# Meowuu7/equi-articulated-pose

Measured on AMD Instinct MI355X. Metric: point-clouds/sec (4096 pts, 60 anchors) fwd+bwd, higher is better.
Workload: dtype f32; 1 GPU; 8 x 4096-pt synthetic laptop clouds per GPU, 3-block inter backbone 1->64->128->512 (NN=64,K=24,A=60), forward+backward+Adam; clouds_per_gpu=8, points=4096, anchors=60

## Files before the change

equi-articulated-pose_amd/csrc/bn_act.hip:

```cpp
#include "common.h"

namespace {

constexpr int TB = 256;
constexpr int VPT = 8;
constexpr int SEG = TB * VPT * 4;

__device__ __forceinline__ float wave_sum(float v) {
#pragma unroll
    for (int o = 32; o > 0; o >>= 1) v += __shfl_xor(v, o);
    return v;
}

__device__ __forceinline__ void block_reduce2(float a, float b, float *pa, float *pb) {
    __shared__ float sa[TB / 64], sb[TB / 64];
    a = wave_sum(a); b = wave_sum(b);
    if ((threadIdx.x & 63) == 0) { sa[threadIdx.x >> 6] = a; sb[threadIdx.x >> 6] = b; }
    __syncthreads();
    if (threadIdx.x == 0) {
        float ta = 0.f, tb = 0.f;
#pragma unroll
        for (int i = 0; i < TB / 64; ++i) { ta += sa[i]; tb += sb[i]; }
        *pa = ta; *pb = tb;
    }
// ... 96 lines not shown
    const size_t o = ((size_t)ci * gridDim.z + bi) * nseg + seg;
    block_reduce2(s, q, pg + o, pgx + o);
}

template <bool CLOUD>
__global__ __launch_bounds__(TB) void bn_act_bwd_apply_kernel(int c, long n, float slope, const float *__restrict__ gy,
                                                             const float *__restrict__ x, const float *__restrict__ scale,
                                                             const float *__restrict__ shift, const float *__restrict__ mean,
                                                             const float *__restrict__ invstd, const float *__restrict__ k2,
                                                             const float *__restrict__ k3, float *__restrict__ gx,
                                                             const float *__restrict__ mask, int na) {
    const int seg = blockIdx.x, ci = blockIdx.y, bi = blockIdx.z;
    const int si = CLOUD ? bi * c + ci : ci;
    const float sc = scale[si], sh = shift[si], mu = mean[si], is = invstd[si], c2 = k2[si], c3 = k3[si];
    const size_t r0 = ((size_t)bi * c + ci) * n;
    const float *mrow = (CLOUD && mask) ? mask + (size_t)bi * (unsigned)(n / na) : nullptr;
    const long base = (long)seg * SEG;
    auto one = [&](float g, float xv, float m) {
        const float pre = fmaf(xv, sc, sh);
        const float gg = pre > 0.f ? g : g * slope;
        if (CLOUD) return fmaf(-m, fmaf((xv - mu) * is, c3, c2), gg * sc);
        return fmaf(gg, sc, -c2) - ((xv - mu) * is) * c3;
    };
#pragma unroll
    for (int v = 0; v < VPT; ++v) {
        const long i = base + ((long)v * TB + threadIdx.x) * 4;
        if (i + 3 < n) {
            const float4 g = *reinterpret_cast<const float4 *>(gy + r0 + i);
            const float4 a = *reinterpret_cast<const float4 *>(x + r0 + i);
            const float m = mrow ? mrow[(unsigned)i / (unsigned)na] : 1.f;
            *reinterpret_cast<float4 *>(gx + r0 + i) = make_float4(one(g.x, a.x, m), one(g.y, a.y, m), one(g.z, a.z, m), one(g.w, a.w, m));
        } else {
            for (long j = i; j < n; ++j) gx[r0 + j] = one(gy[r0 + j], x[r0 + j], mrow ? mrow[(unsigned)j / (unsigned)na] : 1.f);
        }
    }
}

constexpr int RM_PIECES = 16;
__global__ __launch_bounds__(256) void bn_act_bwd_apply_rowmax_kernel(int c, long n4, int nq, float slope, const float4 *__restrict__ gy,
                                                                      const float4 *__restrict__ x, const float *__restrict__ scale,
                                                                      const float *__restrict__ shift, const float *__restrict__ mean,
                                                                      const float *__restrict__ invstd, const float *__restrict__ k2,
                                                                      const float *__restrict__ k3, float4 *__restrict__ gx,
                                                                      unsigned *__restrict__ rowmax) {
    __shared__ unsigned s_max[256][4];
    const int ci = blockIdx.y, bi = blockIdx.z, t = threadIdx.x;
    const int T = nq * (256 / nq);
    const float sc = scale[ci], sh = shift[ci], mu = mean[ci], is = invstd[ci], c2 = k2[ci], c3 = k3[ci];
    const size_t r0 = ((size_t)bi * c + ci) * (size_t)n4;
    const long base = (long)blockIdx.x * RM_PIECES * T;
    auto one = [&](float g, float xv) {
        const float pre = fmaf(xv, sc, sh);
        const float gg = pre > 0.f ? g : g * slope;
        return fmaf(gg, sc, -c2) - ((xv - mu) * is) * c3;
    };
    unsigned m0 = 0, m1 = 0, m2 = 0, m3 = 0;
    if (t < T) {
        float4 g[RM_PIECES], a[RM_PIECES];
#pragma unroll
        for (int v = 0; v < RM_PIECES; ++v) {
            const long i = base + (long)v * T + t;
            if (i < n4) { g[v] = gy[r0 + i]; a[v] = x[r0 + i]; }
        }
#pragma unroll
        for (int v = 0; v < RM_PIECES; ++v) {
            const long i = base + (long)v * T + t;
            if (i < n4) {
                const float4 o = make_float4(one(g[v].x, a[v].x), one(g[v].y, a[v].y), one(g[v].z, a[v].z), one(g[v].w, a[v].w));
                gx[r0 + i] = o;
                m0 = max(m0, __float_as_uint(o.x) & 0x7fffffffu); m1 = max(m1, __float_as_uint(o.y) & 0x7fffffffu);
                m2 = max(m2, __float_as_uint(o.z) & 0x7fffffffu); m3 = max(m3, __float_as_uint(o.w) & 0x7fffffffu);
            }
        }
    }
    s_max[t][0] = m0; s_max[t][1] = m1; s_max[t][2] = m2; s_max[t][3] = m3;
    __syncthreads();
    if (t < 4 * nq) {
        unsigned v = 0;
        for (int u = t >> 2; u < T; u += nq) v = max(v, s_max[u][t & 3]);
        if (v) atomicMax(rowmax + ((size_t)bi * c + ci) * (4 * nq) + t, v);
    }
}

__global__ __launch_bounds__(256) void bn_act_bwd_reduce_fromy_kernel(int c, long n4, int nq, int nblk, float slope, float inv_slope, const float4 *__restrict__ gy,
                                                                      const float4 *__restrict__ y, const float *__restrict__ beta,
                                                                      const float *__restrict__ inv_gamma, float *__restrict__ pg, float *__restrict__ pgx,
                                                                      unsigned *__restrict__ gmax, unsigned *__restrict__ xmax) {
    __shared__ unsigned s_max[256][8];
    const int ci = blockIdx.y, bi = blockIdx.z, t = threadIdx.x;
    const int T = nq * (256 / nq);
    const float be = beta[ci], ig = inv_gamma[ci];
    const size_t r0 = ((size_t)bi * c + ci) * (size_t)n4;
    const long base = (long)blockIdx.x * RM_PIECES * T;
    float s = 0.f, q = 0.f;
    unsigned mg[4] = {0, 0, 0, 0}, mx[4] = {0, 0, 0, 0};
    if (t < T) {
        float4 g[RM_PIECES], a[RM_PIECES];
#pragma unroll
        for (int v = 0; v < RM_PIECES; ++v) {
            const long i = base + (long)v * T + t;
            if (i < n4) { g[v] = gy[r0 + i]; a[v] = y[r0 + i]; }
        }
#pragma unroll
        for (int v = 0; v < RM_PIECES; ++v) {
            const long i = base + (long)v * T + t;
            if (i < n4) {
                const float gv[4] = {g[v].x, g[v].y, g[v].z, g[v].w}, yv[4] = {a[v].x, a[v].y, a[v].z, a[v].w};
#pragma unroll
                for (int e = 0; e < 4; ++e) {
                    const bool pos = yv[e] > 0.f;
                    const float gg = pos ? gv[e] : gv[e] * slope, xh = ((pos ? yv[e] : yv[e] * inv_slope) - be) * ig;
                    s += gg;
                    q = fmaf(gg, xh, q);
                    mg[e] = max(mg[e], __float_as_uint(gg) & 0x7fffffffu);
                    mx[e] = max(mx[e], __float_as_uint(xh) & 0x7fffffffu);
                }
            }
        }
    }
#pragma unroll
    for (int e = 0; e < 4; ++e) { s_max[t][e] = mg[e]; s_max[t][4 + e] = mx[e]; }
    const size_t o = ((size_t)ci * gridDim.z + bi) * nblk + blockIdx.x;
    block_reduce2(s, q, pg + o, pgx + o);
    if (t < 4 * nq) {
        unsigned vg = 0, vx = 0;
        for (int u = t >> 2; u < T; u += nq) { vg = max(vg, s_max[u][t & 3]); vx = max(vx, s_max[u][4 + (t & 3)]); }
        const size_t at = ((size_t)bi * c + ci) * (4 * nq) + t;
        if (vg) atomicMax(gmax + at, vg);
        if (vx) atomicMax(xmax + at, vx);
    }
}

inline int nseg_of(long n) { return (int)((n + SEG - 1) / SEG); }

}

extern "C" int eap_bn_act_segments(int64_t n) { return nseg_of((long)n); }

extern "C" int eap_bn_stats_f32(int b, int c, int64_t n, const float *x, float *psum, float *psq, eap_stream_t stream) {
    if (b <= 0 || c <= 0 || n <= 0) return 0;
    if ((n & 3) != 0) return eap::bad_arg("bn_stats: row length must be a multiple of 4");
    const int nseg = nseg_of(n);
    return eap::run_kernel("bn_stats", bn_stats_kernel<false>, nseg, c, b, dim3(TB), 0, eap::S(stream), c, (long)n, nseg, x, psum, psq, (const float *)nullptr, 1);
}

extern "C" int eap_bn_act_fwd_f32(int b, int c, int64_t n, float slope, const float *x, const float *scale,
                                  const float *shift, float *y, eap_stream_t stream) {
    if (b <= 0 || c <= 0 || n <= 0) return 0;
    if ((n & 3) != 0) return eap::bad_arg("bn_act_fwd: row length must be a multiple of 4");
    return eap::run_kernel("bn_act_fwd", bn_act_fwd_kernel<false, false>, nseg_of(n), c, b, dim3(TB), 0, eap::S(stream), c, (long)n, slope, x, scale, shift,
                           (const float *)nullptr, y);
}

extern "C" int eap_bn_act_add_fwd_f32(int b, int c, int64_t n, float slope, const float *x, const float *scale,
                                      const float *shift, const float *res, float *y, eap_stream_t stream) {
    if (b <= 0 || c <= 0 || n <= 0) return 0;
    if ((n & 3) != 0) return eap::bad_arg("bn_act_add_fwd: row length must be a multiple of 4");
    return eap::run_kernel("bn_act_add_fwd", bn_act_fwd_kernel<true, false>, nseg_of(n), c, b, dim3(TB), 0, eap::S(stream), c, (long)n, slope, x, scale, shift,
                           res, y);
}

extern "C" int eap_bn_act_bwd_reduce_f32(int b, int c, int64_t n, float slope, const float *gy, const float *x,
                                         const float *scale, const float *shift, const float *mean,
                                         const float *invstd, float *pg, float *pgx, eap_stream_t stream) {
    if (b <= 0 || c <= 0 || n <= 0) return 0;
    if ((n & 3) != 0) return eap::bad_arg("bn_act_bwd_reduce: row length must be a multiple of 4");
    const int nseg = nseg_of(n);
    return eap::run_kernel("bn_act_bwd_reduce", bn_act_bwd_reduce_kernel<false>, nseg, c, b, dim3(TB), 0, eap::S(stream), c, (long)n, nseg, slope, gy, x,
                           scale, shift, mean, invstd, pg, pgx);
}

extern "C" int eap_bn_act_bwd_apply_f32(int b, int c, int64_t n, float slope, const float *gy, const float *x,
                                        const float *scale, const float *shift, const float *mean,
                                        const float *invstd, const float *k2, const float *k3, float *gx,
                                        eap_stream_t stream) {
    if (b <= 0 || c <= 0 || n <= 0) return 0;
    if ((n & 3) != 0) return eap::bad_arg("bn_act_bwd_apply: row length must be a multiple of 4");
    return eap::run_kernel("bn_act_bwd_apply", bn_act_bwd_apply_kernel<false>, nseg_of(n), c, b, dim3(TB), 0, eap::S(stream), c, (long)n, slope, gy, x,
                           scale, shift, mean, invstd, k2, k3, gx, (const float *)nullptr, 1);
}

extern "C" int eap_bn_act_bwd_apply_rowmax_f32(int b, int c, int64_t n, int na, float slope, const float *gy, const float *x,
                                               const float *scale, const float *shift, const float *mean,
                                               const float *invstd, const float *k2, const float *k3, float *gx, uint32_t *rowmax,
                                               eap_stream_t stream) {
    if (b <= 0 || c <= 0 || n <= 0) return 0;
    if (na <= 0 || (na & 3) != 0 || na > 256 || n % na != 0 ||
        ((reinterpret_cast<uintptr_t>(gy) | reinterpret_cast<uintptr_t>(x) | reinterpret_cast<uintptr_t>(gx)) & 15) != 0)
        return eap::bad_arg("bn_act_bwd_apply_rowmax: rows of [points][na], na a multiple of 4 up to 256, 16-byte aligned tensors");
    hipStream_t s = eap::S(stream);
    if (int e = eap::hip_fail(hipMemsetAsync(rowmax, 0, sizeof(uint32_t) * (size_t)b * c * na, s), "bn_act_bwd_apply_rowmax memset")) return e;
    const int nq = na / 4, T = nq * (256 / nq);
    const long n4 = (long)(n / 4);
    return eap::run_kernel("bn_act_bwd_apply_rowmax", bn_act_bwd_apply_rowmax_kernel, eap::cdiv(n4, (long)RM_PIECES * T), c, b, dim3(256), 0, s, c, n4, nq,
                           slope, reinterpret_cast<const float4 *>(gy), reinterpret_cast<const float4 *>(x), scale, shift, mean, invstd, k2, k3,
                           reinterpret_cast<float4 *>(gx), rowmax);
}

extern "C" int eap_bn_act_fromy_blocks(int64_t n, int na) {
    if (na <= 0 || (na & 3) != 0 || na > 256) return 0;
    const int nq = na / 4, T = nq * (256 / nq);
    const long n4 = (long)(n / 4);
    return (int)((n4 + (long)RM_PIECES * T - 1) / ((long)RM_PIECES * T));
}

extern "C" int eap_bn_act_bwd_reduce_fromy_f32(int b, int c, int64_t n, int na, float slope, const float *gy, const float *y, const float *beta,
                                               const float *inv_gamma, float *pg, float *pgx, uint32_t *gmax, uint32_t *xmax, eap_stream_t stream) {
    if (b <= 0 || c <= 0 || n <= 0) return 0;
    if (na <= 0 || (na & 3) != 0 || na > 256 || n % na != 0 || !(slope > 0.f) ||
        ((reinterpret_cast<uintptr_t>(gy) | reinterpret_cast<uintptr_t>(y)) & 15) != 0)
        return eap::bad_arg("bn_act_bwd_reduce_fromy: rows of [points][na], na a multiple of 4 up to 256, 16-byte aligned tensors, a positive slope");
    hipStream_t s = eap::S(stream);
    if (int e = eap::hip_fail(hipMemsetAsync(gmax, 0, sizeof(uint32_t) * (size_t)b * c * na, s), "bn_act_bwd_reduce_fromy memset")) return e;
    if (int e = eap::hip_fail(hipMemsetAsync(xmax, 0, sizeof(uint32_t) * (size_t)b * c * na, s), "bn_act_bwd_reduce_fromy memset")) return e;
    const int nq = na / 4, nblk = eap_bn_act_fromy_blocks(n, na);
    return eap::run_kernel("bn_act_bwd_reduce_fromy", bn_act_bwd_reduce_fromy_kernel, nblk, c, b, dim3(256), 0, s, c, (long)(n / 4), nq, nblk, slope,
                           1.0f / slope, reinterpret_cast<const float4 *>(gy), reinterpret_cast<const float4 *>(y), beta, inv_gamma, pg, pgx, gmax, xmax);
}

namespace {
inline int cloud_dims(const char *who, int b, int c, long n, int na, bool masked) {
    char buf[200];
    if ((n & 3) != 0 || n >= (1l << 31)) {
        snprintf(buf, sizeof(buf), "%s: row length must be a multiple of 4 below 2^31", who);
        return eap::bad_arg(buf);
    }
    if (masked && (na <= 0 || (na & 3) != 0 || n % na != 0)) {
        snprintf(buf, sizeof(buf), "%s: with a mask a row is [points][na], na a multiple of 4", who);
        return eap::bad_arg(buf);
    }
    return 0;
}
}

extern "C" int eap_bn_stats_masked_f32(int b, int c, int64_t n, int na, const float *x, const float *mask, float *psum, float *psq,
                                       eap_stream_t stream) {
    if (b <= 0 || c <= 0 || n <= 0) return 0;
    if (!mask) return eap::bad_arg("bn_stats_masked: mask is null");
    if (int e = cloud_dims("bn_stats_masked", b, c, (long)n, na, true)) return e;
    const int nseg = nseg_of(n);
    return eap::run_kernel("bn_stats_masked", bn_stats_kernel<true>, nseg, c, b, dim3(TB), 0, eap::S(stream), c, (long)n, nseg, x, psum, psq, mask, na);
}

extern "C" int eap_bn_act_cloud_fwd_f32(int b, int c, int64_t n, float slope, const float *x, const float *scale, const float *shift,
                                        float *y, eap_stream_t stream) {
    if (b <= 0 || c <= 0 || n <= 0) return 0;
    if (int e = cloud_dims("bn_act_cloud_fwd", b, c, (long)n, 0, false)) return e;
    return eap::run_kernel("bn_act_cloud_fwd", bn_act_fwd_kernel<false, true>, nseg_of(n), c, b, dim3(TB), 0, eap::S(stream), c, (long)n, slope, x, scale,
                           shift, (const float *)nullptr, y);
}

extern "C" int eap_bn_act_cloud_bwd_reduce_f32(int b, int c, int64_t n, float slope, const float *gy, const float *x, const float *scale,
                                               const float *shift, const float *mean, const float *invstd, float *pg, float *pgx,
                                               eap_stream_t stream) {
    if (b <= 0 || c <= 0 || n <= 0) return 0;
    if (int e = cloud_dims("bn_act_cloud_bwd_reduce", b, c, (long)n, 0, false)) return e;
    const int nseg = nseg_of(n);
    return eap::run_kernel("bn_act_cloud_bwd_reduce", bn_act_bwd_reduce_kernel<true>, nseg, c, b, dim3(TB), 0, eap::S(stream), c, (long)n, nseg, slope, gy, x,
                           scale, shift, mean, invstd, pg, pgx);
}

extern "C" int eap_bn_act_cloud_bwd_apply_f32(int b, int c, int64_t n, int na, float slope, const float *gy, const float *x,
                                              const float *scale, const float *shift, const float *mean, const float *invstd,
                                              const float *k2, const float *k3, const float *mask, float *gx, eap_stream_t stream) {
    if (b <= 0 || c <= 0 || n <= 0) return 0;
    if (int e = cloud_dims("bn_act_cloud_bwd_apply", b, c, (long)n, na, mask != nullptr)) return e;
    return eap::run_kernel("bn_act_cloud_bwd_apply", bn_act_bwd_apply_kernel<true>, nseg_of(n), c, b, dim3(TB), 0, eap::S(stream), c, (long)n, slope, gy, x,
                           scale, shift, mean, invstd, k2, k3, gx, mask, mask ? na : 1);
}
```

equi-articulated-pose_amd/csrc/inv_lists.hip:

```cpp
#include "common.h"

namespace {

constexpr int RT = 1024;
constexpr int MAXN = 16384;
constexpr int SORT_COMPACT = 2048;

__global__ __launch_bounds__(256) void inv_count_kernel(int per_cloud, int n, const int32_t *__restrict__ idx,
                                                        int32_t *__restrict__ counts) {
    extern __shared__ int s_hist[];
    const int bi = blockIdx.y, t = threadIdx.x;
    for (int i = t; i < n; i += 256) s_hist[i] = 0;
    __syncthreads();
    const int chunk = (per_cloud + gridDim.x - 1) / gridDim.x;
    const int beg = blockIdx.x * chunk, end = min(per_cloud, beg + chunk);
    const int32_t *src = idx + (size_t)bi * per_cloud;
    for (int e = beg + t; e < end; e += 256) {
        const int q = src[e];
        if ((unsigned)q < (unsigned)n) atomicAdd(&s_hist[q], 1);
    }
    __syncthreads();
    for (int i = t; i < n; i += 256) {
        const int v = s_hist[i];
        if (v) atomicAdd(&counts[(size_t)bi * n + i], v);
// ... 99 lines not shown
        if (i < qend) v = src[i];
        const bool m0 = v.x == q, m1 = v.y == q, m2 = v.z == q, m3 = v.w == q;
        const unsigned long long b0 = __ballot(m0), b1 = __ballot(m1), b2 = __ballot(m2), b3 = __ballot(m3);
        if ((b0 | b1 | b2 | b3) == 0ull) continue;
        int pos = base;
        pos += __builtin_amdgcn_mbcnt_hi((unsigned)(b0 >> 32), __builtin_amdgcn_mbcnt_lo((unsigned)b0, 0));
        pos += __builtin_amdgcn_mbcnt_hi((unsigned)(b1 >> 32), __builtin_amdgcn_mbcnt_lo((unsigned)b1, 0));
        pos += __builtin_amdgcn_mbcnt_hi((unsigned)(b2 >> 32), __builtin_amdgcn_mbcnt_lo((unsigned)b2, 0));
        pos += __builtin_amdgcn_mbcnt_hi((unsigned)(b3 >> 32), __builtin_amdgcn_mbcnt_lo((unsigned)b3, 0));
        const int e = 4 * i;
        if (m0) { dp[pos] = e / nn; dg[pos] = sg[e]; ++pos; }
        if (m1) { dp[pos] = (e + 1) / nn; dg[pos] = sg[e + 1]; ++pos; }
        if (m2) { dp[pos] = (e + 2) / nn; dg[pos] = sg[e + 2]; ++pos; }
        if (m3) { dp[pos] = (e + 3) / nn; dg[pos] = sg[e + 3]; ++pos; }
        base += __popcll(b0) + __popcll(b1) + __popcll(b2) + __popcll(b3);
    }
}

__global__ __launch_bounds__(256) void rows_gather_kernel(int c, int n, int na4, int rcap, int rld,
                                                          const int32_t *__restrict__ rows, const float4 *__restrict__ src,
                                                          float4 *__restrict__ dst) {
    const int bi = blockIdx.z, ci = blockIdx.y;
    const int e = blockIdx.x * 256 + threadIdx.x;
    if (e >= rcap * na4) return;
    const int r = e / na4, a = e - r * na4;
    const int q = rows[(size_t)bi * rld + r];
    float4 v = make_float4(0.f, 0.f, 0.f, 0.f);
    if (q >= 0) v = src[(((size_t)bi * c + ci) * n + q) * na4 + a];
    dst[(((size_t)bi * c + ci) * rcap + r) * na4 + a] = v;
}

__global__ __launch_bounds__(256) void rows_scatter_kernel(int c, int n, int na4, int rcap, int rld,
                                                           const int32_t *__restrict__ rows, const float4 *__restrict__ src,
                                                           float4 *__restrict__ dst) {
    const int bi = blockIdx.z, ci = blockIdx.y;
    const int e = blockIdx.x * 256 + threadIdx.x;
    if (e >= rcap * na4) return;
    const int r = e / na4, a = e - r * na4;
    const int q = rows[(size_t)bi * rld + r];
    if (q >= 0) dst[(((size_t)bi * c + ci) * n + q) * na4 + a] = src[(((size_t)bi * c + ci) * rcap + r) * na4 + a];
}

constexpr int PACKED_SLOTS = 64, PACKED_MAX_NA = 64;
__global__ __launch_bounds__(256) void rows_gather_packed_kernel(int c, int n, int na, int rp, int rld, long long ld, const int32_t *__restrict__ rows,
                                                                 const int32_t *__restrict__ n_rows, const float *__restrict__ src, float *__restrict__ dst) {
    __shared__ float tile[PACKED_SLOTS][PACKED_MAX_NA + 1];
    const int bi = blockIdx.z, ci = blockIdx.y, r0 = blockIdx.x * PACKED_SLOTS, t = threadIdx.x;
    const int live = eap::live16(n_rows[bi], rp), nr = min(n_rows[bi], live);
    if (r0 >= live) return;
    const float *s = src + ((size_t)bi * c + ci) * n * na;
    for (int i = t; i < PACKED_SLOTS * na; i += 256) {
        const int rr = i / na, a = i - rr * na, r = r0 + rr;
        const int q = r < nr ? rows[(size_t)bi * rld + r] : -1;
        tile[rr][a] = (q >= 0 && q < n) ? s[(size_t)q * na + a] : 0.f;
    }
    __syncthreads();
    float *d = dst + ((size_t)bi * c + ci) * ld;
    for (int i = t; i < PACKED_SLOTS * na; i += 256) {
        const int a = i / PACKED_SLOTS, rr = i - a * PACKED_SLOTS, r = r0 + rr;
        if (r < live) d[(size_t)a * live + r] = tile[rr][a];
    }
}

__global__ __launch_bounds__(256) void rows_scatter_packed_kernel(int c, int c_ld, int n, int na, int rp, int rld, long long ld, const int32_t *__restrict__ rows,
                                                                  const int32_t *__restrict__ n_rows, const float *__restrict__ src, float *__restrict__ dst) {
    __shared__ float tile[PACKED_SLOTS][PACKED_MAX_NA + 1];
    const int bi = blockIdx.z, ci = blockIdx.y, r0 = blockIdx.x * PACKED_SLOTS, t = threadIdx.x;
    const int live = eap::live16(n_rows[bi], rp), nr = min(n_rows[bi], live);
    if (r0 >= live) return;
    const float *s = src + ((size_t)bi * c_ld + ci) * ld;
    for (int i = t; i < PACKED_SLOTS * na; i += 256) {
        const int a = i / PACKED_SLOTS, rr = i - a * PACKED_SLOTS, r = r0 + rr;
        if (r < live) tile[rr][a] = s[(size_t)a * live + r];
    }
    __syncthreads();
    float *d = dst + ((size_t)bi * c + ci) * n * na;
    for (int i = t; i < PACKED_SLOTS * na; i += 256) {
        const int rr = i / na, a = i - rr * na, r = r0 + rr;
        const int q = r < nr ? rows[(size_t)bi * rld + r] : -1;
        if (q >= 0 && q < n) d[(size_t)q * na + a] = tile[rr][a];
    }
}

}

extern "C" int eap_inv_lists_rows(int b, int p, int n, int nn, const int32_t *idx, int32_t *counts, int32_t *rows,
                                  int32_t *off, int32_t *cnt, int32_t *n_rows, eap_stream_t stream) {
    if (b <= 0 || p <= 0 || nn <= 0 || n <= 0) return 0;
    if (n > MAXN) return eap::bad_arg("inv_lists_rows: more than 16384 support points per cloud");
    if ((long long)p * nn >= (1ll << 31)) return eap::bad_arg("inv_lists_rows: more than 2^31 entries per cloud");
    hipStream_t s = eap::S(stream);
    int e = eap::hip_fail(hipMemsetAsync(counts, 0, sizeof(int32_t) * (size_t)b * n, s), "inv_lists_rows memset");
    if (e) return e;
    const int per_cloud = p * nn;
    e = eap::run_kernel("inv_lists_rows (count)", inv_count_kernel, eap::cdiv(per_cloud, 8192), b, 1, dim3(256), sizeof(int) * n, s, per_cloud, n, idx, counts);
    if (e) return e;
    int n2 = RT;
    while (n2 < n) n2 <<= 1;
    const size_t shmem = sizeof(unsigned long long) * n2;
    return eap::run_kernel("inv_lists_rows (sort)", inv_rows_kernel, b, 1, 1, dim3(RT), shmem, s, n, n2, counts, rows, off, cnt, n_rows);
}

extern "C" int eap_inv_lists_fill(int b, int p, int n, int nn, int rcap, const int32_t *idx, const float *gx,
                                  const int32_t *rows, const int32_t *off, int32_t *ent_p, float *ent_gx,
                                  eap_stream_t stream) {
    if (b <= 0 || p <= 0 || nn <= 0 || rcap <= 0) return 0;
    if (((long long)p * nn & 3) != 0) return eap::bad_arg("inv_lists_fill: p * nn must be a multiple of 4");
    if (rcap > n) return eap::bad_arg("inv_lists_fill: rcap exceeds the number of support points");
    return eap::run_kernel("inv_lists_fill", inv_fill_kernel, rcap, b, 1, dim3(256), 0, eap::S(stream), p * nn, nn, n, n, idx, reinterpret_cast<const float4 *>(gx),
                           rows, off, ent_p, reinterpret_cast<float4 *>(ent_gx));
}

extern "C" int eap_rows_gather_f32(int b, int c, int n, int na, int rcap, int rows_ld, const int32_t *rows,
                                   const float *src, float *dst, eap_stream_t stream) {
    if (b <= 0 || c <= 0 || rcap <= 0) return 0;
    if ((na & 3) != 0) return eap::bad_arg("rows_gather: na must be a multiple of 4");
    return eap::run_kernel("rows_gather", rows_gather_kernel, eap::cdiv((long long)rcap * (na / 4), 256), c, b, dim3(256), 0, eap::S(stream), c, n, na / 4, rcap, rows_ld,
                           rows, reinterpret_cast<const float4 *>(src), reinterpret_cast<float4 *>(dst));
}

extern "C" int eap_rows_scatter_f32(int b, int c, int n, int na, int rcap, int rows_ld, const int32_t *rows,
                                    const float *src, float *dst, eap_stream_t stream) {
    if (b <= 0 || c <= 0) return 0;
    if ((na & 3) != 0) return eap::bad_arg("rows_scatter: na must be a multiple of 4");
    hipStream_t s = eap::S(stream);
    int e = eap::hip_fail(hipMemsetAsync(dst, 0, sizeof(float) * (size_t)b * c * n * na, s), "rows_scatter memset");
    if (e || rcap <= 0) return e;
    return eap::run_kernel("rows_scatter", rows_scatter_kernel, eap::cdiv((long long)rcap * (na / 4), 256), c, b, dim3(256), 0, s, c, n, na / 4, rcap, rows_ld, rows,
                           reinterpret_cast<const float4 *>(src), reinterpret_cast<float4 *>(dst));
}

extern "C" int eap_rows_gather_packed_f32(int b, int c, int n, int na, int rp, int rows_ld, int64_t ld, const int32_t *rows, const int32_t *n_rows,
                                          const float *src, float *dst, eap_stream_t stream) {
    if (!rows || !n_rows || !src || !dst) return eap::bad_arg("rows_gather_packed: null pointer");
    if (b <= 0 || c <= 0 || n <= 0 || na <= 0 || rp <= 0) return eap::bad_arg("rows_gather_packed: every size must be positive");
    if (na > PACKED_MAX_NA || rp % 16 != 0 || rows_ld < rp || ld < (int64_t)na * rp)
        return eap::bad_arg("rows_gather_packed: na <= 64, rp a multiple of 16, the row stride of rows >= rp, ld >= na * rp");
    return eap::run_kernel("rows_gather_packed", rows_gather_packed_kernel, eap::cdiv(rp, PACKED_SLOTS), c, b, dim3(256), 0, eap::S(stream), c, n, na, rp,
                           rows_ld, (long long)ld, rows, n_rows, src, dst);
}

extern "C" int eap_rows_scatter_packed_f32(int b, int c, int c_ld, int n, int na, int rp, int rows_ld, int64_t ld, const int32_t *rows,
                                           const int32_t *n_rows, const float *src, float *dst, eap_stream_t stream) {
    if (!rows || !n_rows || !src || !dst) return eap::bad_arg("rows_scatter_packed: null pointer");
    if (b <= 0 || c <= 0 || n <= 0 || na <= 0 || rp <= 0) return eap::bad_arg("rows_scatter_packed: every size must be positive");
    if (na > PACKED_MAX_NA || rp % 16 != 0 || rows_ld < rp || ld < (int64_t)na * rp || c_ld < c)
        return eap::bad_arg("rows_scatter_packed: na <= 64, rp a multiple of 16, the row stride of rows >= rp, ld >= na * rp, c_ld >= c");
    hipStream_t s = eap::S(stream);
    if (int e = eap::hip_fail(hipMemsetAsync(dst, 0, sizeof(float) * (size_t)b * c * n * na, s), "rows_scatter_packed memset")) return e;
    return eap::run_kernel("rows_scatter_packed", rows_scatter_packed_kernel, eap::cdiv(rp, PACKED_SLOTS), c, b, dim3(256), 0, s, c, c_ld, n, na, rp, rows_ld,
                           (long long)ld, rows, n_rows, src, dst);
}
```

equi-articulated-pose_amd/csrc/narrow_conv.hip:

```cpp
#include "common.h"
#include "device_prims.h"
#include <type_traits>

namespace {

constexpr int NT = 256, WAVES = 4;
constexpr int TILE = 128;
constexpr int SEGC = 2048;

__device__ __forceinline__ int drow(int r, int h) { return (r & 3) + 8 * (r >> 2) + 4 * h; }

template <int KS2>
__device__ __forceinline__ void load_x(f32x4 (&xa)[KS2], const float *__restrict__ xb, long n, long col0, unsigned voff, bool ok, int ck, int h) {
#pragma unroll
    for (int s = 0; s < KS2; ++s)
        xa[s] = (ok && 2 * s + h < ck) ? ld_off<f32x4>(xb + (size_t)(2 * s) * n + col0, voff) : (f32x4){0.f, 0.f, 0.f, 0.f};
}

template <int KS2>
__device__ __forceinline__ void load_w(float (&wf)[KS2], const float *__restrict__ W, int orow, int ck, int h) {
#pragma unroll
    for (int s = 0; s < KS2; ++s) wf[s] = (2 * s + h < ck) ? W[(size_t)orow * ck + 2 * s + h] : 0.f;
}

template <int KS2, bool T>
__device__ __forceinline__ void conv_tile(f32x16 (&d)[4], const f32x4 (&xa)[KS2], const float (&wf)[KS2]) {
#pragma unroll
    for (int c = 0; c < 4; ++c)
#pragma unroll
        for (int r = 0; r < 16; ++r) d[c][r] = 0.f;
#pragma unroll
    for (int s = 0; s < KS2; ++s) {
        if (T) {
            d[0] = __builtin_amdgcn_mfma_f32_32x32x2f32(xa[s].x, wf[s], d[0], 0, 0, 0);
            d[1] = __builtin_amdgcn_mfma_f32_32x32x2f32(xa[s].y, wf[s], d[1], 0, 0, 0);
            d[2] = __builtin_amdgcn_mfma_f32_32x32x2f32(xa[s].z, wf[s], d[2], 0, 0, 0);
            d[3] = __builtin_amdgcn_mfma_f32_32x32x2f32(xa[s].w, wf[s], d[3], 0, 0, 0);
        } else {
            d[0] = __builtin_amdgcn_mfma_f32_32x32x2f32(wf[s], xa[s].x, d[0], 0, 0, 0);
            d[1] = __builtin_amdgcn_mfma_f32_32x32x2f32(wf[s], xa[s].y, d[1], 0, 0, 0);
            d[2] = __builtin_amdgcn_mfma_f32_32x32x2f32(wf[s], xa[s].z, d[2], 0, 0, 0);
            d[3] = __builtin_amdgcn_mfma_f32_32x32x2f32(wf[s], xa[s].w, d[3], 0, 0, 0);
        }
    }
}

__device__ __forceinline__ void block_sums(float (&sa)[16], float (&qa)[16], float (*s_red)[2][32], int ct, int o0, int bi, int nb,
                                           int nseg, int seg, float *__restrict__ pa, float *__restrict__ pq) {
    const int t = threadIdx.x, lane = t & 63, wave = t >> 6, li = lane & 31, h = lane >> 5;
#pragma unroll
    for (int r = 0; r < 16; ++r) {
        float a = sa[r], q = qa[r];
#pragma unroll
        for (int d = 16; d > 0; d >>= 1) { a += __shfl_xor(a, d); q += __shfl_xor(q, d); }
        if (li == 0) { s_red[wave][0][drow(r, h)] = a; s_red[wave][1][drow(r, h)] = q; }
    }
    __syncthreads();
    if (t < 32 * ct) {
        float a = 0.f, q = 0.f;
        for (int w = t >> 5; w < WAVES; w += ct) { a += s_red[w][0][t & 31]; q += s_red[w][1][t & 31]; }
        const size_t at = ((size_t)(o0 + t) * nb + bi) * nseg + seg;
        pa[at] = a; pq[at] = q;
    }
}

struct Pos {
    int seg, bi, lane, li, h, ch0, cw, ncw;
    long beg, end;
    unsigned xoff;
    __device__ Pos(int ct, long n) {
        seg = blockIdx.x; bi = blockIdx.z;
        const int wave = threadIdx.x >> 6;
        lane = threadIdx.x & 63; li = lane & 31; h = lane >> 5;
        ch0 = (blockIdx.y * ct + wave % ct) * 32; cw = wave / ct; ncw = WAVES / ct;
        beg = (long)seg * SEGC; end = min(n, beg + SEGC);
        xoff = 4u * ((unsigned)h * (unsigned)n + 4u * li);
    }
};

template <int KS2>
__global__ __launch_bounds__(NT) void narrow_conv_stats_kernel(int ct, int ck, long n, int nseg, const float *__restrict__ W,
                                                                 const float *__restrict__ x, float *__restrict__ pivot,
                                                                 float *__restrict__ psum, float *__restrict__ psq) {
    __shared__ __attribute__((aligned(16))) float s_piv[64];
    __shared__ float s_red[WAVES][2][32];
    const Pos w(ct, n);
    const int t = threadIdx.x, o0 = blockIdx.y * ct * 32, h = w.h;
    if (t < 32 * ct) {
        float p = 0.f;
        for (int k = 0; k < ck; ++k) p = fmaf(W[(size_t)(o0 + t) * ck + k], x[(size_t)k * n], p);
        s_piv[t] = p;
        if (w.seg == 0 && w.bi == 0) pivot[o0 + t] = p;
    }
    __syncthreads();
    float wf[KS2];
    load_w<KS2>(wf, W, w.ch0 + w.li, ck, h);
    f32x4 pv[4];
#pragma unroll
    for (int g = 0; g < 4; ++g) pv[g] = *reinterpret_cast<const f32x4 *>(&s_piv[w.ch0 - o0 + 8 * g + 4 * h]);
    float sa[16], qa[16];
#pragma unroll
    for (int r = 0; r < 16; ++r) sa[r] = qa[r] = 0.f;
    const float *xb = x + (size_t)w.bi * ck * n;
#pragma unroll 1
    for (long col0 = w.beg + (long)w.cw * TILE; col0 < w.end; col0 += (long)w.ncw * TILE) {
        const long col = col0 + 4 * w.li;
        const bool ok = col < n;
        f32x4 xa[KS2];
        load_x<KS2>(xa, xb, n, col0, w.xoff, ok, ck, h);
        f32x16 d[4];
        conv_tile<KS2, false>(d, xa, wf);
        if (ok) {
#pragma unroll
            for (int r = 0; r < 16; ++r)
#pragma unroll
                for (int c = 0; c < 4; ++c) {
                    const float dd = d[c][r] - pv[r >> 2][r & 3];
                    sa[r] += dd;
                    qa[r] = fmaf(dd, dd, qa[r]);
                }
        }
    }
    block_sums(sa, qa, s_red, ct, o0, w.bi, gridDim.z, nseg, w.seg, psum, psq);
}

template <int KS2>
__global__ __launch_bounds__(NT) void narrow_conv_bnact_fwd_kernel(int ct, int o, int ck, long n, float slope, const float *__restrict__ W,
                                                                     const float *__restrict__ x, const float *__restrict__ scale,
                                                                     const float *__restrict__ shift, float *__restrict__ y) {
    const Pos w(ct, n);
    const int h = w.h;
    float wf[KS2];
    load_w<KS2>(wf, W, w.ch0 + w.li, ck, h);
    f32x4 sc[4], sh[4];
#pragma unroll
    for (int g = 0; g < 4; ++g) {
        sc[g] = *reinterpret_cast<const f32x4 *>(scale + w.ch0 + 8 * g + 4 * h);
        sh[g] = *reinterpret_cast<const f32x4 *>(shift + w.ch0 + 8 * g + 4 * h);
    }
    const float *xb = x + (size_t)w.bi * ck * n;
    float *yb = y + ((size_t)w.bi * o + w.ch0) * n;
    const unsigned roff = 4u * (4u * h * (unsigned)n + 4u * w.li);
#pragma unroll 1
    for (long col0 = w.beg + (long)w.cw * TILE; col0 < w.end; col0 += (long)w.ncw * TILE) {
        const long col = col0 + 4 * w.li;
        const bool ok = col < n;
        f32x4 xa[KS2];
        load_x<KS2>(xa, xb, n, col0, w.xoff, ok, ck, h);
        f32x16 d[4];
        conv_tile<KS2, false>(d, xa, wf);
        if (ok) {
#pragma unroll
            for (int r = 0; r < 16; ++r) {
                const float a = sc[r >> 2][r & 3], b = sh[r >> 2][r & 3];
                f32x4 v;
                v.x = fmaf(d[0][r], a, b); v.y = fmaf(d[1][r], a, b); v.z = fmaf(d[2][r], a, b); v.w = fmaf(d[3][r], a, b);
                v.x = v.x > 0.f ? v.x : v.x * slope; v.y = v.y > 0.f ? v.y : v.y * slope;
                v.z = v.z > 0.f ? v.z : v.z * slope; v.w = v.w > 0.f ? v.w : v.w * slope;
                st_off<f32x4>(yb + (size_t)(8 * (r >> 2)) * n + col0, roff + 4u * (unsigned)(r & 3) * (unsigned)n, v);
            }
        }
    }
}

template <int KS2>
__global__ __launch_bounds__(NT) void narrow_conv_bwd_reduce_kernel(int ct, int o, int ck, long n, int nseg, float slope,
                                                                      const float *__restrict__ gy, const float *__restrict__ x,
                                                                      const float *__restrict__ W, const float *__restrict__ scale,
                                                                      const float *__restrict__ shift, const float *__restrict__ mean,
                                                                      const float *__restrict__ invstd, float *__restrict__ pg,
                                                                      float *__restrict__ pgx) {
    __shared__ __attribute__((aligned(16))) float s_sc[64], s_sh[64], s_mu[64], s_is[64];
    __shared__ float s_red[WAVES][2][32];
    const Pos w(ct, n);
    const int t = threadIdx.x, o0 = blockIdx.y * ct * 32, h = w.h;
    if (t < 32 * ct) { s_sc[t] = scale[o0 + t]; s_sh[t] = shift[o0 + t]; s_mu[t] = mean[o0 + t]; s_is[t] = invstd[o0 + t]; }
    __syncthreads();
    float wf[KS2];
    load_w<KS2>(wf, W, w.ch0 + w.li, ck, h);
    float sa[16], qa[16];
#pragma unroll
    for (int r = 0; r < 16; ++r) sa[r] = qa[r] = 0.f;
    const float *xb = x + (size_t)w.bi * ck * n;
    const float *gb = gy + ((size_t)w.bi * o + w.ch0) * n;
    const unsigned roff = 4u * (4u * h * (unsigned)n + 4u * w.li);
    const int lc = w.ch0 - o0;
#pragma unroll 1
    for (long col0 = w.beg + (long)w.cw * TILE; col0 < w.end; col0 += (long)w.ncw * TILE) {
        const long col = col0 + 4 * w.li;
        const bool ok = col < n;
        f32x4 xa[KS2];
        load_x<KS2>(xa, xb, n, col0, w.xoff, ok, ck, h);
        f32x16 d[4];
        conv_tile<KS2, false>(d, xa, wf);
        if (ok) {
#pragma unroll
            for (int g = 0; g < 4; ++g) {
                f32x4 gv[4];
#pragma unroll
                for (int q = 0; q < 4; ++q) gv[q] = ld_off<f32x4>(gb + (size_t)(8 * g) * n + col0, roff + 4u * q * (unsigned)n);
                const f32x4 sc = *reinterpret_cast<const f32x4 *>(&s_sc[lc + 8 * g + 4 * h]), sh = *reinterpret_cast<const f32x4 *>(&s_sh[lc + 8 * g + 4 * h]);
                const f32x4 mu = *reinterpret_cast<const f32x4 *>(&s_mu[lc + 8 * g + 4 * h]), is = *reinterpret_cast<const f32x4 *>(&s_is[lc + 8 * g + 4 * h]);
#pragma unroll
                for (int q = 0; q < 4; ++q)
#pragma unroll
                    for (int c = 0; c < 4; ++c) {
                        const float yv = d[c][4 * g + q];
                        const float pre = fmaf(yv, sc[q], sh[q]);
                        const float gg = pre > 0.f ? gv[q][c] : gv[q][c] * slope;
                        sa[4 * g + q] += gg;
                        qa[4 * g + q] = fmaf(gg, (yv - mu[q]) * is[q], qa[4 * g + q]);
                    }
            }
        }
    }
    block_sums(sa, qa, s_red, ct, o0, w.bi, gridDim.z, nseg, w.seg, pg, pgx);
}

template <int KS2>
__global__ __launch_bounds__(NT) void narrow_conv_bwd_dw_kernel(int ct, int o, int ck, long n, int nseg, float slope,
                                                                  const float *__restrict__ gy, const float *__restrict__ x,
                                                                  const float *__restrict__ W, const float *__restrict__ scale,
                                                                  const float *__restrict__ shift, const float *__restrict__ mean,
                                                                  const float *__restrict__ invstd, const float *__restrict__ k2,
                                                                  const float *__restrict__ k3, float *__restrict__ partial) {
    __shared__ float s_part[WAVES][16][64];
    const Pos w(ct, n);
    const int h = w.h, li = w.li, wave = threadIdx.x >> 6;
    const int ch = w.ch0 + li;
    float wf[KS2];
    load_w<KS2>(wf, W, ch, ck, h);
    const float sc = scale[ch], sh = shift[ch], mu = mean[ch], is = invstd[ch], c2 = k2[ch], c3 = k3[ch];
    const float *gb = gy + ((size_t)w.bi * o + w.ch0) * n;
    const unsigned goff = 4u * ((unsigned)li * (unsigned)n + 16u * h), koff = 4u * ((unsigned)min(li, ck - 1) * (unsigned)n + 16u * h);
    f32x16 dw;
#pragma unroll
    for (int r = 0; r < 16; ++r) dw[r] = 0.f;
    const float *xb = x + (size_t)w.bi * ck * n;
    const f32x4 zero4 = {0.f, 0.f, 0.f, 0.f};
#pragma unroll 1
    for (long col0 = w.beg + (long)w.cw * TILE; col0 < w.end; col0 += (long)w.ncw * TILE) {
        const long col = col0 + 4 * li;
        f32x4 xa[KS2];
        load_x<KS2>(xa, xb, n, col0, w.xoff, col < n, ck, h);
        f32x16 d[4];
        conv_tile<KS2, true>(d, xa, wf);
#pragma unroll
        for (int g = 0; g < 4; ++g) {
            f32x4 gv[4], xv[4];
#pragma unroll
            for (int q = 0; q < 4; ++q) {
                const long cq = col0 + 4 * (8 * g + 4 * h + q);
                const bool in = cq < n;
                gv[q] = in ? ld_off<f32x4>(gb + col0 + 4 * (8 * g + q), goff) : zero4;
                xv[q] = (in && li < ck) ? ld_off<f32x4>(xb + col0 + 4 * (8 * g + q), koff) : zero4;
            }
#pragma unroll
            for (int q = 0; q < 4; ++q)
#pragma unroll
                for (int c = 0; c < 4; ++c) {
                    const float yv = d[c][4 * g + q];
                    const float pre = fmaf(yv, sc, sh);
                    const float gg = pre > 0.f ? gv[q][c] : gv[q][c] * slope;
                    const float gx = fmaf(gg, sc, -c2) - ((yv - mu) * is) * c3;
                    dw = __builtin_amdgcn_mfma_f32_32x32x2f32(gx, xv[q][c], dw, 0, 0, 0);
                }
        }
    }
#pragma unroll
    for (int r = 0; r < 16; ++r) s_part[wave][r][w.lane] = dw[r];
    __syncthreads();
    if (wave < ct) {
        float *slab = partial + ((size_t)w.bi * nseg + w.seg) * o * ck;
#pragma unroll
        for (int r = 0; r < 16; ++r) {
            float v = 0.f;
            for (int u = wave; u < WAVES; u += ct) v += s_part[u][r][w.lane];
            if (li < ck) slab[(size_t)(w.ch0 + drow(r, h)) * ck + li] = v;
        }
    }
}

__global__ __launch_bounds__(256) void narrow_conv_dw_sum_kernel(int mn, int slabs, const float *__restrict__ partial, float *__restrict__ dW) {
    const int e = blockIdx.x * 4 + (threadIdx.x >> 6), lane = threadIdx.x & 63;
    if (e >= mn) return;
    float s = 0.f;
    for (int z = lane; z < slabs; z += 64) s += partial[(size_t)z * mn + e];
#pragma unroll
    for (int d = 32; d > 0; d >>= 1) s += __shfl_xor(s, d);
    if (lane == 0) dW[e] = s;
}

inline int nseg_of(long n) { return (int)((n + SEGC - 1) / SEGC); }

inline bool misaligned(const void *p) { return (reinterpret_cast<uintptr_t>(p) & 15) != 0; }

inline int refuse(const char *who, int o, int ck, long n, const void *p0, const void *p1, const void *p2 = nullptr) {
    char buf[200];
    const char *why = nullptr;
    if (ck < 1 || ck > 32) why = "1 to 32 contraction indices (C*K)";
    else if (o < 32 || o % 32 != 0) why = "a multiple of 32 output channels";
    else if (n < 0 || (n & 3) != 0 || n >= (1l << 25)) why = "a row length (P*A) that is a multiple of 4 below 2^25";
    else if (misaligned(p0) || misaligned(p1) || misaligned(p2)) why = "16-byte aligned tensors";
    if (!why) return 0;
    snprintf(buf, sizeof(buf), "%s: takes %s", who, why);
    return eap::bad_arg(buf);
}

inline int tiles_per_block(int o) { return o % 64 == 0 ? 2 : 1; }

template <typename F>
int by_depth(int ck, F &&f) {
    return ck <= 24 ? f(std::integral_constant<int, 12>{}) : f(std::integral_constant<int, 16>{});
}

}

extern "C" int eap_narrow_conv_segments(int64_t n) { return n > 0 ? nseg_of((long)n) : 0; }

extern "C" int eap_narrow_conv_stats_f32(int b, int o, int ck, int64_t n, const float *W, const float *x, float *pivot, float *psum,
                                         float *psq, eap_stream_t stream) {
    if (int e = refuse("narrow_conv_stats", o, ck, (long)n, x, nullptr)) return e;
    if (b <= 0 || n <= 0) return 0;
    const int nseg = nseg_of((long)n), ct = tiles_per_block(o);
    return by_depth(ck, [&](auto ks2) {
        return eap::run_kernel("narrow_conv_stats", narrow_conv_stats_kernel<decltype(ks2)::value>, nseg, o / (32 * ct), b, dim3(NT), 0, eap::S(stream), ct,
                               ck, (long)n, nseg, W, x, pivot, psum, psq);
    });
}

extern "C" int eap_narrow_conv_bnact_fwd_f32(int b, int o, int ck, int64_t n, float slope, const float *W, const float *x, const float *scale,
                                             const float *shift, float *y, eap_stream_t stream) {
    if (int e = refuse("narrow_conv_bnact_fwd", o, ck, (long)n, x, y, scale)) return e;
    if (misaligned(shift)) return eap::bad_arg("narrow_conv_bnact_fwd: takes 16-byte aligned tensors");
    if (b <= 0 || n <= 0) return 0;
    const int ct = tiles_per_block(o);
    return by_depth(ck, [&](auto ks2) {
        return eap::run_kernel("narrow_conv_bnact_fwd", narrow_conv_bnact_fwd_kernel<decltype(ks2)::value>, nseg_of((long)n), o / (32 * ct), b, dim3(NT), 0,
                               eap::S(stream), ct, o, ck, (long)n, slope, W, x, scale, shift, y);
    });
}

extern "C" int eap_narrow_conv_bwd_reduce_f32(int b, int o, int ck, int64_t n, float slope, const float *gy, const float *x, const float *W,
                                              const float *scale, const float *shift, const float *mean, const float *invstd, float *pg,
                                              float *pgx, eap_stream_t stream) {
    if (int e = refuse("narrow_conv_bwd_reduce", o, ck, (long)n, x, gy)) return e;
    if (b <= 0 || n <= 0) return 0;
    const int nseg = nseg_of((long)n), ct = tiles_per_block(o);
    return by_depth(ck, [&](auto ks2) {
        return eap::run_kernel("narrow_conv_bwd_reduce", narrow_conv_bwd_reduce_kernel<decltype(ks2)::value>, nseg, o / (32 * ct), b, dim3(NT), 0, eap::S(stream),
                               ct, o, ck, (long)n, nseg, slope, gy, x, W, scale, shift, mean, invstd, pg, pgx);
    });
}

extern "C" int eap_narrow_conv_bwd_dw_f32(int b, int o, int ck, int64_t n, float slope, const float *gy, const float *x, const float *W,
                                          const float *scale, const float *shift, const float *mean, const float *invstd, const float *k2,
                                          const float *k3, float *partial, float *dW, eap_stream_t stream) {
    if (int e = refuse("narrow_conv_bwd_dw", o, ck, (long)n, x, gy)) return e;
    if (b <= 0 || n <= 0) return 0;
    const int nseg = nseg_of((long)n), ct = tiles_per_block(o);
    hipStream_t s = eap::S(stream);
    int e = by_depth(ck, [&](auto ks2) {
        return eap::run_kernel("narrow_conv_bwd_dw", narrow_conv_bwd_dw_kernel<decltype(ks2)::value>, nseg, o / (32 * ct), b, dim3(NT), 0, s, ct, o, ck, (long)n,
                               nseg, slope, gy, x, W, scale, shift, mean, invstd, k2, k3, partial);
    });
    if (e) return e;
    const int mn = o * ck;
    return eap::run_kernel("narrow_conv_bwd_dw (sum)", narrow_conv_dw_sum_kernel, eap::cdiv(mn, 4), 1, 1, dim3(256), 0, s, mn, b * nseg, partial, dW);
}
```

equi-articulated-pose_amd/csrc/so3_dense.hip:

```cpp
#include <atomic>
#include "common.h"
#include "device_prims.h"
#include <type_traits>

namespace {

typedef unsigned long long u64;
typedef const __attribute__((address_space(4))) unsigned long long *cu64p;

constexpr int KC_BK = 32;
constexpr int KC_LIST_BYTES = 4096;

__host__ __device__ __forceinline__ void dense_kr(int d, int ks, int &k, int &r) {
    const int g = d / (16 * ks), rem = d - g * 16 * ks;
    k = rem >> 4;
    r = 16 * g + (rem & 15);
}


__device__ __forceinline__ void split2(float x0, float x1, unsigned &h, unsigned &l) {
    asm("v_cvt_pk_f16_f32 %0, %2, %3\n\t"
        "v_fma_mixlo_f16 %1, %0, -1.0, %2 op_sel:[0,0,0] op_sel_hi:[1,0,0]\n\t"
        "v_fma_mixhi_f16 %1, %0, -1.0, %3 op_sel:[1,0,0] op_sel_hi:[1,0,0]"
        : "=&v"(h), "=&v"(l) : "v"(x0), "v"(x1));
// ... 173 lines not shown
}

__global__ __launch_bounds__(256) void dense_rows_kernel(int n_sup, int na, int ks, int rp, int kd_pad, int rows_ld,
                                                         const float *__restrict__ s_xyz, const float *__restrict__ centre,
                                                         const int32_t *__restrict__ rows, const float *__restrict__ rk,
                                                         const float *__restrict__ row_rot, f32x4 *__restrict__ kr) {
    const int b = blockIdx.z, a = blockIdx.y, i = blockIdx.x * 256 + threadIdx.x;
    if (i >= kd_pad) return;
    f32x4 v = {1e4f, 1e4f, 1e4f, 0.f};
    if (i < ks * rp) {
        int k, r;
        dense_kr(i, ks, k, r);
        const int row = rows[(size_t)b * rows_ld + r];
        if ((unsigned)row < (unsigned)n_sup) {
            const float *kp = rk + ((size_t)a * ks + k) * 3;
            double k0 = (double)kp[0], k1 = (double)kp[1], k2 = (double)kp[2];
            if (row_rot != nullptr) {
                const float *M = row_rot + ((size_t)b * rows_ld + r) * 9;
                const double t0 = M[0] * k0 + M[1] * k1 + M[2] * k2, t1 = M[3] * k0 + M[4] * k1 + M[5] * k2, t2 = M[6] * k0 + M[7] * k1 + M[8] * k2;
                k0 = t0; k1 = t1; k2 = t2;
            }
            const double x = (double)s_xyz[((size_t)b * 3 + 0) * n_sup + row] - (double)centre[b * 4 + 0] - k0;
            const double y = (double)s_xyz[((size_t)b * 3 + 1) * n_sup + row] - (double)centre[b * 4 + 1] - k1;
            const double z = (double)s_xyz[((size_t)b * 3 + 2) * n_sup + row] - (double)centre[b * 4 + 2] - k2;
            v = (f32x4){(float)x, (float)y, (float)z, 0.f};
        }
    }
    kr[((size_t)b * na + a) * kd_pad + i] = v;
}

__global__ __launch_bounds__(256) void dense_rowmax_kernel(int m, int l, int na, int seg, long long seg_pitch4, const int32_t *__restrict__ colmap,
                                                           const f32x4 *__restrict__ T, float *__restrict__ scale, float *__restrict__ scale2) {
    __shared__ unsigned s[256][4];
    const int nq = na >> 2, G = 256 / nq, b = blockIdx.y, row = blockIdx.x, t = threadIdx.x;
    const int aq = t % nq, pg = t / nq;
    unsigned v0 = 0, v1 = 0, v2 = 0, v3 = 0;
    if (pg < G) {
        const f32x4 *src = T + ((size_t)b * m + row) * (colmap ? (size_t)1 : (size_t)(l / seg)) * seg_pitch4;
        for (int i0 = pg; i0 < l; i0 += 8 * G) {
            f32x4 q[8];
#pragma unroll
            for (int u = 0; u < 8; ++u) {
                const int i = min(i0 + u * G, l - 1), sg = i / seg;
                if (colmap != nullptr) {
                    const int ci = colmap[(size_t)b * l + i];
                    q[u] = ci >= 0 ? src[(size_t)ci * nq + aq] : (f32x4){0.f, 0.f, 0.f, 0.f};
                } else {
                    q[u] = src[(size_t)sg * seg_pitch4 + (size_t)(i - sg * seg) * nq + aq];
                }
            }
#pragma unroll
            for (int u = 0; u < 8; ++u) {
                v0 = max(v0, __float_as_uint(q[u].x) & 0x7fffffffu);
                v1 = max(v1, __float_as_uint(q[u].y) & 0x7fffffffu);
                v2 = max(v2, __float_as_uint(q[u].z) & 0x7fffffffu);
                v3 = max(v3, __float_as_uint(q[u].w) & 0x7fffffffu);
            }
        }
    }
    s[t][0] = v0; s[t][1] = v1; s[t][2] = v2; s[t][3] = v3;
    __syncthreads();
    if (t < na) {
        unsigned v = 0;
        for (int g = 0; g < G; ++g) v = max(v, s[g * nq + (t >> 2)][t & 3]);
        const float sc = pow2_scale(__uint_as_float(v));
        scale[((size_t)b * na + t) * m + row] = sc;
        scale2[((size_t)b * m + row) * na + t] = sc;
    }
}

__global__ __launch_bounds__(256) void dense_scale_kernel(long long total, int m, int na, const unsigned *__restrict__ rowmax,
                                                          float *__restrict__ scale, float *__restrict__ scale2) {
    const long long i = (long long)blockIdx.x * 256 + threadIdx.x;
    if (i >= total) return;
    const int a = (int)(i % na);
    const long long br = i / na;
    const int row = (int)(br % m);
    const long long b = br / m;
    const float sc = pow2_scale(__uint_as_float(rowmax[i]));
    scale[(b * na + a) * m + row] = sc;
    scale2[i] = sc;
}

struct SplitBn { const f32x4 *Y2; const float *coef; float slope, inv_slope; };
template <bool BN>
__global__ __launch_bounds__(256) __attribute__((amdgpu_waves_per_eu(2, 2))) void dense_split_kernel(int m, int l, int na, int kb_total, int seg, long long seg_pitch4, int mapped,
                                                          const int32_t *__restrict__ n_rows, const int32_t *__restrict__ colmap,
                                                          const f32x4 *__restrict__ T, const float *__restrict__ scale2,
                                                          u32x4 *__restrict__ planes, SplitBn bn) {
    extern __shared__ u32x4 image[];
    const int t = threadIdx.x;
    const int MT = m >> 5;
    const unsigned blk = blockIdx.x >> 1;
    const int kg = (int)(blockIdx.x & 1u), kb = (int)(blk % (unsigned)kb_total), grp_ = (int)(blk / (unsigned)kb_total), mt = grp_ % MT, b = grp_ / MT;
    const int nq = na >> 2, RG = 256 / nq;
    const int aq = t % nq, rr = t / nq;
    const int nseg = l / seg;
    if (mapped && n_rows != nullptr && 16 * kb >= ((min(n_rows[b], seg) + 15) & ~15) * nseg) return;
    const int l0 = 16 * kb + 8 * kg;
    unsigned at[8], keep[8];
    int live = 0;
    if (colmap != nullptr) {
        int ci[8] = {-1, -1, -1, -1, -1, -1, -1, -1};
        if (l0 < l) {
            const int4 c0 = *reinterpret_cast<const int4 *>(colmap + (size_t)b * l + l0), c1 = *reinterpret_cast<const int4 *>(colmap + (size_t)b * l + l0 + 4);
            ci[0] = c0.x; ci[1] = c0.y; ci[2] = c0.z; ci[3] = c0.w; ci[4] = c1.x; ci[5] = c1.y; ci[6] = c1.z; ci[7] = c1.w;
        }
#pragma unroll
        for (int e = 0; e < 8; ++e) { keep[e] = ci[e] >= 0 ? ~0u : 0u; at[e] = (unsigned)max(ci[e], 0) * (unsigned)nq; live |= (int)(keep[e] & 1u) << e; }
    } else {
        int sg = l0 / seg, sr = l0 - sg * seg;
        if (mapped) dense_kr(l0, nseg, sg, sr);
#pragma unroll
        for (int e = 0; e < 8; ++e) {
            keep[e] = l0 + e < l ? ~0u : 0u;
            at[e] = keep[e] ? (unsigned)sg * (unsigned)seg_pitch4 + (unsigned)sr * (unsigned)nq : 0u;
            live |= (int)(keep[e] & 1u) << e;
            if (++sr == seg) { sr = 0; ++sg; }
        }
#pragma unroll
        for (int e = 1; e < 8; ++e) at[e] = keep[e] ? at[e] : at[0];
    }
    if (live == 0)
        for (int i = t; i < 64 * na; i += 256) image[i] = (u32x4){0u, 0u, 0u, 0u};
    for (int it0 = rr; it0 < 32 && rr < RG && live != 0; it0 += 2 * RG) {
        f32x4 q[2][8];
        f32x4 q2[BN ? 2 : 1][BN ? 8 : 1];
        int rowv[2];
#pragma unroll
        for (int u = 0; u < 2; ++u) {
            const int row = 32 * mt + min(it0 + u * RG, 31);
            rowv[u] = row;
            const size_t row_off = ((size_t)b * m + row) * (colmap ? (size_t)1 : (size_t)nseg) * seg_pitch4 + aq;
#pragma unroll
            for (int e = 0; e < 8; ++e) q[u][e] = T[row_off + at[e]];
            if constexpr (BN) {
#pragma unroll
                for (int e = 0; e < 8; ++e) q2[u][e] = bn.Y2[row_off + at[e]];
            }
        }
        __builtin_amdgcn_sched_barrier(0);
        if constexpr (BN) {
#pragma unroll
            for (int u = 0; u < 2; ++u) {
                const float k1 = bn.coef[rowv[u]], k2 = bn.coef[m + rowv[u]], k3 = bn.coef[2 * m + rowv[u]], be = bn.coef[3 * m + rowv[u]], ig = bn.coef[4 * m + rowv[u]];
#pragma unroll
                for (int e = 0; e < 8; ++e)
#pragma unroll
                    for (int j = 0; j < 4; ++j) {
                        const float yv = q2[u][e][j], gv = q[u][e][j];
                        const bool pos = yv > 0.f;
                        const float gg = pos ? gv : gv * bn.slope, pre = pos ? yv : yv * bn.inv_slope;
                        const float gx = fmaf(gg, k1, -k2) - ((pre - be) * ig) * k3;
                        q[u][e][j] = __uint_as_float(__float_as_uint(gx) & keep[e]);
                    }
            }
        } else if (live != 255) {
#pragma unroll
            for (int u = 0; u < 2; ++u)
#pragma unroll
                for (int e = 0; e < 8; ++e)
#pragma unroll
                    for (int j = 0; j < 4; ++j) q[u][e][j] = __uint_as_float(__float_as_uint(q[u][e][j]) & keep[e]);
        }
#pragma unroll
        for (int u = 0; u < 2; ++u) {
            const int i = it0 + u * RG;
            if (i >= 32) break;
            const f32x4 sc = *reinterpret_cast<const f32x4 *>(scale2 + ((size_t)b * m + rowv[u]) * na + 4 * aq);
            u32x4 *dst = image + 256 * aq + ((i + aq) & 31);
#pragma unroll
            for (int j = 0; j < 4; ++j) {
                unsigned h[4], lo[4];
#pragma unroll
                for (int e = 0; e < 4; ++e) split2(q[u][2 * e][j] * sc[j], q[u][2 * e + 1][j] * sc[j], h[e], lo[e]);
                dst[64 * j] = (u32x4){h[0], h[1], h[2], h[3]};
                dst[64 * j + 32] = (u32x4){lo[0], lo[1], lo[2], lo[3]};
            }
        }
    }
    __syncthreads();
    const int w = t >> 6, pl = (t >> 5) & 1, i = t & 31;
    for (int k = 0; k < nq; ++k) {
        const int a = 4 * k + w;
        planes[((((size_t)b * na + a) * kb_total + kb) * MT + mt) * 128 + 64 * pl + 32 * kg + i] = image[64 * a + 32 * pl + ((i + k) & 31)];
    }
}

template <int CSTEPS>
__global__ __launch_bounds__(256) void dense_gplanes_kernel(int m, int na, int ks, int rp, int rch, int kb_total, const float *__restrict__ W3,
                                                            const float *__restrict__ Ft, const int32_t *__restrict__ n_rows,
                                                            const float *__restrict__ bound, float *__restrict__ scale, u32x4 *__restrict__ planes) {
    constexpr int C = 16 * CSTEPS, PITCH = 2 * C + 16;
    extern __shared__ __attribute__((aligned(16))) unsigned char smem[];
    __shared__ unsigned s_red[4];
    const int z = blockIdx.y, b = z / na;
    const int t = threadIdx.x, lane = t & 63, li = lane & 31, kg = lane >> 5, wave = t >> 6;
    const int rows_b = n_rows ? min((min(n_rows[b], rp) + 15) & ~15, rp) : rp;
    unsigned char *Fh = smem, *Fl = smem + (size_t)rch * PITCH;
    const int MT = m >> 5, mt = blockIdx.x * 4 + wave;
    const bool active = mt < MT;
    const int o = 32 * min(mt, MT - 1) + li;
    const float s_out = pow2_scale(bound[(size_t)z * m + o]);
    if (active && kg == 0) scale[(size_t)z * m + o] = s_out;
    for (int rc0 = 0; rc0 < rows_b; rc0 += rch) {
        const int nrows = min(rch, rows_b - rc0);
        if (rc0 > 0) __syncthreads();
        const f32x4 *src = reinterpret_cast<const f32x4 *>(Ft + ((size_t)z * rp + rc0) * C);
        const int n4 = nrows * (C / 4);
        unsigned mx = 0;
        for (int i = t; i < n4; i += 256) {
            const f32x4 v = src[i];
            mx = max(mx, max(max(__float_as_uint(v.x) & 0x7fffffffu, __float_as_uint(v.y) & 0x7fffffffu),
                             max(__float_as_uint(v.z) & 0x7fffffffu, __float_as_uint(v.w) & 0x7fffffffu)));
        }
#pragma unroll
        for (int o_ = 32; o_ > 0; o_ >>= 1) mx = max(mx, (unsigned)__shfl_xor((int)mx, o_));
        if (lane == 0) s_red[wave] = mx;
// ... 490 lines not shown
    const int wtiles = 4 * ((n + 255) / 256), steps = kd / KC_BK;
    return ((int64_t)b * wtiles * steps * 64 + 1) / 2;
}

namespace {
template <int W>
int dense_member(int b, int p, int n_sup, int nn, int rp, int rows_ld, const int32_t *idx, const int32_t *rows, const int32_t *n_rows, int32_t *slot_of,
                 uint32_t *memb, int32_t *flags, eap_stream_t stream) {
    if (b <= 0 || p <= 0) return 0;
    if (rp <= 0 || rp > 32 * W) return eap::bad_arg(W == MEMB_WORDS ? "so3_dense_member: 0 < rp <= 512" : "so3_dense_member_wide: 0 < rp <= 1024");
    hipStream_t s = eap::S(stream);
    if (int e = eap::hip_fail(hipMemsetAsync(slot_of, 0xff, sizeof(int32_t) * (size_t)b * n_sup, s), "so3_dense_member memset")) return e;
    if (int e = eap::hip_fail(hipMemsetAsync(flags, 0, sizeof(int32_t) * (size_t)b, s), "so3_dense_member memset")) return e;
    if (int e = eap::run_kernel("so3_dense_member", dense_slots_kernel, eap::cdiv(rp, 256), b, 1, dim3(256), 0, s, n_sup, rp, rows_ld, rows, n_rows, slot_of)) return e;
    return eap::run_kernel("so3_dense_member", dense_member_kernel<W>, eap::cdiv(p, 256), b, 1, dim3(256), 0, s, p, n_sup, nn, rp, idx, slot_of, memb, flags);
}

template <int W>
int dense_masks(int b, int p, int ks, int rp, int dir, const uint32_t *memb, uint64_t *mask, eap_stream_t stream) {
    if (b <= 0) return 0;
    if (!dense_shape_ok(p, 4, ks, rp, 256, W)) return eap::bad_arg("so3_dense_masks: shape not taken");
    const int n = dir ? p : ks * rp, kd = dir ? ceil_to(ks * rp, KC_BK) : p;
    const int wtiles = 4 * ((n + 255) / 256), steps = kd / KC_BK;
    return eap::run_kernel("so3_dense_masks", dense_mask_kernel<W>, eap::cdiv((long long)wtiles * steps, 4), b, 1, dim3(256), 0, eap::S(stream), p, ks, rp, dir, wtiles, steps,
                           memb, reinterpret_cast<unsigned *>(mask));
}
}

extern "C" int eap_so3_dense_member(int b, int p, int n_sup, int nn, int rp, int rows_ld, const int32_t *idx, const int32_t *rows,
                                    const int32_t *n_rows, int32_t *slot_of, uint32_t *memb, int32_t *flags, eap_stream_t stream) {
    return dense_member<MEMB_WORDS>(b, p, n_sup, nn, rp, rows_ld, idx, rows, n_rows, slot_of, memb, flags, stream);
}

extern "C" int eap_so3_dense_member_wide(int b, int p, int n_sup, int nn, int rp, int rows_ld, const int32_t *idx, const int32_t *rows,
                                         const int32_t *n_rows, int32_t *slot_of, uint32_t *memb, int32_t *flags, eap_stream_t stream) {
    return dense_member<MEMB_WORDS_WIDE>(b, p, n_sup, nn, rp, rows_ld, idx, rows, n_rows, slot_of, memb, flags, stream);
}

extern "C" int eap_so3_dense_masks(int b, int p, int ks, int rp, int dir, const uint32_t *memb, uint64_t *mask, eap_stream_t stream) {
    return dense_masks<MEMB_WORDS>(b, p, ks, rp, dir, memb, mask, stream);
}

extern "C" int eap_so3_dense_masks_wide(int b, int p, int ks, int rp, int dir, const uint32_t *memb, uint64_t *mask, eap_stream_t stream) {
    return dense_masks<MEMB_WORDS_WIDE>(b, p, ks, rp, dir, memb, mask, stream);
}

extern "C" int eap_so3_dense_tables_f32(int b, int p, int n_sup, int na, int ks, int rp, int rows_ld, float sigma, const float *q_xyz,
                                        const float *s_xyz, const int32_t *rows, const float *rk, const float *row_rot, float *centre, float *pt,
                                        float *kr, eap_stream_t stream) {
    if (b <= 0) return 0;
    if (!(sigma > 0.f)) return eap::bad_arg("so3_dense_tables: sigma > 0");
    hipStream_t s = eap::S(stream);
    const int p_pad = ceil_to(p, KC_BK), kd_pad = ceil_to(ks * rp, KC_BK);
    if (int e = eap::run_kernel("so3_dense_tables", dense_centre_kernel, b, 1, 1, dim3(256), 0, s, n_sup, s_xyz, centre)) return e;
    if (int e = eap::run_kernel("so3_dense_tables", dense_points_kernel, eap::cdiv(p_pad, 256), b, 1, dim3(256), 0, s, p, p_pad, q_xyz, centre,
                                reinterpret_cast<f32x4 *>(pt)))
        return e;
    return eap::run_kernel("so3_dense_tables", dense_rows_kernel, eap::cdiv(kd_pad, 256), na, b, dim3(256), 0, s, n_sup, na, ks, rp, kd_pad, rows_ld,
                           s_xyz, centre, rows, rk, row_rot, reinterpret_cast<f32x4 *>(kr));
}

extern "C" int eap_so3_dense_split_f32(int b, int m, int l, int na, int seg, int64_t seg_pitch, int mapped, const int32_t *n_rows, const uint32_t *rowmax,
                                       const int32_t *colmap, const float *src, float *scale, void *planes, eap_stream_t stream) {
    if (b <= 0) return 0;
    if (colmap != nullptr) {
        if (mapped || seg_pitch <= 0 || (l & 7) != 0 || (reinterpret_cast<uintptr_t>(colmap) & 15) != 0)
            return eap::bad_arg("so3_dense_split: a column map (16-byte aligned, a multiple of 8 columns) comes with the source row pitch and without the dense-index mapping");
        seg = l;
    }
    if (seg <= 0) { seg = l; seg_pitch = (int64_t)l * na; }
    if ((m % 32) != 0 || (na % 4) != 0 || na > 64 || (reinterpret_cast<uintptr_t>(src) & 15) || l % seg != 0 ||
        (seg_pitch & 3) != 0 || (colmap == nullptr && seg_pitch < (int64_t)seg * na) || (mapped && ((seg % 16) != 0 || ((l / seg) % 2) != 0)))
        return eap::bad_arg("so3_dense_split: m % 32, na % 4, na <= 64, 16-byte aligned source, whole segments of a 16-byte aligned pitch (mapped: seg % 16, an even number of segments)");
    if ((colmap ? (int64_t)1 : (int64_t)(l / seg)) * (seg_pitch / 4) > 0x7fffffffLL) return eap::bad_arg("so3_dense_split: a source row of at most 2^31 16-byte pieces");
    hipStream_t s = eap::S(stream);
    const int kb_total = ceil_to(l, KC_BK) / 16;
    float *scale2 = scale + (size_t)b * na * m;
    const int e = rowmax != nullptr
                      ? eap::run_kernel("so3_dense_split", dense_scale_kernel, eap::cdiv((long long)b * m * na, 256), 1, 1, dim3(256), 0, s, (long long)b * m * na, m, na, rowmax, scale, scale2)
                      : eap::run_kernel("so3_dense_split", dense_rowmax_kernel, m, b, 1, dim3(256), 0, s, m, l, na, seg, (long long)(seg_pitch / 4), colmap,
                                        reinterpret_cast<const f32x4 *>(src), scale, scale2);
    if (e) return e;
    return eap::run_kernel("so3_dense_split", dense_split_kernel<false>, (long long)kb_total * (m / 32) * b * 2, 1, 1, dim3(256), (size_t)na * 1024, s, m, l, na, kb_total, seg, (long long)(seg_pitch / 4),
                           mapped ? 1 : 0, n_rows, colmap, reinterpret_cast<const f32x4 *>(src), scale2, reinterpret_cast<u32x4 *>(planes), SplitBn{nullptr, nullptr, 1.f, 1.f});
}

extern "C" int eap_so3_dense_split_bn_f32(int b, int m, int l, int l_src, int na, const uint32_t *rowbound, const int32_t *colmap, const float *grad,
                                          const float *act, const float *coef, float slope, float *scale, void *planes, eap_stream_t stream) {
    if (b <= 0) return 0;
    if (colmap == nullptr && l != l_src) return eap::bad_arg("so3_dense_split_bn: without a column map l = l_src");
    if ((m % 32) != 0 || (na % 4) != 0 || na > 64 || ((reinterpret_cast<uintptr_t>(grad) | reinterpret_cast<uintptr_t>(act)) & 15) ||
        (colmap != nullptr && ((l & 7) != 0 || (reinterpret_cast<uintptr_t>(colmap) & 15) != 0)) || rowbound == nullptr || coef == nullptr || !(slope > 0.f))
        return eap::bad_arg("so3_dense_split_bn: m % 32, na % 4, na <= 64, 16-byte aligned sources, a bound per row, a positive slope (column map: 16-byte aligned, l % 8)");
    if ((int64_t)l_src * na / 4 > 0x7fffffffLL) return eap::bad_arg("so3_dense_split_bn: a source row of at most 2^31 16-byte pieces");
    hipStream_t s = eap::S(stream);
    const int kb_total = ceil_to(l, KC_BK) / 16;
    float *scale2 = scale + (size_t)b * na * m;
    if (int e = eap::run_kernel("so3_dense_split_bn", dense_scale_kernel, eap::cdiv((long long)b * m * na, 256), 1, 1, dim3(256), 0, s, (long long)b * m * na, m, na, rowbound, scale,
                                scale2))
        return e;
    const int seg = colmap ? l : l_src;
    return eap::run_kernel("so3_dense_split_bn", dense_split_kernel<true>, (long long)kb_total * (m / 32) * b * 2, 1, 1, dim3(256), (size_t)na * 1024, s, m, l, na, kb_total, seg,
                           (long long)l_src * na / 4, 0, nullptr, colmap, reinterpret_cast<const f32x4 *>(grad), scale2, reinterpret_cast<u32x4 *>(planes),
                           SplitBn{reinterpret_cast<const f32x4 *>(act), coef, slope, 1.0f / slope});
}

namespace {
int untranspose_args(const char *what, int o, int p, int na, const float *yt, const float *y) {
    char buf[256];
    const char *why = nullptr;
    if (o <= 0 || p <= 0) why = "o > 0 and p > 0";
    else if (na <= 0 || (na % 4) != 0) why = "na % 4 == 0 (rows of Y are stored as 16-byte pieces)";
    else if (na > 64) why = "na <= 64 (the tile of a block)";
    else if (yt == nullptr || (reinterpret_cast<uintptr_t>(yt) & 15) != 0) why = "yt 16-byte aligned";
    else if (y == nullptr || (reinterpret_cast<uintptr_t>(y) & 15) != 0) why = "y 16-byte aligned";
    if (why == nullptr) return 0;
    snprintf(buf, sizeof(buf), "%s: %s", what, why);
    return eap::bad_arg(buf);
}

int untranspose_tile(const char *what, int b, int o, int p, int na, int p_dst, const int32_t *map, const float *yt, float *y, const float *bn_scale,
                     const float *bn_shift, float slope, eap_stream_t stream) {
    return eap::run_kernel(what, dense_untranspose_tile_kernel, (long long)eap::cdiv(p, UT_PTS) * o * b, 1, 1, dim3(256), sizeof(float) * (size_t)na * UT_PTS,
                           eap::S(stream), o, p, na, p_dst, map, yt, y, bn_scale, bn_shift, slope);
}
}

extern "C" int eap_so3_dense_untranspose_bnact_f32(int b, int o, int p, int na, int p_dst, const int32_t *map, const float *yt, const float *bn_scale,
                                                   const float *bn_shift, float slope, float *y, eap_stream_t stream) {
    if (b <= 0) return 0;
    if (bn_scale == nullptr || bn_shift == nullptr || (map != nullptr && p_dst <= 0) || (map == nullptr && p_dst != p))
        return eap::bad_arg("so3_dense_untranspose_bnact: scale and shift per channel; p_dst = p without a map");
    if (int e = untranspose_args("so3_dense_untranspose_bnact", o, p, na, yt, y)) return e;
    return untranspose_tile("so3_dense_untranspose_bnact", b, o, p, na, p_dst, map, yt, y, bn_scale, bn_shift, slope, stream);
}

extern "C" int eap_so3_dense_gplanes_supported(int o, int c, int na, int ks, int rp) {
    return (o % 32) == 0 && (c == 64 || c == 128) && na > 0 && ks > 0 && (ks % 2) == 0 && rp > 0 && (rp % 16) == 0;
}

extern "C" int eap_so3_dense_gplanes_f32(int b, int o, int c, int na, int ks, int rp, const float *W3, const float *Ft, const int32_t *n_rows,
                                         const float *bound, float *scale, void *planes, eap_stream_t stream) {
    if (b <= 0) return 0;
    if (!eap_so3_dense_gplanes_supported(o, c, na, ks, rp) ||
        ((reinterpret_cast<uintptr_t>(W3) | reinterpret_cast<uintptr_t>(Ft) | reinterpret_cast<uintptr_t>(planes)) & 15) != 0)
        return eap::bad_arg("so3_dense_gplanes: shape not taken (eap_so3_dense_gplanes_supported), 16-byte aligned operands");
    const int kb_total = ceil_to(ks * rp, KC_BK) / 16;
    const int fit = (int)((84u * 1024u) / ((size_t)(2 * c + 16) * 2)) / 16 * 16;
    const int rch = min(rp, max(fit, 32));
    const size_t shmem = (size_t)rch * (2 * c + 16) * 2;
    return eap::run_kernel("so3_dense_gplanes", c == 128 ? dense_gplanes_kernel<8> : dense_gplanes_kernel<4>, eap::cdiv(o / 32, 4), (long long)b * na, 1, dim3(256), shmem,
                           eap::S(stream), o, na, ks, rp, rch, kb_total, W3, Ft, n_rows, bound, scale, reinterpret_cast<u32x4 *>(planes));
}

namespace {

int dense_product(int dir, int packed, int b, int o, int p, int na, int ks, int rp, int64_t ldz, float sigma, const int32_t *n_rows, const void *planes,
                  const float *scale, const float *pt, const float *kr, const uint64_t *mask, const int32_t *steps, float *out, eap_stream_t stream) {
    if (b <= 0) return 0;
    if (!eap_so3_dense_supported(p, na, ks, rp, o)) return eap::bad_arg("so3_dense_product: shape not taken (eap_so3_dense_supported)");
    const int p_pad = ceil_to(p, KC_BK), kd_pad = ceil_to(ks * rp, KC_BK);
    KcArgs g;
    g.MT = o / 32; g.na = na; g.zcount = b * na; g.row_slots = rp; g.packed = packed;
    g.N = dir ? p : ks * rp;
    g.KS = (dir ? kd_pad : p) / KC_BK;
    const bool wide = (o % 256) == 0;
    g.tiles_m = wide ? o / 256 : o / 128;
    g.blocks_n = (g.N + 255) / 256;
    g.mask_tiles = 4 * g.blocks_n;
    g.A = reinterpret_cast<const u32x4 *>(planes);
    g.scale = scale;
    const f32x4 *ptT = reinterpret_cast<const f32x4 *>(pt), *krT = reinterpret_cast<const f32x4 *>(kr);
    if (dir == 0) {
        g.strT = ptT; g.strB = p_pad; g.strA = 0;
        g.colT = krT; g.colB = (long long)na * kd_pad; g.colA = kd_pad;
        if (ldz < (int64_t)na * rp) return eap::bad_arg("so3_dense_product: ldz < na rp");
        g.cB = (long long)o * ks * ldz; g.cA = rp; g.ldm = (long long)ks * ldz; g.rp = rp; g.kstride = ldz;
    } else {
        g.strT = krT; g.strB = (long long)na * kd_pad; g.strA = kd_pad;
        g.colT = ptT; g.colB = p_pad; g.colA = 0;
        g.cB = (long long)na * o * p; g.cA = (long long)o * p; g.ldm = p; g.rp = p; g.kstride = 0;
    }
    g.mask = reinterpret_cast<const unsigned *>(mask);
    g.steps = (steps != nullptr && g.KS <= KC_LIST_BYTES / 4) ? steps : nullptr;
    g.C = out;
    g.neg_inv_sigma = -1.0f / sigma;
    g.n_rows = n_rows; g.ks = ks; g.trim = dir ? 2 : 1;
// ... 96 lines not shown
```

equi-articulated-pose_amd/vgtk/_hip.py:

```python
import ctypes
import os
import re
import struct
import types
import warnings
import weakref

import torch

_PKG_ROOT = os.path.abspath(os.path.join(os.path.dirname(__file__), '..'))
LIB_PATH = os.path.join(_PKG_ROOT, 'libeap_hip.so')

if not os.path.exists(LIB_PATH):
    raise ImportError(
        f'{LIB_PATH} not found: build the HIP extension first '
        '(python -c "import __graft_entry__ as g; g.build()" or make -C equi-articulated-pose_amd/csrc). '
        'This package has no CPU fallback.')

lib = ctypes.CDLL(LIB_PATH)


_HEADERS = (os.path.join(_PKG_ROOT, 'include', 'eap_hip.h'), os.path.join(os.path.dirname(_PKG_ROOT), 'include', 'eap_hip.h'))
HEADER_PATH = next((p for p in _HEADERS if os.path.exists(p)), _HEADERS[-1])

# ... 1099 lines not shown


def matmul_reduce_tail(A, B, out, ncols):
    if not matmul_reduce_tail_takes(A, B, out):
        raise RuntimeError('matmul_reduce_tail: the operands do not qualify for the split kernel (matmul_reduce_tail_takes)')
    ta, tb, M, N, K, lda, sa, ldb, sb, ldc, _, batch = _product(A, B, out, reduce=True)
    ws = torch.empty(max(int(abi.eap_gemm_bf16x3_reduce_workspace(M, N, K, batch)), 4), dtype=torch.float32, device=out.device)
    tag = {'flops': 2.0 * M * N * K * batch, 'shape': ('gemm_reduce_tail', 0, 1, M, N, K, batch)}
    call('eap_gemm_bf16x3_reduce_tail_f32', out, M, N, K, A, lda, sa, B, ldb, sb, out, ldc, batch, ncols, ws, tag=tag)


def so3_dense_gplanes_bound(W3, fc4, ks):
    check_input(W3, fc4)
    b, c, rp, na = fc4.shape
    o = W3.shape[0] // ks
    dev = fc4.device
    fpart = torch.empty(b, c, na, dtype=torch.float32, device=dev)
    wsum = torch.empty(o, dtype=torch.float32, device=dev)
    bound = torch.empty(b, na, o, dtype=torch.float32, device=dev)
    call('eap_so3_dense_gplanes_bound_f32', fc4, b, o, c, na, int(ks), rp, W3, fc4, fpart, wsum, bound)
    return bound


def so3_dense_point_order(order, memb, q_xyz):
    check_input(order, memb, q_xyz)
    b, p = order.shape
    order32 = torch.empty(b, p, dtype=torch.int32, device=order.device)
    memb_out, xyz_out = torch.empty_like(memb), torch.empty_like(q_xyz)
    pivot_pos = torch.empty(1, dtype=torch.int32, device=order.device)
    call('eap_so3_dense_point_order', order, b, p, memb.shape[2], order, memb, q_xyz, order32, memb_out, xyz_out, pivot_pos)
    return order32, memb_out, xyz_out, pivot_pos


def so3_dense_fwd(g, geo, p, c=0, ldg=None, out=None, col_map=None, operand=None, o=None):
    yt = _dense_fwd_yt(g, geo, p, c, ldg, operand, o)
    b, na, o = yt.shape[0], geo.na, yt.shape[2]
    if col_map is not None:
        if out is None or col_map.dtype != torch.int32 or tuple(col_map.shape) != (b, p) or not col_map.is_contiguous() or not out.is_contiguous():
            raise RuntimeError('so3_dense_fwd: col_map must be a contiguous int32 [b,p] and come with a contiguous out')
        call('eap_so3_dense_untranspose_map_f32', yt, b, o, p, na, out.shape[2], geo.columns(col_map), yt, out)
        return out
    y = torch.empty(b, o, p, na, dtype=torch.float32, device=yt.device)
    chunks = (p + 63) // 64
    ps = torch.empty(o, b * chunks, dtype=torch.float32, device=yt.device)
    pq = torch.empty_like(ps)
    if geo.order is not None:
        call('eap_so3_dense_untranspose_map_stats_f32', yt, b, o, p, na, p, geo.order, geo.pivot_pos, yt, y, ps, pq)
    else:
        call('eap_so3_dense_untranspose_f32', yt, b, o, p, na, yt, y, ps, pq)
    leave_stats_hint(y, (ps, pq))
    return y


def _dense_fwd_yt(g, geo, p, c, ldg, operand, o):
    na = geo.na
    if operand is None:
        b, o = g.shape[:2]
        ldg = geo.rp * na if ldg is None else int(ldg)
        scale, planes = so3_dense_split(g, seg=geo.rp, seg_pitch=ldg, shape=(b, o, geo.ks * geo.rp, na), mapped=True, n_rows=geo.n_rows)
    else:
        scale, planes = operand
        b = geo.b
    yt = torch.empty(b, na, o, p, dtype=torch.float32, device=planes.device)
    return _dense_product(1, geo, b, o, p, 0, scale, planes, yt, 2.0 * b * c * geo.ks * na * (p * geo.nn + o * p - o * geo.rp))


def so3_dense_fwd_bnact(g, geo, p, c, ldg, norm_moments, operand=None, o=None, affine=None, partials=False):
    yt = _dense_fwd_yt(g, geo, p, c, ldg, operand, o)
    b, na, o = yt.shape[0], geo.na, yt.shape[2]
    if affine is not None:
        bn_scale, bn_shift, slope = affine[0].contiguous(), affine[1].contiguous(), float(affine[2])
    else:
        ps, pq = _partials(yt, b * na, o, p)
        call('eap_bn_stats_f32', yt, b * na, o, p, yt, ps, pq)
        if partials:
            bn_scale, bn_shift, slope = norm_moments(ps, pq, yt[0, 0, :, 0], b * na * p)
        else:
            bn_scale, bn_shift, slope = norm_moments(ps.sum(1, dtype=torch.float64), pq.sum(1, dtype=torch.float64), yt[0, 0, :, 0].double(), b * na * p)
    y = torch.empty(b, o, p, na, dtype=torch.float32, device=yt.device)
    call('eap_so3_dense_untranspose_bnact_f32', yt, b, o, p, na, p, geo.order, yt, bn_scale, bn_shift, slope, y)
    return y


def bn_act_bwd_reduce_fromy(gy, y, beta, inv_gamma, slope, partials=False):
    b, c, p, na = y.shape
    n = p * na
    nblk = int(abi.eap_bn_act_fromy_blocks(n, na))
    pg = torch.empty(c, b * nblk, dtype=torch.float32, device=y.device)
    pgx = torch.empty_like(pg)
    gmax = torch.empty(b, c, na, dtype=torch.int32, device=y.device)
    xmax = torch.empty_like(gmax)
    call('eap_bn_act_bwd_reduce_fromy_f32', y, b, c, n, na, slope, gy, y, beta, inv_gamma, pg, pgx, gmax, xmax)
    if partials:
        return pg, pgx, gmax.view(torch.float32), xmax.view(torch.float32)
    return pg.sum(1, dtype=torch.float64), pgx.sum(1, dtype=torch.float64), gmax.view(torch.float32), xmax.view(torch.float32)


def so3_dense_bwd_bn(gy, yact, geo, ldz, coef, rowbound, slope, packed=False):
    b, o, p, na = gy.shape
    ldz = na * geo.rp if ldz is None else int(ldz)
    colmap = geo.columns(None)
    l = p if colmap is None else colmap.shape[1]
    scale = torch.empty(2, b, na, o, dtype=torch.float32, device=gy.device)
    planes = torch.empty(b * na * o * ((l + 31) // 32 * 32), dtype=torch.int32, device=gy.device)
    call('eap_so3_dense_split_bn_f32', gy, b, o, l, p, na, rowbound.view(torch.int32), colmap, gy, yact, coef, slope, scale, planes)
    z = torch.empty(b, o, geo.ks, ldz, dtype=torch.float32, device=gy.device)
    return _dense_product(0, geo, b, o, l, ldz, scale, planes, z, 2.0 * b * o * l * na * geo.ks * geo.nn, packed=packed)


def _partials(x, b, c, n):
    nseg = int(abi.eap_bn_act_segments(n))
    return (torch.empty(c, b * nseg, dtype=torch.float32, device=x.device),
            torch.empty(c, b * nseg, dtype=torch.float32, device=x.device))


_STATS_HINT = [None]
STATS_HINTS_TAKEN = 0


def _leave_hint(slot, t, payload):
    slot[0] = (weakref.ref(t), t._version, tuple(t.shape), payload)


def _take_hint(slot, t):
    h, slot[0] = slot[0], None
    if not USE_ROWMAX_HINT or h is None or h[0]() is not t or h[1] != t._version or h[2] != tuple(t.shape):
        return None
    return h[3]


def leave_stats_hint(t, partials):
    _leave_hint(_STATS_HINT, t, partials)


def take_stats_hint(t):
    global STATS_HINTS_TAKEN
    partials = _take_hint(_STATS_HINT, t)
    STATS_HINTS_TAKEN += partials is not None
    return partials


def bn_stats(x, b, c, n):
    hint = take_stats_hint(x)
    if hint is not None and hint[0].shape[0] == c:
        return hint[0].sum(1, dtype=torch.float64), hint[1].sum(1, dtype=torch.float64)
    ps, pq = _partials(x, b, c, n)
    call('eap_bn_stats_f32', x, b, c, n, x, ps, pq)
    return ps.sum(1, dtype=torch.float64), pq.sum(1, dtype=torch.float64)


def bn_act_fwd(x, b, c, n, scale, shift, slope, residual=None):
    y = torch.empty_like(x)
    if residual is None:
        call('eap_bn_act_fwd_f32', x, b, c, n, slope, x, scale, shift, y)
    else:
        call('eap_bn_act_add_fwd_f32', x, b, c, n, slope, x, scale, shift, residual, y)
    return y


def bn_act_bwd_reduce(gy, x, b, c, n, scale, shift, mean, invstd, slope):
    pg, pgx = _partials(x, b, c, n)
    call('eap_bn_act_bwd_reduce_f32', x, b, c, n, slope, gy, x, scale, shift, mean, invstd, pg, pgx)
    return pg.sum(1, dtype=torch.float64), pgx.sum(1, dtype=torch.float64)


_ROWMAX_HINT = [None]
USE_ROWMAX_HINT = True
ROWMAX_HINTS_TAKEN = 0


def leave_rowmax_hint(t, rowmax):
    _leave_hint(_ROWMAX_HINT, t, rowmax)


def take_rowmax_hint(t):
    global ROWMAX_HINTS_TAKEN
    rowmax = _take_hint(_ROWMAX_HINT, t)
    ROWMAX_HINTS_TAKEN += rowmax is not None
    return rowmax


def bn_act_bwd_apply(gy, x, b, c, n, scale, shift, mean, invstd, k2, k3, slope):
    gx = torch.empty_like(x)
    if x.dim() == 4 and x.shape[3] % 4 == 0 and x.shape[3] <= 64 and n == x.shape[2] * x.shape[3] and c % 128 == 0 and gx.data_ptr() % 16 == 0 \
            and gy.data_ptr() % 16 == 0 and x.data_ptr() % 16 == 0:
        rowmax = torch.empty(b, c, x.shape[3], dtype=torch.int32, device=x.device)
        call('eap_bn_act_bwd_apply_rowmax_f32', x, b, c, n, int(x.shape[3]), slope, gy, x, scale, shift, mean, invstd, k2, k3, gx, rowmax)
        leave_rowmax_hint(gx, rowmax)
        return gx
    call('eap_bn_act_bwd_apply_f32', x, b, c, n, slope, gy, x, scale, shift, mean, invstd, k2, k3, gx)
    return gx



NARROW_CONV_MAX_CK = 32


def narrow_conv_takes(o, ck, n):
    return 1 <= ck <= NARROW_CONV_MAX_CK and o >= 32 and o % 32 == 0 and n % 4 == 0 and n < (1 << 25)


def _narrow_partials(x, b, o, n):
    nseg = int(abi.eap_narrow_conv_segments(n))
    return (torch.empty(o, b * nseg, dtype=torch.float32, device=x.device),
            torch.empty(o, b * nseg, dtype=torch.float32, device=x.device))


def narrow_conv_stats(W, x, partials=False):
    check_input(W, x)
    b, ck, n = x.shape
    o = W.shape[0]
    ps, pq = _narrow_partials(x, b, o, n)
    pivot = torch.empty(o, dtype=torch.float32, device=x.device)
    call('eap_narrow_conv_stats_f32', x, b, o, ck, n, W, x, pivot, ps, pq)
    if partials:
        return ps, pq, pivot
    return ps.sum(1, dtype=torch.float64), pq.sum(1, dtype=torch.float64), pivot.double()


def narrow_conv_bnact_fwd(W, x, scale, shift, slope):
    check_input(W, x, scale, shift)
    b, ck, n = x.shape
    o = W.shape[0]
    y = torch.empty(b, o, n, dtype=torch.float32, device=x.device)
    call('eap_narrow_conv_bnact_fwd_f32', x, b, o, ck, n, slope, W, x, scale, shift, y)
    return y


def narrow_conv_bwd_reduce(gy, x, W, scale, shift, mean, invstd, slope, partials=False):
    check_input(gy, x, W, scale, shift, mean, invstd)
    b, ck, n = x.shape
    o = W.shape[0]
    pg, pgx = _narrow_partials(x, b, o, n)
    call('eap_narrow_conv_bwd_reduce_f32', x, b, o, ck, n, slope, gy, x, W, scale, shift, mean, invstd, pg, pgx)
    if partials:
        return pg, pgx
    return pg.sum(1, dtype=torch.float64), pgx.sum(1, dtype=torch.float64)


def narrow_conv_bwd_dw(gy, x, W, scale, shift, mean, invstd, k2, k3, slope):
    check_input(gy, x, W, scale, shift, mean, invstd, k2, k3)
    b, ck, n = x.shape
    o = W.shape[0]
    nseg = int(abi.eap_narrow_conv_segments(n))
    partial = torch.empty(b * nseg, o, ck, dtype=torch.float32, device=x.device)
    dW = torch.empty(o, ck, dtype=torch.float32, device=x.device)
    call('eap_narrow_conv_bwd_dw_f32', x, b, o, ck, n, slope, gy, x, W, scale, shift, mean, invstd, k2, k3, partial, dW)
    return dW



def bn_stats_masked(x, b, c, n, na, mask):
    ps, pq = _partials(x, b, c, n)
    call('eap_bn_stats_masked_f32', x, b, c, n, na, x, mask, ps, pq)
    return ps.view(c, b, -1).sum(2, dtype=torch.float64).t(), pq.view(c, b, -1).sum(2, dtype=torch.float64).t()


def bn_act_cloud_fwd(x, b, c, n, scale, shift, slope):
    y = torch.empty_like(x)
    call('eap_bn_act_cloud_fwd_f32', x, b, c, n, slope, x, scale, shift, y)
    return y


def bn_act_cloud_bwd_reduce(gy, x, b, c, n, scale, shift, mean, invstd, slope):
    pg, pgx = _partials(x, b, c, n)
    call('eap_bn_act_cloud_bwd_reduce_f32', x, b, c, n, slope, gy, x, scale, shift, mean, invstd, pg, pgx)
    return pg.view(c, b, -1).sum(2, dtype=torch.float64).t(), pgx.view(c, b, -1).sum(2, dtype=torch.float64).t()


def bn_act_cloud_bwd_apply(gy, x, b, c, n, na, scale, shift, mean, invstd, k2, k3, mask, slope):
    gx = torch.empty_like(x)
    call('eap_bn_act_cloud_bwd_apply_f32', x, b, c, n, na, slope, gy, x, scale, shift, mean, invstd, k2, k3, mask, gx)
    return gx



def _cloud_mean_entries(na):
    return 'eap_bn_act_cloud_mean_wide' if na > 64 else 'eap_bn_act_cloud_mean'


def bn_act_cloud_mean_fwd(x, scale, shift, w, inv_den, slope):
    b, c, p, na = x.shape
    out = torch.empty(b, c, na, dtype=torch.float32, device=x.device)
    call(_cloud_mean_entries(na) + '_fwd_f32', x, b, c, p, na, slope, x, scale, shift, w, inv_den, out)
    return out


def bn_act_cloud_mean_bwd_reduce(g, x, scale, shift, mean, invstd, w, inv_den, slope):
    b, c, p, na = x.shape
    parts = int(getattr(abi, _cloud_mean_entries(na) + '_parts')(p))
    pg = torch.empty(b, c, parts, dtype=torch.float32, device=x.device)
    pgx = torch.empty_like(pg)
    call(_cloud_mean_entries(na) + '_bwd_reduce_f32', x, b, c, p, na, slope, g, x, scale, shift, mean, invstd, w, inv_den, pg, pgx)
    return pg.sum(2, dtype=torch.float64), pgx.sum(2, dtype=torch.float64)


def bn_act_cloud_mean_bwd_apply(g, x, scale, shift, mean, invstd, k2, k3, w, inv_den, stat_mask, slope):
    b, c, p, na = x.shape
    gx = torch.empty_like(x)
    call(_cloud_mean_entries(na) + '_bwd_apply_f32', x, b, c, p, na, slope, g, x, scale, shift, mean, invstd, k2, k3, w, inv_den, stat_mask, gx)
    return gx



def _slot_f32(*tensors):
    check_input(*tensors)
    for t in tensors:
        if t is not None and t.dtype != torch.float32:
            raise RuntimeError(f'slot attention kernels take float32 tensors, not {t.dtype}')


def slot_attn_stats(x, ln_eps):
    _slot_f32(x)
    b, d, n = x.shape
    mean = torch.empty(b, n, dtype=torch.float32, device=x.device)
    rstd = torch.empty_like(mean)
    call('eap_slot_attn_stats_f32', x, b, d, n, ln_eps, x, mean, rstd)
    return mean, rstd


def slot_attn_scores_fwd(x, mean, rstd, u, c0, eps):
    _slot_f32(x, mean, rstd, u, c0)
    (b, d, n), s = x.shape, u.shape[1]
    attn = torch.empty(b, s, n, dtype=torch.float32, device=x.device)
    call('eap_slot_attn_scores_fwd_f32', x, b, s, d, n, eps, x, mean, rstd, u, c0, attn)
    return attn


def slot_attn_pool(x, mean, rstd, w):
    _slot_f32(x, mean, rstd, w)
# ... 56 lines not shown
```

equi-articulated-pose_amd/vgtk/so3conv/functional.py:

```python
import math
import os
import weakref

import numpy as np
import torch

import vgtk
import vgtk.functional as fr
import vgtk.pc as pctk
import vgtk.spconv as zpconv
import vgtk.cuda.grouping as cuda_nn

from .. import _hip
from . import norm_fold

inter_so3conv_feat_grouping = zpconv.inter_zpconv_grouping_naive
batched_index_select = zpconv.batched_index_select
batched_index_select_other = zpconv.batched_index_select_other

MATERIALIZE_INTER_W = False

GAMMA_SIZE = 3
ROOT = vgtk.__path__[0]
Rs, R_idx, canonical_relative = fr.icosahedron_so3(GAMMA_SIZE)
# ... 870 lines not shown
    return torch.empty(feats.shape[0], W.shape[0], grouping.points(feats), feats.shape[3], dtype=feats.dtype, device=feats.device)


def _group_contract(grouping, feats, W, y, slabs, keep, contract):
    x = None
    for b0, b1 in slabs:
        x = grouping.group(feats, b0, b1)
        contract(W, x, y[b0:b1].view(b1 - b0, y.shape[1], -1), b0)
        x = x if keep else None
    return x


def _backward_textbook(grouping, gy, W, feats, x, need_f, need_w, slabs):
    b, c, n, _ = feats.shape
    (o, ck), p, a = W.shape, gy.shape[2], gy.shape[3]
    pa, layout = p * a, grouping.layout
    gF = gW = None
    for b0, b1 in slabs:
        nb = b1 - b0
        gys = gy[b0:b1].view(nb, o, pa)
        if need_w:
            xs = x if x is not None else grouping.group(feats, b0, b1)
            gW = torch.empty_like(W) if gW is None else gW
            if layout == 2:
                _hip.matmul_reduce(gys, xs.view(nb, pa, ck), gW, accumulate=b0 > 0)
            elif layout == 1:
                _hip.gemm_reduce(0, 1, o, ck, pa, gys, pa, o * pa, xs, pa, ck * pa, gW, ck, nb, b_blocked=True)
            else:
                _hip.matmul_reduce(gys, xs.view(nb, ck, pa).transpose(1, 2), gW, accumulate=b0 > 0)
            xs = None
        if need_f:
            gx = torch.empty(nb, ck, pa, dtype=gy.dtype, device=gy.device)
            _hip.matmul(W.t() if gy.dtype == torch.float64 else W.t().contiguous(), gys, gx)
            g = grouping.group_transposed(gx.view(nb, c, grouping.mid, p, a), n, b0, b1)
            del gx
            if nb == b:
                gF = g
            else:
                gF = torch.empty_like(feats) if gF is None else gF
                gF[b0:b1] = g
            del g
    return gF, gW


def _forward_lists(feats, W, args, layout, keep, folded, head, fill):
    b, c, n, na = feats.shape
    ks, mult = args.rk.shape[1], args.mult
    if fill:
        head.fill(args.idx, args.gx, n)
    grouping = _ListGrouping(args, layout)
    y = _empty_output(grouping, feats, W)
    x_bound = _grouped_bound(feats, args.idx) if layout == 2 else None
    tp = (not keep and STORE_ORDER_COLUMNS and layout == 2 and _hip.so3_group_fwd_tp_takes(c, na, ks)
          and (mult is None or (grouping.coset is not None and _hip.so3_group_perm_lists2_takes(c, na, ks, n))))
    grouping.store_order = tp
    Wc = W.index_select(1, _hip.so3_group_fwd_tp_columns(c, ks, W.device)) if tp else W

    def contract(Wc, x, ys, b0):
        _contract_into(Wc, x, ys, layout, folded, b0, x_bound=None if x_bound is None else (x_bound[b0:b0 + x.shape[0]], na, 1.0))
    return y, _group_contract(grouping, feats, Wc, y, _f32_slabs(b, keep), keep, contract)



def _forward_narrow(feats, W, args, train_ep):
    idx, rk = args.idx, args.rk
    b, c, _, na = feats.shape
    p, ks, o = idx.shape[1], rk.shape[1], W.shape[0]
    x = _hip.so3_inter_group_fwd(feats, idx, args.gx, rk, args.mult, args.sigma, args.nonident).view(b, c * ks, p * na)
    if train_ep.takes_partials(x):
        scale, shift, slope = train_ep.moments_from_partials(*_hip.narrow_conv_stats(W, x, partials=True), b * p * na)
    else:
        s1, s2, pivot = _hip.narrow_conv_stats(W, x)
        scale, shift, slope = train_ep.moments(s1, s2, pivot, b * p * na)
    y = _hip.narrow_conv_bnact_fwd(W, x, scale, shift, slope).view(b, o, p, na)
    train_ep.applied = True
    mean, invstd = train_ep.stats
    return y, x, (scale, shift, mean.float(), invstd.float(), train_ep.saved[3], slope, bool(train_ep.norm.sync))


def _native_norm_bwd(gy, count, sync):
    return bool(_hip.NATIVE_NORM_GLUE and gy.is_cuda and isinstance(count, int) and not norm_fold._syncing(sync))


def _backward_narrow(gy, W, x, bn, need_w):
    scale, shift, mean, invstd, count, slope, sync = bn
    b, o = gy.shape[0], gy.shape[1]
    gy = gy.view(b, o, -1)
    if _native_norm_bwd(gy, count, sync):
        g_bn_w, g_bn_b, k2, k3 = _hip.norm_fold_bwd(*_hip.narrow_conv_bwd_reduce(gy, x, W, scale, shift, mean, invstd, slope, partials=True), scale, count)
        return (_hip.narrow_conv_bwd_dw(gy, x, W, scale, shift, mean, invstd, k2, k3, slope) if need_w else None), g_bn_w, g_bn_b
    sg, sgx = _hip.narrow_conv_bwd_reduce(gy, x, W, scale, shift, mean, invstd, slope)
    gW = None
    if need_w:
        k2, k3 = norm_fold.backward_coefficients(scale, sg, sgx, count, True, sync)
        gW = _hip.narrow_conv_bwd_dw(gy, x, W, scale, shift, mean, invstd, k2, k3, slope)
    return gW, sgx.float(), sg.float()



def _weight_operand(W, c, ks, pad_c=None):
    o = W.shape[0]
    W2 = W.view(o, c, ks).permute(1, 0, 2).reshape(c, o * ks).contiguous()
    if pad_c is not None and pad_c != c:
        W2 = torch.cat([W2, torch.zeros(pad_c - c, o * ks, dtype=torch.float32, device=W.device)])
    return W2


def _rows_grad_from_z(z, W2, c, rp, na, ldz, anchor_major, z_bound=None, reorder=None):
    b, (pad_c, oks) = z.shape[0], W2.shape
    gFc = torch.empty(b, pad_c, ldz, dtype=torch.float32, device=z.device)
    _hip.matmul(W2, z.view(b, oks, ldz), gFc, b_bound=z_bound)
    if anchor_major:
        return gFc[:, :c, :rp * na].reshape(b, c, na, rp).transpose(2, 3)
    gFc = gFc.view(b, c, rp, na)
    return gFc if reorder is None else _hip.anchor_reorder(gFc, reorder)


def _weight_grad_rows(z, fc4, o, ks, ldz, anchor_major, reorder=None):
    b, c, rp, na = fc4.shape
    if reorder is not None:
        fc4 = _hip.anchor_reorder(fc4, reorder)
    fc = fc4.transpose(2, 3).contiguous() if anchor_major else fc4
    return _weight_grad_from_z(z, fc.view(b, c, rp * na), b, c, o, ks, rp * na, ldz)



DENSE_TAIL_PACKED = True


def _dense_tail_packed_takes(W, feats, head, geo, c, pad_c, ldz, need_f, need_w):
    na, o, ks, rp = feats.shape[3], W.shape[0], geo.ks, geo.rp
    if not (need_f and need_w and pad_c == c and c % 128 == 0 and rp % 16 == 0 and ldz == _hip.dense_pitch(na * rp) and geo.n_rows is not None
            and head.n_rows is geo.n_rows and feats.is_cuda):
        return False
    return _hip.dense_tail_packed_takes(c, o * ks, na * rp, ldz)


def _dense_tail_packed(z, W, feats, head, geo, colmax, p, ldz, need_f, need_w):
    b, c, n, na = feats.shape
    o, ks, rp = W.shape[0], geo.ks, geo.rp
    ra = na * rp
    words, ncols = _hip.so3_dense_zbound_packed(colmax, head.cnt, head.n_rows, rp, p, ldz)
    zm = z.view(b, o * ks, ldz)
    gFc = torch.empty(b, c, ldz, dtype=torch.float32, device=z.device)
    _hip.matmul_tail(_weight_operand(W, c, ks), zm, gFc, ncols, (words.view(torch.int32), 4, 1.0))
    gF = _hip.rows_scatter_packed(gFc, c, head.rows, head.n_rows, rp, n, na)
    fc = _hip.rows_gather_packed(feats, head.rows, head.n_rows, rp, ldz)
    dt = torch.empty(c, o * ks, dtype=torch.float32, device=z.device)
    _hip.matmul_reduce_tail(fc[..., :ra], zm[..., :ra].transpose(1, 2), dt, ncols)
    return gF, dt.view(c, o, ks).permute(1, 0, 2).reshape(o, c * ks).contiguous()


def _backward_dense(gy, W, feats, head, geo, bn, yact, need_f, need_w):
    b, c, n, na = feats.shape
    o, ks, p, rp = W.shape[0], geo.ks, gy.shape[2], geo.rp
    if BACKWARD_LOG is not None:
        BACKWARD_LOG.append({'channels': (c, o), 'support_rows': n, 'referenced_rows_max': int(rp), 'regime': 'dense rows',
                             **({'norm': 'in the node'} if bn is not None else {})})
    ra = na * rp
    pad_c = 128 if (c == 64 and bn is not None) else c
    ldz = _hip.dense_pitch(ra) if (pad_c % 128 == 0 and (o * ks) % 16 == 0 and need_f) else ra
    gF = gW = g_bn_w = g_bn_b = z_bound = None
    if bn is not None:
        k1, beta, inv_gamma, count, slope, sync = bn
        native = _native_norm_bwd(gy, count, sync)
        if native:
            pg, pgx, gmax, xmax = _hip.bn_act_bwd_reduce_fromy(gy, yact, beta, inv_gamma, slope, partials=True)
            g_bn_w, g_bn_b, _, _, coef, bound, colmax = _hip.norm_fold_bwd(pg, pgx, k1, count, beta, inv_gamma, gmax, xmax)
        else:
            sg, sgx, gmax, xmax = _hip.bn_act_bwd_reduce_fromy(gy, yact, beta, inv_gamma, slope)
            g_bn_w, g_bn_b = sgx.float(), sg.float()
            k2, k3 = norm_fold.backward_coefficients(k1, sg, sgx, count, True, sync)
            coef = torch.stack([k1, k2, k3, beta, inv_gamma]).contiguous()
            bound = (k1.abs()[None, :, None] * gmax + k2.abs()[None, :, None] + k3.abs()[None, :, None] * xmax).contiguous()
        if DENSE_TAIL_PACKED and native and _dense_tail_packed_takes(W, feats, head, geo, c, pad_c, ldz, need_f, need_w):
            z = _hip.so3_dense_bwd_bn(gy, yact, geo, ldz, coef, bound, slope, packed=True)
            return (*_dense_tail_packed(z, W, feats, head, geo, colmax, p, ldz, need_f, need_w), g_bn_w, g_bn_b)
        z = _hip.so3_dense_bwd_bn(gy, yact, geo, ldz, coef, bound, slope)
        if ldz % 4 == 0 and rp % 4 == 0 and native:
            z_bound = (_hip.so3_dense_zbound(colmax, head.cnt, head.n_rows, rp, p, ldz).view(torch.int32), 4, 1.0)
        elif ldz % 4 == 0 and rp % 4 == 0:
            live = torch.arange(rp, device=gy.device)[None, :] < head.n_rows[:, None]
            cntf = torch.where(live, head.cnt[:, :rp], torch.zeros_like(head.cnt[:, :rp])).clamp(min=0, max=p).to(torch.float32)
            cols = bound.amax(1)[:, :, None] * cntf[:, None, :]
            words = torch.zeros(b, ldz // 4, dtype=torch.float32, device=gy.device)
            words[:, :ra // 4] = cols.view(b, na, rp // 4, 4).amax(3).view(b, ra // 4)
            z_bound = (words.view(torch.int32), 4, 1.0)
    else:
        z = _hip.so3_dense_bwd(gy, geo, ldz)
    if need_f:
        gFr = _rows_grad_from_z(z, _weight_operand(W, c, ks, pad_c), c, rp, na, ldz, True, z_bound)
        gF = _hip.rows_scatter(gFr.contiguous(), head.rows, n)
    if need_w:
        gW = _weight_grad_rows(z, _hip.rows_gather(feats, head.rows, rp), o, ks, ldz, True)
    return gF, gW, g_bn_w, g_bn_b


def _backward_dense_parts(gy, W, feats, head, pd, need_f, need_w):
    b, c, n, na = feats.shape
    o, ks, rp = W.shape[0], pd.ks, pd.rp
    ra = na * rp
    if BACKWARD_LOG is not None:
        BACKWARD_LOG.append({'channels': (c, o), 'support_rows': n, 'referenced_rows_max': int(rp), 'regime': 'dense rows', 'parts': pd.parts.n})
    ldz = _hip.dense_pitch(ra) if (c % 128 == 0 and (o * ks) % 16 == 0 and need_f) else ra
    W2 = _weight_operand(W, c, ks) if need_f else None
    fc0 = _hip.rows_gather(feats, head.rows, rp) if need_w else None
    gFr = gW = None
    rowmax = _hip.take_rowmax_hint(gy)
    for i, geo in enumerate(pd.geo):
        perm = pd.perm[i]
        z = _hip.so3_dense_bwd(gy, geo, ldz, colmap=pd.parts.col_map[i], rowmax=rowmax)
        pe = None if perm is None else perm[:, None].expand(b, c, rp, na)
        if need_f:
            t = _rows_grad_from_z(z, W2, c, rp, na, ldz, True)
            if gFr is None:
                gFr = torch.zeros(b, c, rp, na, dtype=torch.float32, device=gy.device)
            if pe is None:
                gFr += t
            else:
                gFr.scatter_add_(3, pe, t.contiguous())
        if need_w:
            gw = _weight_grad_rows(z, fc0 if pe is None else fc0.gather(3, pe), o, ks, ldz, True)
            gW = gw if gW is None else gW + gw
        del z
    gF = _hip.rows_scatter(gFr, head.rows, n) if need_f else None
    return gF, gW


def _backward_lists(gy, W, feats, idx, gx, rk, mult, args, head, rcap, any_nonident, need_f, need_w):
    b, c, n, na = feats.shape
    p, ks, o = idx.shape[1], rk.shape[1], W.shape[0]
    gF = gW = None
    rcap = min((rcap + 3) & ~3, n)
    head.wait()
    rows = head.rows[:, :rcap].contiguous()
    off, cnt = head.off[:, :rcap].contiguous(), head.cnt[:, :rcap].contiguous()
    ent_p, ent_gx = head.entries if head.entries is not None else _hip.inv_lists_fill(idx, gx, head.rows, head.off, rcap)
    multinv = _group_tables_inverse(mult) if (mult is not None and any_nonident) else None
    coset = _coset_tables(multinv, args.ident) if multinv is not None else None
    z_order = z_pos = None
    if coset is not None and _hip.so3_group_perm_lists2_takes(o, na, ks, p):
        z_order, z_pos = coset[0], coset[2]
        ent_pc, ent_gx2 = _hip.so3_perm_entries(ent_p, ent_gx, coset[1], args.anchors, args.ident, na, p)
        z = _hip.so3_inter_group_inv_perm2(_hip.anchor_reorder(gy, z_order), rows, off, cnt, ent_pc, ent_gx2, rk, z_order,
                                           args.sigma, idx.shape[2])
    else:
        z = _hip.so3_inter_group_inv(gy, rows, off, cnt, ent_p, ent_gx, rk, multinv, args.sigma, idx.shape[2],
                                     args.ident, args.anchors, coset)
    if need_f:
        gFr = _rows_grad_from_z(z, _weight_operand(W, c, ks), c, rcap, na, rcap * na, False, reorder=z_pos)
        gF = _hip.rows_scatter(gFr, rows, n)
    if need_w:
        gW = _weight_grad_rows(z, _hip.rows_gather(feats, rows, rcap), o, ks, rcap * na, False, reorder=z_order)
    return gF, gW


class _InterConv(torch.autograd.Function):

    DIFFERENTIABLE = 4

    @staticmethod
    def forward(ctx, feats, W_param, bn_weight, bn_bias, args):
        feats = feats.contiguous()
        W = W_param.contiguous()
        idx, rk, mult, nonident = args.idx, args.rk, args.mult, args.nonident
        can = X_LAYOUT != 'reference' and _hip.so3_inter_group_fwd_can_block(
            feats.shape[1], feats.shape[2], feats.shape[3], rk.shape[1], mult is not None, nonident is not None)
        layout = 0 if not can else (2 if X_LAYOUT == 'transposed' else 1)
        _, c, n, na = feats.shape
        p, ks, o = idx.shape[1], rk.shape[1], W.shape[0]
        needs_grad = (ctx.needs_input_grad[0] or ctx.needs_input_grad[1]) and args.grad_mode
        train_ep = args.epilogue if isinstance(args.epilogue, TrainEpilogue) else None
        folded = None if train_ep is not None else args.epilogue
        if folded is not None and (needs_grad or not folded.inference):
            raise RuntimeError('a folded epilogue is an inference-time fusion: build and use it under torch.no_grad()')
        if args.amap is not None or args.shift is not None:
            grouping, keep = _MapGrouping(args), bool(needs_grad and ctx.needs_input_grad[1])
            if FORWARD_LOG is not None:
                FORWARD_LOG.append({'channels': (c, o), 'dense': False, 'parts': None, 'regime': grouping.regime})
            y = _empty_output(grouping, feats, W)
            x = _group_contract(grouping, feats, W, y, _f32_slabs(feats.shape[0], keep), keep,
                                lambda W, x, ys, b0: _contract_into(W, x, ys, 0, folded, b0))
            ctx.bn, ctx.conv_args, ctx.head, ctx.layout, ctx.plan = None, args, None, 0, None
            ctx.W_param = weakref.ref(W_param)
            ctx.save_for_backward(W, x, idx, args.gx, rk, None, nonident, feats, None)
            return y
        narrow = c * ks <= _hip.NARROW_CONV_MAX_CK and not ctx.needs_input_grad[0]
        if narrow and train_ep is not None and FUSE_CONV_NORM and _hip.narrow_conv_takes(o, c * ks, p * na):
            if FORWARD_LOG is not None:
                FORWARD_LOG.append({'channels': (c, o), 'dense': False, 'parts': None, 'regime': 'narrow input'})
            y, x, bn = _forward_narrow(feats, W, args, train_ep)
            wanted = args.grad_mode and any(ctx.needs_input_grad[1:_InterConv.DIFFERENTIABLE])
            ctx.bn, ctx.conv_args, ctx.head, ctx.layout, ctx.plan = (bn if wanted else None), args, None, 0, None
            ctx.narrow = True
            ctx.W_param = weakref.ref(W_param)
            ctx.save_for_backward(W, x if wanted else None, idx, None, rk, None, None, feats, None)
            return y
        lists_ok = BACKWARD_MODE != 'dx' and _inv_lists_supported(idx, n, na, ks) and not narrow
        keep = needs_grad and (not lists_ok or _keep_x_hint(W_param))
        plan = _DensePlan(args, n, o, lists_ok, needs_grad, keep, folded, train_ep.norm if (train_ep is not None and FUSE_CONV_NORM) else None)
        head = plan.head if needs_grad else None
        if FORWARD_LOG is not None:
            FORWARD_LOG.append({'channels': (c, o), 'dense': bool(plan.forward), 'parts': None if plan.parts is None else plan.parts.n})
        if plan.forward:
            bn_only = args.grad_mode and not needs_grad and (ctx.needs_input_grad[2] or ctx.needs_input_grad[3])
            join = FUSE_CONV_NORM and not bn_only and train_ep is not None and not plan.head.norm_ill()
            y, ctx.bn = _forward_dense(feats, W, plan, p, train_ep if join else None, folded)
            x, layout = None, 0
# ... 671 lines not shown
```

include/eap_hip.h:

```cpp
#ifndef EAP_HIP_H
#define EAP_HIP_H

#include <stdint.h>

#ifdef __cplusplus
extern "C" {
#endif

typedef void *eap_stream_t;

const char *eap_last_error(void);
int eap_launch_dims_ok(int64_t gx, int64_t gy, int64_t gz, int bx, int by, int bz);
const char *eap_last_kernel(void);
int eap_abi_version(void);


int eap_ball_query_f32(int b, int n, int m, float radius, int nsample, const float *new_xyz,
                       const float *xyz, int32_t *idx, eap_stream_t stream);
int eap_ball_query_f64(int b, int n, int m, float radius, int nsample, const double *new_xyz,
                       const double *xyz, int32_t *idx, eap_stream_t stream);

int eap_furthest_point_sampling_f32(int b, int n, int m, const float *xyz, float *temp,
                                    int32_t *idx, eap_stream_t stream);
int eap_furthest_point_sampling_f64(int b, int n, int m, const double *xyz, double *temp,
// ... 107 lines not shown
                                const float *rk, const uint8_t *mult, float *gfeats,
                                eap_stream_t stream);

int64_t eap_so3_inter_group_bwd_workspace(int b, int c, int p, int n, int na);
int eap_so3_inter_group_bwd_slab_f32(int b, int c, int p, int n, int nn, int na, int ks, float sigma,
                                     const float *gout, const int32_t *idx, const float *gx,
                                     const float *rk, const uint8_t *mult, int identity_anchor,
                                     float *gfeats, float *workspace, eap_stream_t stream);


int eap_so3_anchor_map_f32(int b, int p, int n, int nn, int na, const int32_t *idx, const float *q_pose,
                           const float *s_pose, const float *anchors, uint8_t *amap, int32_t *nontrivial,
                           eap_stream_t stream);

int eap_so3_inter_group_fwd_map_f32(int b, int c, int p, int n, int nn, int na, int ks, float sigma,
                                    const float *feats, const int32_t *idx, const float *gx, const float *rk,
                                    const uint8_t *amap, float *out, eap_stream_t stream);

int64_t eap_so3_inter_group_bwd_map_workspace(int b, int c, int p, int n, int na);
int eap_so3_inter_group_bwd_map_f32(int b, int c, int p, int n, int nn, int na, int ks, float sigma,
                                    const float *gout, const int32_t *idx, const float *gx, const float *rk,
                                    const uint8_t *amap, float *gfeats, float *workspace, eap_stream_t stream);


int eap_so3_residual_index_f32(int b, int p, int n, int nn, const int32_t *idx, const float *q_pose,
                               const float *s_pose, const float *res, uint8_t *shift, int32_t *nontrivial,
                               eap_stream_t stream);

int eap_so3_inter_group_fwd_res_f32(int b, int c, int p, int n, int nn, int na, int ks, float sigma,
                                    const float *feats, const int32_t *idx, const float *gx, const float *rk,
                                    const uint8_t *shift, float *out, eap_stream_t stream);

int64_t eap_so3_inter_group_bwd_res_workspace(int b, int c, int p, int n, int na);
int eap_so3_inter_group_bwd_res_f32(int b, int c, int p, int n, int nn, int na, int ks, float sigma,
                                    const float *gout, const int32_t *idx, const float *gx, const float *rk,
                                    const uint8_t *shift, float *gfeats, float *workspace, eap_stream_t stream);

int eap_so3_group_lists_tiles(int tiles);
int eap_so3_group_lists_store16(int on);
int eap_so3_group_perm_lists2(int on);
int eap_so3_group_perm_lists2_takes(int channels, int na, int ks, int n_support);
int eap_so3_perm_entries_f32(int b, int per_cloud, int na, int n_support, const int32_t *ent_p, const float *ent_gx, const uint8_t *code,
                             const float *anchors, int identity_anchor, const int32_t *nonident, int32_t *ent_pc, float *ent_gx2,
                             eap_stream_t stream);
int eap_so3_inter_group_fwd_perm2_t_f32(int b, int c, int p, int n, int nn, int na, int ks, float sigma, const float *feats,
                                        const float *feats_c, const int32_t *idx, const float *gx, const int32_t *ent_pc,
                                        const float *ent_gx2, const float *rk, const uint8_t *order, const int32_t *nonident,
                                        int store_order_columns, float *out, eap_stream_t stream);
int eap_so3_group_fwd_tp_takes(int c, int na, int ks);
int eap_so3_group_fwd_tp_columns(int c, int ks, int32_t *perm);
int eap_so3_inter_group_fwd_tp_f32(int b, int c, int p, int n, int nn, int na, int ks, float sigma, const float *feats,
                                   const int32_t *idx, const float *gx, const float *rk, float *out, eap_stream_t stream);
int eap_so3_inter_group_inv_perm2_f32(int b, int o, int p, int nn, int na, int ks, int rcap, float sigma, const float *gy,
                                      const int32_t *rows, const int32_t *off, const int32_t *cnt, const int32_t *ent_pc,
                                      const float *ent_gx2, const float *rk, const uint8_t *order, float *z, eap_stream_t stream);

int eap_so3_inter_group_inv_f32(int b, int o, int p, int nn, int na, int ks, int rcap, float sigma,
                                const float *gy, const int32_t *rows, const int32_t *off,
                                const int32_t *cnt, const int32_t *ent_p, const float *ent_gx,
                                const float *rk, const uint8_t *multinv, const float *anchors,
                                int identity_anchor, float *z, eap_stream_t stream);
int eap_anchor_reorder_f32(int64_t rows, int na, const float *src, const uint8_t *order, float *dst, eap_stream_t stream);
int eap_anchor_reorder_clouds_f32(int b, int64_t rows_per_cloud, int na, const float *src, const uint8_t *order,
                                  const int32_t *nonident, float *dst, eap_stream_t stream);
int eap_so3_inter_group_inv_coset_f32(int b, int o, int p, int nn, int na, int ks, int rcap, float sigma,
                                      const float *gy, const int32_t *rows, const int32_t *off, const int32_t *cnt,
                                      const int32_t *ent_p, const float *ent_gx, const float *rk, const uint8_t *multinv,
                                      const float *anchors, int identity_anchor, const uint8_t *coset_order,
                                      const uint8_t *coset_code, float *z, eap_stream_t stream);

int eap_inv_lists_rows(int b, int p, int n, int nn, const int32_t *idx, int32_t *counts, int32_t *rows,
                       int32_t *off, int32_t *cnt, int32_t *n_rows, eap_stream_t stream);
int eap_inv_lists_fill(int b, int p, int n, int nn, int rcap, const int32_t *idx, const float *gx,
                       const int32_t *rows, const int32_t *off, int32_t *ent_p, float *ent_gx,
                       eap_stream_t stream);
int eap_rows_gather_f32(int b, int c, int n, int na, int rcap, int rows_ld, const int32_t *rows,
                        const float *src, float *dst, eap_stream_t stream);
int eap_rows_scatter_f32(int b, int c, int n, int na, int rcap, int rows_ld, const int32_t *rows,
                         const float *src, float *dst, eap_stream_t stream);
int eap_rows_gather_packed_f32(int b, int c, int n, int na, int rp, int rows_ld, int64_t ld, const int32_t *rows, const int32_t *n_rows,
                               const float *src, float *dst, eap_stream_t stream);
int eap_rows_scatter_packed_f32(int b, int c, int c_ld, int n, int na, int rp, int rows_ld, int64_t ld, const int32_t *rows,
                                const int32_t *n_rows, const float *src, float *dst, eap_stream_t stream);

int eap_so3_dense_supported(int p, int na, int ks, int rp, int o);
int eap_so3_dense_member(int b, int p, int n, int nn, int rp, int rows_ld, const int32_t *idx, const int32_t *rows,
                         const int32_t *n_rows, int32_t *slot_of, uint32_t *memb, int32_t *flags, eap_stream_t stream);
int64_t eap_so3_dense_mask_words(int b, int p, int ks, int rp, int dir);
int eap_so3_dense_masks(int b, int p, int ks, int rp, int dir, const uint32_t *memb, uint64_t *mask, eap_stream_t stream);
int eap_so3_dense_tables_f32(int b, int p, int n, int na, int ks, int rp, int rows_ld, float sigma, const float *q_xyz,
                             const float *s_xyz, const int32_t *rows, const float *rk, const float *row_rot, float *centre, float *pt,
                             float *kr, eap_stream_t stream);
int eap_so3_dense_split_f32(int b, int m, int l, int na, int seg, int64_t seg_pitch, int mapped, const int32_t *n_rows, const uint32_t *rowmax,
                            const int32_t *colmap, const float *src, float *scale, void *planes, eap_stream_t stream);
int eap_so3_dense_product_f32(int dir, int b, int o, int p, int na, int ks, int rp, int64_t ldz, float sigma, const int32_t *n_rows, const void *planes,
                              const float *scale,
                              const float *pt, const float *kr, const uint64_t *mask, float *out, eap_stream_t stream);
int eap_so3_dense_untranspose_f32(int b, int o, int p, int na, const float *yt, float *y, float *psum, float *psq, eap_stream_t stream);
int eap_so3_dense_untranspose_map_f32(int b, int o, int p, int na, int p_dst, const int32_t *map, const float *yt, float *y,
                                      eap_stream_t stream);
int eap_so3_dense_untranspose_map_stats_f32(int b, int o, int p, int na, int p_dst, const int32_t *map, const int32_t *pivot_pos, const float *yt,
                                            float *y, float *psum, float *psq, eap_stream_t stream);
int eap_so3_dense_split_bn_f32(int b, int m, int l, int l_src, int na, const uint32_t *rowbound, const int32_t *colmap, const float *grad,
                               const float *act, const float *coef, float slope, float *scale, void *planes, eap_stream_t stream);
int eap_so3_dense_untranspose_bnact_f32(int b, int o, int p, int na, int p_dst, const int32_t *map, const float *yt, const float *bn_scale,
                                        const float *bn_shift, float slope, float *y, eap_stream_t stream);
int eap_so3_dense_gplanes_supported(int o, int c, int na, int ks, int rp);
int eap_so3_dense_gplanes_f32(int b, int o, int c, int na, int ks, int rp, const float *W3, const float *Ft, const int32_t *n_rows,
                              const float *bound, float *scale, void *planes, eap_stream_t stream);
int eap_so3_dense_point_keys(int b, int p, const uint32_t *memb, int32_t *keys, eap_stream_t stream);
int64_t eap_so3_dense_steps_words(int b, int p, int ks, int rp, int dir);
int eap_so3_dense_steps(int b, int p, int ks, int rp, int dir, int skip, const int32_t *n_rows, const uint64_t *mask, int32_t *steps,
                        eap_stream_t stream);
int eap_so3_dense_product_steps_f32(int dir, int b, int o, int p, int na, int ks, int rp, int64_t ldz, float sigma, const int32_t *n_rows,
                                    const void *planes, const float *scale, const float *pt, const float *kr, const uint64_t *mask,
                                    const int32_t *steps, float *out, eap_stream_t stream);
int eap_so3_dense_product_packed_f32(int b, int o, int p, int na, int ks, int rp, int64_t ldz, float sigma, const int32_t *n_rows,
                                     const void *planes, const float *scale, const float *pt, const float *kr, const uint64_t *mask,
                                     const int32_t *steps, float *out, eap_stream_t stream);
int eap_so3_dense_live16(int n_rows, int rp);
int eap_so3_dense_max_rows(void);
int eap_so3_dense_member_wide(int b, int p, int n, int nn, int rp, int rows_ld, const int32_t *idx, const int32_t *rows,
                              const int32_t *n_rows, int32_t *slot_of, uint32_t *memb, int32_t *flags, eap_stream_t stream);
int eap_so3_dense_point_keys_wide(int b, int p, const uint32_t *memb, int64_t *keys, eap_stream_t stream);
int eap_so3_dense_masks_wide(int b, int p, int ks, int rp, int dir, const uint32_t *memb, uint64_t *mask, eap_stream_t stream);
int eap_so3_dense_steps_wide(int b, int p, int ks, int rp, int dir, int skip, const int32_t *n_rows, const uint64_t *mask, int32_t *steps,
                             eap_stream_t stream);
int64_t eap_so3_dense_probe_workspace(int b);
int eap_so3_dense_probe(int b, int p, int words, const int32_t *n_rows, const int32_t *nonident, const int32_t *dflags,
                        const uint32_t *memb, const float *rot_a, int64_t blocks_a, const float *rot_b, int64_t blocks_b,
                        const float *rot_cloud, const float *norm_w, const float *norm_b, int channels, float ratio,
                        int32_t *work, int32_t *out, eap_stream_t stream);


int eap_so3_intra_group_fwd_f32(int b, int c, int p, int na, int t, const float *feats,
                                const int32_t *intra_idx, float *out, eap_stream_t stream);
int eap_so3_intra_group_bwd_f32(int b, int c, int p, int na, int t, const float *gout,
                                const int32_t *intra_idx, float *gfeats, eap_stream_t stream);



int eap_gemm_f32(int transA, int transB, int M, int N, int K, const float *A, int64_t lda,
                 int64_t strideA, const float *B, int64_t ldb, int64_t strideB, float *C,
                 int64_t ldc, int64_t strideC, int batch, eap_stream_t stream);

int64_t eap_gemm_f32_reduce_workspace(int M, int N, int K, int batch);
int eap_gemm_f32_reduce(int transA, int transB, int M, int N, int K, const float *A, int64_t lda,
                        int64_t strideA, const float *B, int64_t ldb, int64_t strideB, float *C,
                        int64_t ldc, int batch, float *workspace, eap_stream_t stream);

int eap_gemm_bf16x3_f32_supported(int M, int N, int K, const float *A, int64_t lda, const float *B, int64_t ldb,
                                  int64_t strideB);
int eap_gemm_bf16x3_f32(int M, int N, int K, const float *A, int64_t lda, const float *B, int64_t ldb, int64_t strideB,
                        float *C, int64_t ldc, int64_t strideC, int batch, eap_stream_t stream);
int eap_gemm_bf16x3_presplit(int on);
int eap_gemm_bf16x3_nn_f32_supported(int M, int N, int K, const float *A, int64_t lda, const float *B, int64_t ldb,
                                     int64_t strideB);
int eap_gemm_bf16x3_nn_f32(int M, int N, int K, const float *A, int64_t lda, const float *B, int64_t ldb, int64_t strideB,
                           float *C, int64_t ldc, int64_t strideC, int batch, eap_stream_t stream);
int eap_gemm_bf16x3_ep_f32(int transB, int M, int N, int K, const float *A, int64_t lda, const float *B, int64_t ldb, int64_t strideB,
                           float *C, int64_t ldc, int64_t strideC, int batch, const float *scale, const float *shift, float slope,
                           const float *residual, int64_t strideRes, eap_stream_t stream);
int eap_gemm_bf16x3_reduce_f32_supported(int M, int N, int K, const float *A, int64_t lda, int64_t strideA, const float *B,
                                         int64_t ldb, int64_t strideB, int64_t ldc);
int64_t eap_gemm_bf16x3_reduce_workspace(int M, int N, int K, int batch);
int eap_gemm_bf16x3_reduce_f32(int M, int N, int K, const float *A, int64_t lda, int64_t strideA, const float *B, int64_t ldb,
                               int64_t strideB, float *C, int64_t ldc, int batch, float *workspace, eap_stream_t stream);
int eap_gemm_bf16x3_reduce_tail_f32(int M, int N, int K, const float *A, int64_t lda, int64_t strideA, const float *B, int64_t ldb,
                                    int64_t strideB, float *C, int64_t ldc, int batch, const int32_t *ncols, float *workspace,
                                    eap_stream_t stream);
int eap_so3_intra_conv_bf16x3_f32_supported(int b, int o, int c, int p, int na, int nt);
int eap_so3_intra_conv_bf16x3_f32(int b, int o, int c, int p, int na, int nt, const float *W, const float *feats,
                                  const int32_t *intra_idx, float *out, eap_stream_t stream);
int eap_absmax_rows_f32(const float *x, int batch, int rows, int cols, int64_t ld, int64_t stride, int32_t *out_bits, eap_stream_t stream);
int eap_absmax_colgroups_f32(const float *x, int batch, int rows, int cols, int64_t ld, int64_t stride, int grp, int32_t *out_bits,
                             eap_stream_t stream);
int eap_so3_grouped_bound_f32(int b, int p, int nn, int n_sup, const int32_t *point_max_bits, const int32_t *idx, int32_t *out_bits,
                              eap_stream_t stream);
int eap_gemm_f16x2_f32(int trans_b, int M, int N, int K, const float *A, int64_t lda, const float *B, int64_t ldb, int64_t strideB,
                       float *C, int64_t ldc, int64_t strideC, int batch, const int32_t *abs_a, const int32_t *abs_b, int grp_b, float mult_b,
                       const float *scale, const float *shift, float slope, const float *residual, int64_t strideRes,
                       eap_stream_t stream);
int eap_gemm_f16x2_splitk_slabs(int M, int N, int K, int batch, int cus);
int64_t eap_gemm_f16x2_splitk_workspace(int M, int N, int batch, int slabs);
int eap_gemm_f16x2_splitk_f32(int M, int N, int K, const float *A, int64_t lda, const float *B, int64_t ldb, int64_t strideB,
                              float *C, int64_t ldc, int64_t strideC, int batch, const int32_t *abs_a, const int32_t *abs_b, int grp_b,
                              float mult_b, int slabs, float *workspace, int64_t workspace_floats, eap_stream_t stream);
// ... 19 lines not shown
int64_t eap_gemm_skinny_reduce_workspace(int M, int N, int K, int batch);
int eap_gemm_skinny_reduce_f32(int M, int N, int K, const float *A, int64_t lda, int64_t strideA, const float *B, int64_t ldb,
                               int64_t strideB, float *C, int64_t ldc, int batch, float *workspace, eap_stream_t stream);

int eap_so3_inter_group_fwd_can_block(int c, int n, int na, int ks, int has_mult, int has_flag);
int eap_so3_inter_group_fwd_xb_f32(int b, int c, int p, int n, int nn, int na, int ks, float sigma,
                                   const float *feats, const int32_t *idx, const float *gx,
                                   const float *rk, const uint8_t *mult, const int32_t *nonident,
                                   float *out, eap_stream_t stream);
int eap_so3_inter_group_fwd_t_f32(int b, int c, int p, int n, int nn, int na, int ks, float sigma,
                                  const float *feats, const int32_t *idx, const float *gx,
                                  const float *rk, const uint8_t *mult, const int32_t *nonident,
                                  float *out, eap_stream_t stream);
int eap_gemm_f32_xb(int transA, int transB, int M, int N, int K, const float *A, int64_t lda,
                    int64_t strideA, const float *B, int64_t b_block_rows, int64_t strideB, float *C,
                    int64_t ldc, int64_t strideC, int batch, eap_stream_t stream);
int eap_gemm_f32_reduce_xb(int transA, int transB, int M, int N, int K, const float *A, int64_t lda,
                           int64_t strideA, const float *B, int64_t b_block_rows, int64_t strideB,
                           float *C, int64_t ldc, int batch, float *workspace, eap_stream_t stream);

int eap_so3_intra_conv_f32(int b, int o, int c, int p, int na, int nt, const float *W, const float *feats,
                           const int32_t *intra_idx, float *out, eap_stream_t stream);


int eap_so3_intra_group2d_fwd_f32(int b, int c, int p, int na, int nr, int t, const float *feats, const int32_t *intra_idx, float *out,
                                  eap_stream_t stream);
int eap_so3_intra_group2d_bwd_f32(int b, int c, int p, int na, int nr, int t, const float *gout, const int32_t *intra_idx, float *gfeats,
                                  eap_stream_t stream);
int eap_so3_intra_conv2d_f32(int b, int o, int c, int p, int na, int nr, int nt, const float *W, const float *feats,
                             const int32_t *intra_idx, float *out, eap_stream_t stream);
int eap_so3_intra_conv2d_split_supported(int b, int o, int c, int p, int na, int nr, int nt);
int eap_so3_intra_conv2d_bf16x3_f32(int b, int o, int c, int p, int na, int nr, int nt, const float *W, const float *feats,
                                    const int32_t *intra_idx, float *out, eap_stream_t stream);
int eap_so3_intra_conv2d_f16x2_f32(int b, int o, int c, int p, int na, int nr, int nt, const float *W, const float *feats,
                                   const int32_t *intra_idx, float *out, const int32_t *abs_w, const int32_t *abs_f, eap_stream_t stream);


int eap_chamfer_fwd_f32(int b, int n, int m, const float *xyz1, const float *xyz2, float *dist1,
                        float *dist2, int32_t *idx1, int32_t *idx2, eap_stream_t stream);
int eap_chamfer_fwd_f64(int b, int n, int m, const double *xyz1, const double *xyz2, double *dist1,
                        double *dist2, int32_t *idx1, int32_t *idx2, eap_stream_t stream);
int eap_chamfer_bwd_f32(int b, int n, int m, const float *xyz1, const float *xyz2,
                        const int32_t *idx1, const int32_t *idx2, const float *g1, const float *g2,
                        float *gxyz1, float *gxyz2, eap_stream_t stream);
int eap_chamfer_bwd_ordered_f32(int b, int n, int m, const float *xyz1, const float *xyz2,
                                const int32_t *idx1, const int32_t *idx2, const float *g1, const float *g2,
                                float *gxyz1, float *gxyz2, eap_stream_t stream);
int eap_chamfer_bwd_ordered_f64(int b, int n, int m, const double *xyz1, const double *xyz2,
                                const int32_t *idx1, const int32_t *idx2, const double *g1, const double *g2,
                                double *gxyz1, double *gxyz2, eap_stream_t stream);

int eap_orbit_chamfer_fwd_f32(int g, int s, int a, int m, int n, const float *recon, const float *ori, const uint8_t *member,
                              float *r2o_all, int32_t *r2o_all_idx, float *r2o_in, int32_t *r2o_in_idx, float *o2r_all,
                              int32_t *o2r_idx, float *o2r_in, eap_stream_t stream);
int eap_orbit_chamfer_fwd_f64(int g, int s, int a, int m, int n, const double *recon, const double *ori, const uint8_t *member,
                              double *r2o_all, int32_t *r2o_all_idx, double *r2o_in, int32_t *r2o_in_idx, double *o2r_all,
                              int32_t *o2r_idx, double *o2r_in, eap_stream_t stream);
int eap_orbit_chamfer_bwd_f32(int g, int s, int a, int m, int n, const float *recon, const float *ori, const uint8_t *member,
                              const int32_t *r2o_all_idx, const int32_t *r2o_in_idx, const int32_t *o2r_idx, const float *g_r2o_all,
                              const float *g_r2o_in, const float *g_o2r_all, const float *g_o2r_in, float *grecon, eap_stream_t stream);
int eap_orbit_chamfer_bwd_f64(int g, int s, int a, int m, int n, const double *recon, const double *ori, const uint8_t *member,
                              const int32_t *r2o_all_idx, const int32_t *r2o_in_idx, const int32_t *o2r_idx, const double *g_r2o_all,
                              const double *g_r2o_in, const double *g_o2r_all, const double *g_o2r_in, double *grecon, eap_stream_t stream);

int eap_bn_act_segments(int64_t n);
int eap_bn_stats_f32(int b, int c, int64_t n, const float *x, float *psum, float *psq, eap_stream_t stream);
int eap_bn_act_fwd_f32(int b, int c, int64_t n, float slope, const float *x, const float *scale,
                       const float *shift, float *y, eap_stream_t stream);
int eap_bn_act_add_fwd_f32(int b, int c, int64_t n, float slope, const float *x, const float *scale,
                           const float *shift, const float *res, float *y, eap_stream_t stream);
int eap_bn_act_bwd_reduce_f32(int b, int c, int64_t n, float slope, const float *gy, const float *x,
                              const float *scale, const float *shift, const float *mean,
                              const float *invstd, float *pg, float *pgx, eap_stream_t stream);
int eap_bn_act_bwd_apply_f32(int b, int c, int64_t n, float slope, const float *gy, const float *x,
                             const float *scale, const float *shift, const float *mean,
                             const float *invstd, const float *k2, const float *k3, float *gx,
                             eap_stream_t stream);
int eap_bn_act_bwd_apply_rowmax_f32(int b, int c, int64_t n, int na, float slope, const float *gy, const float *x,
                                    const float *scale, const float *shift, const float *mean, const float *invstd,
                                    const float *k2, const float *k3, float *gx, uint32_t *rowmax, eap_stream_t stream);
int eap_bn_act_fromy_blocks(int64_t n, int na);
int eap_bn_act_bwd_reduce_fromy_f32(int b, int c, int64_t n, int na, float slope, const float *gy, const float *y, const float *beta,
                                    const float *inv_gamma, float *pg, float *pgx, uint32_t *gmax, uint32_t *xmax, eap_stream_t stream);

int eap_bn_stats_masked_f32(int b, int c, int64_t n, int na, const float *x, const float *mask, float *psum, float *psq,
                            eap_stream_t stream);
int eap_bn_act_cloud_fwd_f32(int b, int c, int64_t n, float slope, const float *x, const float *scale, const float *shift,
                             float *y, eap_stream_t stream);
int eap_bn_act_cloud_bwd_reduce_f32(int b, int c, int64_t n, float slope, const float *gy, const float *x, const float *scale,
                                    const float *shift, const float *mean, const float *invstd, float *pg, float *pgx,
                                    eap_stream_t stream);
int eap_bn_act_cloud_bwd_apply_f32(int b, int c, int64_t n, int na, float slope, const float *gy, const float *x,
                                   const float *scale, const float *shift, const float *mean, const float *invstd,
                                   const float *k2, const float *k3, const float *mask, float *gx, eap_stream_t stream);

int eap_narrow_contract_supported(int b, int o, int c, int64_t n);
int eap_narrow_contract_fwd_f32(int b, int o, int c, int64_t n, const float *W, const float *x, float *y, eap_stream_t stream);
int eap_narrow_contract_dx_f32(int b, int o, int c, int64_t n, const float *W, const float *g, float *dx, eap_stream_t stream);
int eap_narrow_contract_dw_slabs(int64_t n);
int eap_narrow_contract_dw_f32(int b, int o, int c, int64_t n, const float *g, const float *x, float *partial, eap_stream_t stream);

int eap_narrow_conv_segments(int64_t n);
int eap_narrow_conv_stats_f32(int b, int o, int ck, int64_t n, const float *W, const float *x, float *pivot, float *psum, float *psq,
                              eap_stream_t stream);
int eap_narrow_conv_bnact_fwd_f32(int b, int o, int ck, int64_t n, float slope, const float *W, const float *x, const float *scale,
                                  const float *shift, float *y, eap_stream_t stream);
int eap_narrow_conv_bwd_reduce_f32(int b, int o, int ck, int64_t n, float slope, const float *gy, const float *x, const float *W,
                                   const float *scale, const float *shift, const float *mean, const float *invstd, float *pg, float *pgx,
                                   eap_stream_t stream);
int eap_narrow_conv_bwd_dw_f32(int b, int o, int ck, int64_t n, float slope, const float *gy, const float *x, const float *W,
                               const float *scale, const float *shift, const float *mean, const float *invstd, const float *k2,
                               const float *k3, float *partial, float *dW, eap_stream_t stream);

int eap_norm_fold_train_f32(int o, int parts, int64_t pivot_stride, int64_t count, int64_t eps_bits, int64_t momentum_bits, const float *ps,
                            const float *pq, const float *pivot, const float *gamma, const float *beta, float *running_mean, float *running_var,
                            float *scale, float *shift, double *mean, double *invstd, float *beta_copy, float *inv_gamma, eap_stream_t stream);
int eap_norm_fold_bwd_f32(int o, int parts, int b, int na, int64_t count, const float *pg, const float *pgx, const float *k1, const float *beta,
                          const float *inv_gamma, const float *gmax, const float *xmax, float *dgamma, float *dbeta, float *k2, float *k3, float *coef,
                          float *bound, float *colmax, eap_stream_t stream);
int eap_so3_dense_zbound_f32(int b, int na, int rp, int p, int ldz, int64_t cnt_stride, const float *colmax, const int32_t *cnt,
                             const int32_t *n_rows, float *words, eap_stream_t stream);
int eap_so3_dense_zbound_packed_f32(int b, int na, int rp, int p, int ldz, int64_t cnt_stride, const float *colmax, const int32_t *cnt,
                                    const int32_t *n_rows, float *words, int32_t *ncols, eap_stream_t stream);
int eap_so3_dense_gplanes_bound_f32(int b, int o, int c, int na, int ks, int rp, const float *W3, const float *fc4, float *fpart, float *wsum,
                                    float *bound, eap_stream_t stream);
int eap_so3_dense_point_order(int b, int p, int words, const int64_t *order, const uint32_t *memb, const float *q_xyz, int32_t *order32,
                              uint32_t *memb_out, float *xyz_out, int32_t *pivot_pos, eap_stream_t stream);

int eap_anchor_attn_pool_fwd_f32(int b, int c, int n, int na, float temperature, const float *x, const float *logits,
                                 float *out, float *conf, eap_stream_t stream);
int eap_anchor_attn_pool_bwd_f32(int b, int c, int n, int na, float temperature, const float *x, const float *logits,
                                 const float *g, float *dx, float *dlogits, eap_stream_t stream);
int eap_slot_masked_mean_fwd_f32(int b, int ns, int c, int n, int na, const float *x, const float *mask,
                                 const float *inv_den, float *out, eap_stream_t stream);
int eap_slot_masked_mean_bwd_f32(int b, int ns, int c, int n, int na, const float *g, const float *mask,
                                 const float *inv_den, float *dx, eap_stream_t stream);
int eap_masked_max_fwd_f32(int b, int c, int n, int na, const float *x, const float *mask, float *out, int32_t *arg,
                           eap_stream_t stream);
int eap_masked_max_bwd_f32(int b, int c, int n, int na, const float *g, const int32_t *arg, const float *mask, float *dx,
                           eap_stream_t stream);
int eap_anchor_attn_pool_wide_fwd_f32(int b, int c, int n, int na, float temperature, const float *x, const float *logits,
                                      float *out, float *conf, eap_stream_t stream);
int eap_anchor_attn_pool_wide_bwd_f32(int b, int c, int n, int na, float temperature, const float *x, const float *logits,
                                      const float *g, float *dx, float *dlogits, eap_stream_t stream);
int eap_slot_masked_mean_wide_fwd_f32(int b, int ns, int c, int n, int na, const float *x, const float *mask,
                                      const float *inv_den, float *out, eap_stream_t stream);
int eap_slot_masked_mean_wide_bwd_f32(int b, int ns, int c, int n, int na, const float *g, const float *mask,
                                      const float *inv_den, float *dx, eap_stream_t stream);
int eap_masked_max_wide_fwd_f32(int b, int c, int n, int na, const float *x, const float *mask, float *out, int32_t *arg,
                                eap_stream_t stream);
int eap_masked_max_wide_bwd_f32(int b, int c, int n, int na, const float *g, const int32_t *arg, const float *mask, float *dx,
                                eap_stream_t stream);
int eap_bn_act_cloud_mean_fwd_f32(int b, int c, int n, int na, float slope, const float *x, const float *scale, const float *shift,
                                  const float *w, const float *inv_den, float *out, eap_stream_t stream);
int eap_bn_act_cloud_mean_parts(int n);
int eap_bn_act_cloud_mean_bwd_reduce_f32(int b, int c, int n, int na, float slope, const float *g, const float *x, const float *scale,
                                         const float *shift, const float *mean, const float *invstd, const float *w, const float *inv_den,
                                         float *pg, float *pgx, eap_stream_t stream);
int eap_bn_act_cloud_mean_bwd_apply_f32(int b, int c, int n, int na, float slope, const float *g, const float *x, const float *scale,
                                        const float *shift, const float *mean, const float *invstd, const float *k2, const float *k3,
                                        const float *w, const float *inv_den, const float *stat_mask, float *gx, eap_stream_t stream);
int eap_bn_act_cloud_mean_wide_fwd_f32(int b, int c, int n, int na, float slope, const float *x, const float *scale, const float *shift,
                                       const float *w, const float *inv_den, float *out, eap_stream_t stream);
int eap_bn_act_cloud_mean_wide_parts(int n);
int eap_bn_act_cloud_mean_wide_bwd_reduce_f32(int b, int c, int n, int na, float slope, const float *g, const float *x, const float *scale,
                                              const float *shift, const float *mean, const float *invstd, const float *w, const float *inv_den,
                                              float *pg, float *pgx, eap_stream_t stream);
int eap_bn_act_cloud_mean_wide_bwd_apply_f32(int b, int c, int n, int na, float slope, const float *g, const float *x, const float *scale,
                                             const float *shift, const float *mean, const float *invstd, const float *k2, const float *k3,
                                             const float *w, const float *inv_den, const float *stat_mask, float *gx, eap_stream_t stream);

int eap_slot_attn_stats_f32(int b, int d, int n, float ln_eps, const float *x, float *mean, float *rstd, eap_stream_t stream);
int eap_slot_attn_scores_fwd_f32(int b, int s, int d, int n, float eps, const float *x, const float *mean, const float *rstd, const float *u,
                                 const float *c0, float *attn, eap_stream_t stream);
int eap_slot_attn_pool_parts(int n);
int eap_slot_attn_pool_f32(int b, int s, int d, int n, const float *x, const float *mean, const float *rstd, const float *w, float *psum,
                           eap_stream_t stream);
int eap_slot_attn_scores_bwd_f32(int b, int s, int d, int n, float eps, const float *x, const float *mean, const float *rstd, const float *attn,
                                 const float *gmsum, const float *gwsum, const float *gattn, float *gdots, eap_stream_t stream);
int eap_slot_attn_input_grad_f32(int b, int j, int d, int n, const float *x, const float *mean, const float *rstd, const float *rows,
                                 const float *vecs, float *gx, eap_stream_t stream);

int eap_pointnet_max_parts(int n);
int eap_pointnet_max_fwd_f32(int b, int c, int o, int n, int na, const float *feats, const float *xyz, const float *centre, const float *member,
                             const float *wt, const float *v, const float *bias, float *pval, int32_t *parg, float *out, int32_t *arg,
                             eap_stream_t stream);
int eap_pointnet_max_bwd_data_f32(int b, int c, int o, int n, int na, const float *g, const int32_t *arg, const float *w, int ldw, float *dfeats,
                                  float *dcoords, eap_stream_t stream);
int eap_pointnet_max_bwd_weight_f32(int b, int c, int o, int n, int na, const float *g, const int32_t *arg, const float *feats, const float *xyz,
                                    const float *centre, const float *anchors, float *dwp, eap_stream_t stream);

int eap_so3_prep_f64(int b, int p, int n, int nn, int na, const double *q_xyz, const double *s_xyz, const int32_t *idx,
                     const double *q_pose, const double *s_pose, const double *anchors, int identity_anchor, double *g, int32_t *r,
                     int32_t *nonident, eap_stream_t stream);
int eap_so3_inter_weights_f64(int b, int p, int nn, int na, int ks, int64_t sigma_bits, const double *g, const double *rk, double *w,
// ... 26 lines not shown
```

Before: 173.1 point-clouds/sec.

## Skip reading zero gradient rows in BN backward via a listed-points bitmask

After a rows_scatter writes a gradient that is nonzero only at the listed (subsampled) points, the code leaves a hint, and the backward BN/conv reductions build a per-cloud bitmask of those points. The kernels then skip global loads of gy for unlisted points or whole tiles, substituting zeros. This is meant to cut memory traffic in the backward reduce, dW and dense-BN kernels. In exchange it adds a bitmask build kernel, a memset, extra bit tests per load, and relies on the scattered gradient being zero outside the listed rows.

```diff
diff --git a/equi-articulated-pose_amd/csrc/bn_act.hip b/equi-articulated-pose_amd/csrc/bn_act.hip
--- a/equi-articulated-pose_amd/csrc/bn_act.hip
+++ b/equi-articulated-pose_amd/csrc/bn_act.hip
@@ -202,13 +202,17 @@
     }
 }
 
+template <bool LISTED>
 __global__ __launch_bounds__(256) void bn_act_bwd_reduce_fromy_kernel(int c, long n4, int nq, int nblk, float slope, float inv_slope, const float4 *__restrict__ gy,
                                                                       const float4 *__restrict__ y, const float *__restrict__ beta,
                                                                       const float *__restrict__ inv_gamma, float *__restrict__ pg, float *__restrict__ pgx,
-                                                                      unsigned *__restrict__ gmax, unsigned *__restrict__ xmax) {
+                                                                      unsigned *__restrict__ gmax, unsigned *__restrict__ xmax,
+                                                                      const unsigned *__restrict__ listed, int lwords) {
     __shared__ unsigned s_max[256][8];
     const int ci = blockIdx.y, bi = blockIdx.z, t = threadIdx.x;
     const int T = nq * (256 / nq);
+    const unsigned *lrow = LISTED ? listed + (size_t)bi * lwords : nullptr;
+    const long pt0 = (long)blockIdx.x * RM_PIECES * (T / nq) + t / nq;
     const float be = beta[ci], ig = inv_gamma[ci];
     const size_t r0 = ((size_t)bi * c + ci) * (size_t)n4;
     const long base = (long)blockIdx.x * RM_PIECES * T;
@@ -219,7 +223,15 @@
 #pragma unroll
         for (int v = 0; v < RM_PIECES; ++v) {
             const long i = base + (long)v * T + t;
-            if (i < n4) { g[v] = gy[r0 + i]; a[v] = y[r0 + i]; }
+            if (i < n4) {
+                a[v] = y[r0 + i];
+                if (LISTED) {
+                    const long pt = pt0 + (long)v * (T / nq);
+                    g[v] = ((lrow[pt >> 5] >> (pt & 31)) & 1u) ? gy[r0 + i] : make_float4(0.f, 0.f, 0.f, 0.f);
+                } else {
+                    g[v] = gy[r0 + i];
+                }
+            }
         }
 #pragma unroll
         for (int v = 0; v < RM_PIECES; ++v) {
@@ -324,18 +336,41 @@
     return (int)((n4 + (long)RM_PIECES * T - 1) / ((long)RM_PIECES * T));
 }
 
-extern "C" int eap_bn_act_bwd_reduce_fromy_f32(int b, int c, int64_t n, int na, float slope, const float *gy, const float *y, const float *beta,
-                                               const float *inv_gamma, float *pg, float *pgx, uint32_t *gmax, uint32_t *xmax, eap_stream_t stream) {
-    if (b <= 0 || c <= 0 || n <= 0) return 0;
+namespace {
+int reduce_fromy(const char *who, int b, int c, int64_t n, int na, float slope, const float *gy, const float *y, const float *beta, const float *inv_gamma,
+                 const uint32_t *listed, float *pg, float *pgx, uint32_t *gmax, uint32_t *xmax, eap_stream_t stream) {
+    char buf[256];
     if (na <= 0 || (na & 3) != 0 || na > 256 || n % na != 0 || !(slope > 0.f) ||
-        ((reinterpret_cast<uintptr_t>(gy) | reinterpret_cast<uintptr_t>(y)) & 15) != 0)
-        return eap::bad_arg("bn_act_bwd_reduce_fromy: rows of [points][na], na a multiple of 4 up to 256, 16-byte aligned tensors, a positive slope");
+        ((reinterpret_cast<uintptr_t>(gy) | reinterpret_cast<uintptr_t>(y)) & 15) != 0) {
+        snprintf(buf, sizeof(buf), "%s: rows of [points][na], na a multiple of 4 up to 256, 16-byte aligned tensors, a positive slope", who);
+        return eap::bad_arg(buf);
+    }
+    if (n / na >= (1ll << 31)) {
+        snprintf(buf, sizeof(buf), "%s: fewer than 2^31 points per row", who);
+        return eap::bad_arg(buf);
+    }
     hipStream_t s = eap::S(stream);
     if (int e = eap::hip_fail(hipMemsetAsync(gmax, 0, sizeof(uint32_t) * (size_t)b * c * na, s), "bn_act_bwd_reduce_fromy memset")) return e;
     if (int e = eap::hip_fail(hipMemsetAsync(xmax, 0, sizeof(uint32_t) * (size_t)b * c * na, s), "bn_act_bwd_reduce_fromy memset")) return e;
-    const int nq = na / 4, nblk = eap_bn_act_fromy_blocks(n, na);
-    return eap::run_kernel("bn_act_bwd_reduce_fromy", bn_act_bwd_reduce_fromy_kernel, nblk, c, b, dim3(256), 0, s, c, (long)(n / 4), nq, nblk, slope,
-                           1.0f / slope, reinterpret_cast<const float4 *>(gy), reinterpret_cast<const float4 *>(y), beta, inv_gamma, pg, pgx, gmax, xmax);
+    const int nq = na / 4, nblk = eap_bn_act_fromy_blocks(n, na), lwords = (int)((n / na + 31) / 32);
+    auto kernel = listed ? bn_act_bwd_reduce_fromy_kernel<true> : bn_act_bwd_reduce_fromy_kernel<false>;
+    return eap::run_kernel(who, kernel, nblk, c, b, dim3(256), 0, s, c, (long)(n / 4), nq, nblk, slope, 1.0f / slope, reinterpret_cast<const float4 *>(gy),
+                           reinterpret_cast<const float4 *>(y), beta, inv_gamma, pg, pgx, gmax, xmax, listed, lwords);
+}
+}
+
+extern "C" int eap_bn_act_bwd_reduce_fromy_f32(int b, int c, int64_t n, int na, float slope, const float *gy, const float *y, const float *beta,
+                                               const float *inv_gamma, float *pg, float *pgx, uint32_t *gmax, uint32_t *xmax, eap_stream_t stream) {
+    if (b <= 0 || c <= 0 || n <= 0) return 0;
+    return reduce_fromy("bn_act_bwd_reduce_fromy", b, c, n, na, slope, gy, y, beta, inv_gamma, nullptr, pg, pgx, gmax, xmax, stream);
+}
+
+extern "C" int eap_bn_act_bwd_reduce_fromy_listed_f32(int b, int c, int64_t n, int na, float slope, const float *gy, const float *y, const float *beta,
+                                                      const float *inv_gamma, const uint32_t *listed, float *pg, float *pgx, uint32_t *gmax,
+                                                      uint32_t *xmax, eap_stream_t stream) {
+    if (!gy || !y || !beta || !inv_gamma || !listed || !pg || !pgx || !gmax || !xmax) return eap::bad_arg("bn_act_bwd_reduce_fromy_listed: null pointer");
+    if (b <= 0 || c <= 0 || n <= 0) return 0;
+    return reduce_fromy("bn_act_bwd_reduce_fromy_listed", b, c, n, na, slope, gy, y, beta, inv_gamma, listed, pg, pgx, gmax, xmax, stream);
 }
 
 namespace {
diff --git a/equi-articulated-pose_amd/csrc/inv_lists.hip b/equi-articulated-pose_amd/csrc/inv_lists.hip
--- a/equi-articulated-pose_amd/csrc/inv_lists.hip
+++ b/equi-articulated-pose_amd/csrc/inv_lists.hip
@@ -205,6 +205,14 @@
     }
 }
 
+__global__ __launch_bounds__(256) void rows_bitmask_kernel(int n, int rp, int rld, int words, const int32_t *__restrict__ rows,
+                                                           const int32_t *__restrict__ n_rows, unsigned *__restrict__ mask) {
+    const int bi = blockIdx.y, r = blockIdx.x * 256 + threadIdx.x;
+    if (r >= rp || (n_rows != nullptr && r >= n_rows[bi])) return;
+    const int q = rows[(size_t)bi * rld + r];
+    if (q >= 0 && q < n) atomicOr(mask + (size_t)bi * words + (q >> 5), 1u << (q & 31));
+}
+
 }
 
 extern "C" int eap_inv_lists_rows(int b, int p, int n, int nn, const int32_t *idx, int32_t *counts, int32_t *rows,
@@ -274,3 +282,16 @@
     return eap::run_kernel("rows_scatter_packed", rows_scatter_packed_kernel, eap::cdiv(rp, PACKED_SLOTS), c, b, dim3(256), 0, s, c, c_ld, n, na, rp, rows_ld,
                            (long long)ld, rows, n_rows, src, dst);
 }
+
+extern "C" int eap_rows_bitmask_words(int n) { return n > 0 ? (n + 31) / 32 : 0; }
+
+extern "C" int eap_rows_bitmask(int b, int n, int rp, int rows_ld, const int32_t *rows, const int32_t *n_rows, uint32_t *mask, eap_stream_t stream) {
+    if (!rows || !mask) return eap::bad_arg("rows_bitmask: null pointer");
+    if (b <= 0 || n <= 0 || rp <= 0) return eap::bad_arg("rows_bitmask: every size must be positive");
+    if (rp % 16 != 0 || rows_ld < rp) return eap::bad_arg("rows_bitmask: rp a multiple of 16, the row stride of rows >= rp");
+    if (b > 65535) return eap::bad_arg("rows_bitmask: at most 65535 clouds");
+    hipStream_t s = eap::S(stream);
+    const int words = eap_rows_bitmask_words(n);
+    if (int e = eap::hip_fail(hipMemsetAsync(mask, 0, sizeof(uint32_t) * (size_t)b * words, s), "rows_bitmask memset")) return e;
+    return eap::run_kernel("rows_bitmask", rows_bitmask_kernel, eap::cdiv(rp, 256), b, 1, dim3(256), 0, s, n, rp, rows_ld, words, rows, n_rows, mask);
+}
diff --git a/equi-articulated-pose_amd/csrc/narrow_conv.hip b/equi-articulated-pose_amd/csrc/narrow_conv.hip
--- a/equi-articulated-pose_amd/csrc/narrow_conv.hip
+++ b/equi-articulated-pose_amd/csrc/narrow_conv.hip
@@ -77,6 +77,20 @@
         xoff = 4u * ((unsigned)h * (unsigned)n + 4u * li);
     }
 };
+
+struct Listed { const unsigned *bits; int lwords, na; };
+__device__ __forceinline__ bool listed_any(const Listed &ls, int bi, long col0, long end) {
+    const unsigned *row = ls.bits + (size_t)bi * ls.lwords;
+    const int lo = (int)((unsigned)col0 / (unsigned)ls.na), hi = (int)((unsigned)(min(col0 + TILE, end) - 1) / (unsigned)ls.na);
+    unsigned any = 0;
+    for (int w = lo >> 5; w <= hi >> 5; ++w) {
+        unsigned v = row[w];
+        if (w == lo >> 5) v &= ~0u << (lo & 31);
+        if (w == hi >> 5) v &= ~0u >> (31 - (hi & 31));
+        any |= v;
+    }
+    return __builtin_amdgcn_readfirstlane(any) != 0;
+}
 
 template <int KS2>
 __global__ __launch_bounds__(NT) void narrow_conv_stats_kernel(int ct, int ck, long n, int nseg, const float *__restrict__ W,
@@ -163,13 +177,13 @@
     }
 }
 
-template <int KS2>
+template <int KS2, bool LISTED>
 __global__ __launch_bounds__(NT) void narrow_conv_bwd_reduce_kernel(int ct, int o, int ck, long n, int nseg, float slope,
                                                                       const float *__restrict__ gy, const float *__restrict__ x,
                                                                       const float *__restrict__ W, const float *__restrict__ scale,
                                                                       const float *__restrict__ shift, const float *__restrict__ mean,
                                                                       const float *__restrict__ invstd, float *__restrict__ pg,
-                                                                      float *__restrict__ pgx) {
+                                                                      float *__restrict__ pgx, Listed ls) {
     __shared__ __attribute__((aligned(16))) float s_sc[64], s_sh[64], s_mu[64], s_is[64];
     __shared__ float s_red[WAVES][2][32];
     const Pos w(ct, n);
@@ -193,12 +207,14 @@
         load_x<KS2>(xa, xb, n, col0, w.xoff, ok, ck, h);
         f32x16 d[4];
         conv_tile<KS2, false>(d, xa, wf);
+        const bool some = !LISTED || listed_any(ls, w.bi, col0, w.end);
         if (ok) {
 #pragma unroll
             for (int g = 0; g < 4; ++g) {
                 f32x4 gv[4];
 #pragma unroll
-                for (int q = 0; q < 4; ++q) gv[q] = ld_off<f32x4>(gb + (size_t)(8 * g) * n + col0, roff + 4u * q * (unsigned)n);
+                for (int q = 0; q < 4; ++q)
+                    gv[q] = some ? ld_off<f32x4>(gb + (size_t)(8 * g) * n + col0, roff + 4u * q * (unsigned)n) : (f32x4){0.f, 0.f, 0.f, 0.f};
                 const f32x4 sc = *reinterpret_cast<const f32x4 *>(&s_sc[lc + 8 * g + 4 * h]), sh = *reinterpret_cast<const f32x4 *>(&s_sh[lc + 8 * g + 4 * h]);
                 const f32x4 mu = *reinterpret_cast<const f32x4 *>(&s_mu[lc + 8 * g + 4 * h]), is = *reinterpret_cast<const f32x4 *>(&s_is[lc + 8 * g + 4 * h]);
 #pragma unroll
@@ -217,13 +233,13 @@
     block_sums(sa, qa, s_red, ct, o0, w.bi, gridDim.z, nseg, w.seg, pg, pgx);
 }
 
-template <int KS2>
+template <int KS2, bool LISTED>
 __global__ __launch_bounds__(NT) void narrow_conv_bwd_dw_kernel(int ct, int o, int ck, long n, int nseg, float slope,
                                                                   const float *__restrict__ gy, const float *__restrict__ x,
                                                                   const float *__restrict__ W, const float *__restrict__ scale,
                                                                   const float *__restrict__ shift, const float *__restrict__ mean,
                                                                   const float *__restrict__ invstd, const float *__restrict__ k2,
-                                                                  const float *__restrict__ k3, float *__restrict__ partial) {
+                                                                  const float *__restrict__ k3, float *__restrict__ partial, Listed ls) {
     __shared__ float s_part[WAVES][16][64];
     const Pos w(ct, n);
     const int h = w.h, li = w.li, wave = threadIdx.x >> 6;
@@ -245,6 +261,7 @@
         load_x<KS2>(xa, xb, n, col0, w.xoff, col < n, ck, h);
         f32x16 d[4];
         conv_tile<KS2, true>(d, xa, wf);
+        const bool some = !LISTED || listed_any(ls, w.bi, col0, w.end);
 #pragma unroll
         for (int g = 0; g < 4; ++g) {
             f32x4 gv[4], xv[4];
@@ -252,7 +269,7 @@
             for (int q = 0; q < 4; ++q) {
                 const long cq = col0 + 4 * (8 * g + 4 * h + q);
                 const bool in = cq < n;
-                gv[q] = in ? ld_off<f32x4>(gb + col0 + 4 * (8 * g + q), goff) : zero4;
+                gv[q] = (in && some) ? ld_off<f32x4>(gb + col0 + 4 * (8 * g + q), goff) : zero4;
                 xv[q] = (in && li < ck) ? ld_off<f32x4>(xb + col0 + 4 * (8 * g + q), koff) : zero4;
             }
 #pragma unroll
@@ -341,30 +358,70 @@
     });
 }
 
-extern "C" int eap_narrow_conv_bwd_reduce_f32(int b, int o, int ck, int64_t n, float slope, const float *gy, const float *x, const float *W,
-                                              const float *scale, const float *shift, const float *mean, const float *invstd, float *pg,
-                                              float *pgx, eap_stream_t stream) {
-    if (int e = refuse("narrow_conv_bwd_reduce", o, ck, (long)n, x, gy)) return e;
+namespace {
+int bwd_reduce(const char *who, int b, int o, int ck, long n, float slope, const float *gy, const float *x, const float *W, const float *scale,
+               const float *shift, const float *mean, const float *invstd, float *pg, float *pgx, Listed ls, eap_stream_t stream) {
+    if (int e = refuse(who, o, ck, n, x, gy)) return e;
     if (b <= 0 || n <= 0) return 0;
-    const int nseg = nseg_of((long)n), ct = tiles_per_block(o);
+    const int nseg = nseg_of(n), ct = tiles_per_block(o);
     return by_depth(ck, [&](auto ks2) {
-        return eap::run_kernel("narrow_conv_bwd_reduce", narrow_conv_bwd_reduce_kernel<decltype(ks2)::value>, nseg, o / (32 * ct), b, dim3(NT), 0, eap::S(stream),
-                               ct, o, ck, (long)n, nseg, slope, gy, x, W, scale, shift, mean, invstd, pg, pgx);
+        constexpr int K = decltype(ks2)::value;
+        return eap::run_kernel(who, ls.bits ? narrow_conv_bwd_reduce_kernel<K, true> : narrow_conv_bwd_reduce_kernel<K, false>, nseg, o / (32 * ct), b, dim3(NT), 0,
+                               eap::S(stream), ct, o, ck, n, nseg, slope, gy, x, W, scale, shift, mean, invstd, pg, pgx, ls);
     });
 }
 
-extern "C" int eap_narrow_conv_bwd_dw_f32(int b, int o, int ck, int64_t n, float slope, const float *gy, const float *x, const float *W,
-                                          const float *scale, const float *shift, const float *mean, const float *invstd, const float *k2,
-                                          const float *k3, float *partial, float *dW, eap_stream_t stream) {
-    if (int e = refuse("narrow_conv_bwd_dw", o, ck, (long)n, x, gy)) return e;
+int bwd_dw(const char *who, int b, int o, int ck, long n, float slope, const float *gy, const float *x, const float *W, const float *scale,
+           const float *shift, const float *mean, const float *invstd, const float *k2, const float *k3, float *partial, float *dW, Listed ls,
+           eap_stream_t stream) {
+    if (int e = refuse(who, o, ck, n, x, gy)) return e;
     if (b <= 0 || n <= 0) return 0;
-    const int nseg = nseg_of((long)n), ct = tiles_per_block(o);
+    const int nseg = nseg_of(n), ct = tiles_per_block(o);
     hipStream_t s = eap::S(stream);
     int e = by_depth(ck, [&](auto ks2) {
-        return eap::run_kernel("narrow_conv_bwd_dw", narrow_conv_bwd_dw_kernel<decltype(ks2)::value>, nseg, o / (32 * ct), b, dim3(NT), 0, s, ct, o, ck, (long)n,
-                               nseg, slope, gy, x, W, scale, shift, mean, invstd, k2, k3, partial);
+        constexpr int K = decltype(ks2)::value;
+        return eap::run_kernel(who, ls.bits ? narrow_conv_bwd_dw_kernel<K, true> : narrow_conv_bwd_dw_kernel<K, false>, nseg, o / (32 * ct), b, dim3(NT), 0, s, ct, o, ck,
+                               n, nseg, slope, gy, x, W, scale, shift, mean, invstd, k2, k3, partial, ls);
     });
     if (e) return e;
     const int mn = o * ck;
     return eap::run_kernel("narrow_conv_bwd_dw (sum)", narrow_conv_dw_sum_kernel, eap::cdiv(mn, 4), 1, 1, dim3(256), 0, s, mn, b * nseg, partial, dW);
 }
+
+int refuse_listed(const char *who, long n, int na, const void *listed) {
+    char buf[200];
+    if (listed != nullptr && na > 0 && (na & 3) == 0 && n % na == 0) return 0;
+    snprintf(buf, sizeof(buf), "%s: takes the mask of listed points (not null) and rows of [points][na], na a multiple of 4", who);
+    return eap::bad_arg(buf);
+}
+}
+
+extern "C" int eap_narrow_conv_bwd_reduce_f32(int b, int o, int ck, int64_t n, float slope, const float *gy, const float *x, const float *W,
+                                              const float *scale, const float *shift, const float *mean, const float *invstd, float *pg,
+                                              float *pgx, eap_stream_t stream) {
+    return bwd_reduce("narrow_conv_bwd_reduce", b, o, ck, (long)n, slope, gy, x, W, scale, shift, mean, invstd, pg, pgx, Listed{nullptr, 0, 1}, stream);
+}
+
+extern "C" int eap_narrow_conv_bwd_reduce_listed_f32(int b, int o, int ck, int64_t n, int na, float slope, const float *gy, const float *x, const float *W,
+                                                     const float *scale, const float *shift, const float *mean, const float *invstd,
+                                                     const uint32_t *listed, float *pg, float *pgx, eap_stream_t stream) {
+    if (!gy || !x || !W || !scale || !shift || !mean || !invstd || !pg || !pgx) return eap::bad_arg("narrow_conv_bwd_reduce_listed: null pointer");
+    if (int e = refuse_listed("narrow_conv_bwd_reduce_listed", (long)n, na, listed)) return e;
+    return bwd_reduce("narrow_conv_bwd_reduce_listed", b, o, ck, (long)n, slope, gy, x, W, scale, shift, mean, invstd, pg, pgx,
+                      Listed{listed, (int)((n / na + 31) / 32), na}, stream);
+}
+
+extern "C" int eap_narrow_conv_bwd_dw_f32(int b, int o, int ck, int64_t n, float slope, const float *gy, const float *x, const float *W,
+                                          const float *scale, const float *shift, const float *mean, const float *invstd, const float *k2,
+                                          const float *k3, float *partial, float *dW, eap_stream_t stream) {
+    return bwd_dw("narrow_conv_bwd_dw", b, o, ck, (long)n, slope, gy, x, W, scale, shift, mean, invstd, k2, k3, partial, dW, Listed{nullptr, 0, 1}, stream);
+}
+
+extern "C" int eap_narrow_conv_bwd_dw_listed_f32(int b, int o, int ck, int64_t n, int na, float slope, const float *gy, const float *x, const float *W,
+                                                 const float *scale, const float *shift, const float *mean, const float *invstd, const float *k2,
+                                                 const float *k3, const uint32_t *listed, float *partial, float *dW, eap_stream_t stream) {
+    if (!gy || !x || !W || !scale || !shift || !mean || !invstd || !k2 || !k3 || !partial || !dW) return eap::bad_arg("narrow_conv_bwd_dw_listed: null pointer");
+    if (int e = refuse_listed("narrow_conv_bwd_dw_listed", (long)n, na, listed)) return e;
+    return bwd_dw("narrow_conv_bwd_dw_listed", b, o, ck, (long)n, slope, gy, x, W, scale, shift, mean, invstd, k2, k3, partial, dW,
+                  Listed{listed, (int)((n / na + 31) / 32), na}, stream);
+}
diff --git a/equi-articulated-pose_amd/csrc/so3_dense.hip b/equi-articulated-pose_amd/csrc/so3_dense.hip
--- a/equi-articulated-pose_amd/csrc/so3_dense.hip
+++ b/equi-articulated-pose_amd/csrc/so3_dense.hip
@@ -279,8 +279,8 @@
     scale2[i] = sc;
 }
 
-struct SplitBn { const f32x4 *Y2; const float *coef; float slope, inv_slope; };
-template <bool BN>
+struct SplitBn { const f32x4 *Y2; const float *coef; float slope, inv_slope; const unsigned *listed; int lwords; };
+template <bool BN, bool LISTED = false>
 __global__ __launch_bounds__(256) __attribute__((amdgpu_waves_per_eu(2, 2))) void dense_split_kernel(int m, int l, int na, int kb_total, int seg, long long seg_pitch4, int mapped,
                                                           const int32_t *__restrict__ n_rows, const int32_t *__restrict__ colmap,
                                                           const f32x4 *__restrict__ T, const float *__restrict__ scale2,
@@ -297,6 +297,7 @@
     const int l0 = 16 * kb + 8 * kg;
     unsigned at[8], keep[8];
     int live = 0;
+    unsigned gbits = 255u;
     if (colmap != nullptr) {
         int ci[8] = {-1, -1, -1, -1, -1, -1, -1, -1};
         if (l0 < l) {
@@ -305,6 +306,13 @@
         }
 #pragma unroll
         for (int e = 0; e < 8; ++e) { keep[e] = ci[e] >= 0 ? ~0u : 0u; at[e] = (unsigned)max(ci[e], 0) * (unsigned)nq; live |= (int)(keep[e] & 1u) << e; }
+        if constexpr (LISTED) {
+            const unsigned *lrow = bn.listed + (size_t)b * bn.lwords;
+            gbits = 0;
+#pragma unroll
+            for (int e = 0; e < 8; ++e)
+                if (ci[e] >= 0) gbits |= ((lrow[ci[e] >> 5] >> (ci[e] & 31)) & 1u) << e;
+        }
     } else {
         int sg = l0 / seg, sr = l0 - sg * seg;
         if (mapped) dense_kr(l0, nseg, sg, sr);
@@ -317,6 +325,7 @@
         }
 #pragma unroll
         for (int e = 1; e < 8; ++e) at[e] = keep[e] ? at[e] : at[0];
+        if constexpr (LISTED) gbits = l0 < l ? (bn.listed[(size_t)b * bn.lwords + (l0 >> 5)] >> (l0 & 31)) & 255u : 0u;
     }
     if (live == 0)
         for (int i = t; i < 64 * na; i += 256) image[i] = (u32x4){0u, 0u, 0u, 0u};
@@ -330,7 +339,10 @@
             rowv[u] = row;
             const size_t row_off = ((size_t)b * m + row) * (colmap ? (size_t)1 : (size_t)nseg) * seg_pitch4 + aq;
 #pragma unroll
-            for (int e = 0; e < 8; ++e) q[u][e] = T[row_off + at[e]];
+            for (int e = 0; e < 8; ++e) {
+                if (!LISTED || ((gbits >> e) & 1u)) q[u][e] = T[row_off + at[e]];
+                else q[u][e] = (f32x4){0.f, 0.f, 0.f, 0.f};
+            }
             if constexpr (BN) {
 #pragma unroll
                 for (int e = 0; e < 8; ++e) q2[u][e] = bn.Y2[row_off + at[e]];
@@ -987,27 +999,45 @@
                                         reinterpret_cast<const f32x4 *>(src), scale, scale2);
     if (e) return e;
     return eap::run_kernel("so3_dense_split", dense_split_kernel<false>, (long long)kb_total * (m / 32) * b * 2, 1, 1, dim3(256), (size_t)na * 1024, s, m, l, na, kb_total, seg, (long long)(seg_pitch / 4),
-                           mapped ? 1 : 0, n_rows, colmap, reinterpret_cast<const f32x4 *>(src), scale2, reinterpret_cast<u32x4 *>(planes), SplitBn{nullptr, nullptr, 1.f, 1.f});
+                           mapped ? 1 : 0, n_rows, colmap, reinterpret_cast<const f32x4 *>(src), scale2, reinterpret_cast<u32x4 *>(planes), SplitBn{nullptr, nullptr, 1.f, 1.f, nullptr, 0});
+}
+
+namespace {
+int split_bn(const char *who, int b, int m, int l, int l_src, int na, const uint32_t *rowbound, const int32_t *colmap, const float *grad, const float *act,
+             const float *coef, const uint32_t *listed, float slope, float *scale, void *planes, eap_stream_t stream) {
+    char buf[320];
+    if (colmap == nullptr && l != l_src) { snprintf(buf, sizeof(buf), "%s: without a column map l = l_src", who); return eap::bad_arg(buf); }
+    if ((m % 32) != 0 || (na % 4) != 0 || na > 64 || ((reinterpret_cast<uintptr_t>(grad) | reinterpret_cast<uintptr_t>(act)) & 15) ||
+        (colmap != nullptr && ((l & 7) != 0 || (reinterpret_cast<uintptr_t>(colmap) & 15) != 0)) || rowbound == nullptr || coef == nullptr || !(slope > 0.f)) {
+        snprintf(buf, sizeof(buf), "%s: m %% 32, na %% 4, na <= 64, 16-byte aligned sources, a bound per row, a positive slope (column map: 16-byte aligned, l %% 8)", who);
+        return eap::bad_arg(buf);
+    }
+    if ((int64_t)l_src * na / 4 > 0x7fffffffLL) { snprintf(buf, sizeof(buf), "%s: a source row of at most 2^31 16-byte pieces", who); return eap::bad_arg(buf); }
+    hipStream_t s = eap::S(stream);
+    const int kb_total = ceil_to(l, KC_BK) / 16;
+    float *scale2 = scale + (size_t)b * na * m;
+    if (int e = eap::run_kernel(who, dense_scale_kernel, eap::cdiv((long long)b * m * na, 256), 1, 1, dim3(256), 0, s, (long long)b * m * na, m, na, rowbound, scale,
+                                scale2))
+        return e;
+    const int seg = colmap ? l : l_src;
+    return eap::run_kernel(who, listed ? dense_split_kernel<true, true> : dense_split_kernel<true, false>, (long long)kb_total * (m / 32) * b * 2, 1, 1, dim3(256), (size_t)na * 1024, s, m, l, na, kb_total, seg,
+                           (long long)l_src * na / 4, 0, nullptr, colmap, reinterpret_cast<const f32x4 *>(grad), scale2, reinterpret_cast<u32x4 *>(planes),
+                           SplitBn{reinterpret_cast<const f32x4 *>(act), coef, slope, 1.0f / slope, listed, (l_src + 31) / 32});
+}
 }
 
 extern "C" int eap_so3_dense_split_bn_f32(int b, int m, int l, int l_src, int na, const uint32_t *rowbound, const int32_t *colmap, const float *grad,
                                           const float *act, const float *coef, float slope, float *scale, void *planes, eap_stream_t stream) {
     if (b <= 0) return 0;
-    if (colmap == nullptr && l != l_src) return eap::bad_arg("so3_dense_split_bn: without a column map l = l_src");
-    if ((m % 32) != 0 || (na % 4) != 0 || na > 64 || ((reinterpret_cast<uintptr_t>(grad) | reinterpret_cast<uintptr_t>(act)) & 15) ||
-        (colmap != nullptr && ((l & 7) != 0 || (reinterpret_cast<uintptr_t>(colmap) & 15) != 0)) || rowbound == nullptr || coef == nullptr || !(slope > 0.f))
-        return eap::bad_arg("so3_dense_split_bn: m % 32, na % 4, na <= 64, 16-byte aligned sources, a bound per row, a positive slope (column map: 16-byte aligned, l % 8)");
-    if ((int64_t)l_src * na / 4 > 0x7fffffffLL) return eap::bad_arg("so3_dense_split_bn: a source row of at most 2^31 16-byte pieces");
-    hipStream_t s = eap::S(stream);
-    const int kb_total = ceil_to(l, KC_BK) / 16;
-    float *scale2 = scale + (size_t)b * na * m;
-    if (int e = eap::run_kernel("so3_dense_split_bn", dense_scale_kernel, eap::cdiv((long long)b * m * na, 256), 1, 1, dim3(256), 0, s, (long long)b * m * na, m, na, rowbound, scale,
-                                scale2))
-        return e;
-    const int seg = colmap ? l : l_src;
-    return eap::run_kernel("so3_dense_split_bn", dense_split_kernel<true>, (long long)kb_total * (m / 32) * b * 2, 1, 1, dim3(256), (size_t)na * 1024, s, m, l, na, kb_total, seg,
-                           (long long)l_src * na / 4, 0, nullptr, colmap, reinterpret_cast<const f32x4 *>(grad), scale2, reinterpret_cast<u32x4 *>(planes),
-                           SplitBn{reinterpret_cast<const f32x4 *>(act), coef, slope, 1.0f / slope});
+    return split_bn("so3_dense_split_bn", b, m, l, l_src, na, rowbound, colmap, grad, act, coef, nullptr, slope, scale, planes, stream);
+}
+
+extern "C" int eap_so3_dense_split_bn_listed_f32(int b, int m, int l, int l_src, int na, const uint32_t *rowbound, const int32_t *colmap, const float *grad,
+                                                 const float *act, const float *coef, const uint32_t *listed, float slope, float *scale, void *planes,
+                                                 eap_stream_t stream) {
+    if (!rowbound || !grad || !act || !coef || !listed || !scale || !planes) return eap::bad_arg("so3_dense_split_bn_listed: null pointer");
+    if (b <= 0) return 0;
+    return split_bn("so3_dense_split_bn_listed", b, m, l, l_src, na, rowbound, colmap, grad, act, coef, listed, slope, scale, planes, stream);
 }
 
 namespace {
diff --git a/equi-articulated-pose_amd/vgtk/_hip.py b/equi-articulated-pose_amd/vgtk/_hip.py
--- a/equi-articulated-pose_amd/vgtk/_hip.py
+++ b/equi-articulated-pose_amd/vgtk/_hip.py
@@ -1205,7 +1205,7 @@
     return y
 
 
-def bn_act_bwd_reduce_fromy(gy, y, beta, inv_gamma, slope, partials=False):
+def bn_act_bwd_reduce_fromy(gy, y, beta, inv_gamma, slope, partials=False, listed=None):
     b, c, p, na = y.shape
     n = p * na
     nblk = int(abi.eap_bn_act_fromy_blocks(n, na))
@@ -1213,20 +1213,26 @@
     pgx = torch.empty_like(pg)
     gmax = torch.empty(b, c, na, dtype=torch.int32, device=y.device)
     xmax = torch.empty_like(gmax)
-    call('eap_bn_act_bwd_reduce_fromy_f32', y, b, c, n, na, slope, gy, y, beta, inv_gamma, pg, pgx, gmax, xmax)
+    if listed is not None:
+        call('eap_bn_act_bwd_reduce_fromy_listed_f32', y, b, c, n, na, slope, gy, y, beta, inv_gamma, listed, pg, pgx, gmax, xmax)
+    else:
+        call('eap_bn_act_bwd_reduce_fromy_f32', y, b, c, n, na, slope, gy, y, beta, inv_gamma, pg, pgx, gmax, xmax)
     if partials:
         return pg, pgx, gmax.view(torch.float32), xmax.view(torch.float32)
     return pg.sum(1, dtype=torch.float64), pgx.sum(1, dtype=torch.float64), gmax.view(torch.float32), xmax.view(torch.float32)
 
 
-def so3_dense_bwd_bn(gy, yact, geo, ldz, coef, rowbound, slope, packed=False):
+def so3_dense_bwd_bn(gy, yact, geo, ldz, coef, rowbound, slope, packed=False, listed=None):
     b, o, p, na = gy.shape
     ldz = na * geo.rp if ldz is None else int(ldz)
     colmap = geo.columns(None)
     l = p if colmap is None else colmap.shape[1]
     scale = torch.empty(2, b, na, o, dtype=torch.float32, device=gy.device)
     planes = torch.empty(b * na * o * ((l + 31) // 32 * 32), dtype=torch.int32, device=gy.device)
-    call('eap_so3_dense_split_bn_f32', gy, b, o, l, p, na, rowbound.view(torch.int32), colmap, gy, yact, coef, slope, scale, planes)
+    if listed is not None:
+        call('eap_so3_dense_split_bn_listed_f32', gy, b, o, l, p, na, rowbound.view(torch.int32), colmap, gy, yact, coef, listed, slope, scale, planes)
+    else:
+        call('eap_so3_dense_split_bn_f32', gy, b, o, l, p, na, rowbound.view(torch.int32), colmap, gy, yact, coef, slope, scale, planes)
     z = torch.empty(b, o, geo.ks, ldz, dtype=torch.float32, device=gy.device)
     return _dense_product(0, geo, b, o, l, ldz, scale, planes, z, 2.0 * b * o * l * na * geo.ks * geo.nn, packed=packed)
 
@@ -1245,9 +1251,10 @@
     slot[0] = (weakref.ref(t), t._version, tuple(t.shape), payload)
 
 
-def _take_hint(slot, t):
+def _take_hint(slot, t, use=None):
     h, slot[0] = slot[0], None
-    if not USE_ROWMAX_HINT or h is None or h[0]() is not t or h[1] != t._version or h[2] != tuple(t.shape):
+    use = USE_ROWMAX_HINT if use is None else use
+    if not use or h is None or h[0]() is not t or h[1] != t._version or h[2] != tuple(t.shape):
         return None
     return h[3]
 
@@ -1301,6 +1308,38 @@
     rowmax = _take_hint(_ROWMAX_HINT, t)
     ROWMAX_HINTS_TAKEN += rowmax is not None
     return rowmax
+
+
+_ROWS_HINT = [None]
+USE_ROWS_HINT = True
+ROWS_HINTS_TAKEN = 0
+
+
+def leave_rows_hint(t, rows, n_rows, rp):
+    rp = int(rp)
+    ok = (t.dim() == 4 and rp > 0 and rp % 16 == 0 and rows.dtype == torch.int32 and rows.dim() == 2 and rows.shape[0] == t.shape[0]
+          and rows.stride(1) == 1 and rows.shape[1] >= rp and rows.stride(0) >= rp
+          and (n_rows is None or (n_rows.dtype == torch.int32 and tuple(n_rows.shape) == (t.shape[0],) and n_rows.is_contiguous())))
+    _ROWS_HINT[0] = None
+    if ok:
+        _leave_hint(_ROWS_HINT, t, (rows, n_rows, rp))
+
+
+def take_rows_hint(t):
+    global ROWS_HINTS_TAKEN
+    payload = _take_hint(_ROWS_HINT, t, USE_ROWS_HINT)
+    ROWS_HINTS_TAKEN += payload is not None
+    return payload
+
+
+def rows_bitmask(rows, n_rows, rp, n):
+    b = rows.shape[0]
+    if rows.dtype != torch.int32 or rows.stride(1) != 1 or (n_rows is not None and (n_rows.dtype != torch.int32 or not n_rows.is_contiguous()
+                                                                                    or tuple(n_rows.shape) != (b,))):
+        raise RuntimeError('rows_bitmask: rows and n_rows must be int32, the rows of `rows` contiguous, one n_rows per cloud')
+    mask = torch.empty(b, int(abi.eap_rows_bitmask_words(int(n))), dtype=torch.int32, device=rows.device)
+    call('eap_rows_bitmask', rows, b, int(n), int(rp), rows.stride(0), rows, n_rows, mask)
+    return mask
 
 
 def bn_act_bwd_apply(gy, x, b, c, n, scale, shift, mean, invstd, k2, k3, slope):
@@ -1350,25 +1389,31 @@
     return y
 
 
-def narrow_conv_bwd_reduce(gy, x, W, scale, shift, mean, invstd, slope, partials=False):
+def narrow_conv_bwd_reduce(gy, x, W, scale, shift, mean, invstd, slope, partials=False, listed=None):
     check_input(gy, x, W, scale, shift, mean, invstd)
     b, ck, n = x.shape
     o = W.shape[0]
     pg, pgx = _narrow_partials(x, b, o, n)
-    call('eap_narrow_conv_bwd_reduce_f32', x, b, o, ck, n, slope, gy, x, W, scale, shift, mean, invstd, pg, pgx)
+    if listed is not None:
+        call('eap_narrow_conv_bwd_reduce_listed_f32', x, b, o, ck, n, int(listed[1]), slope, gy, x, W, scale, shift, mean, invstd, listed[0], pg, pgx)
+    else:
+        call('eap_narrow_conv_bwd_reduce_f32', x, b, o, ck, n, slope, gy, x, W, scale, shift, mean, invstd, pg, pgx)
     if partials:
         return pg, pgx
     return pg.sum(1, dtype=torch.float64), pgx.sum(1, dtype=torch.float64)
 
 
-def narrow_conv_bwd_dw(gy, x, W, scale, shift, mean, invstd, k2, k3, slope):
+def narrow_conv_bwd_dw(gy, x, W, scale, shift, mean, invstd, k2, k3, slope, listed=None):
     check_input(gy, x, W, scale, shift, mean, invstd, k2, k3)
     b, ck, n = x.shape
     o = W.shape[0]
     nseg = int(abi.eap_narrow_conv_segments(n))
     partial = torch.empty(b * nseg, o, ck, dtype=torch.float32, device=x.device)
     dW = torch.empty(o, ck, dtype=torch.float32, device=x.device)
-    call('eap_narrow_conv_bwd_dw_f32', x, b, o, ck, n, slope, gy, x, W, scale, shift, mean, invstd, k2, k3, partial, dW)
+    if listed is not None:
+        call('eap_narrow_conv_bwd_dw_listed_f32', x, b, o, ck, n, int(listed[1]), slope, gy, x, W, scale, shift, mean, invstd, k2, k3, listed[0], partial, dW)
+    else:
+        call('eap_narrow_conv_bwd_dw_f32', x, b, o, ck, n, slope, gy, x, W, scale, shift, mean, invstd, k2, k3, partial, dW)
     return dW
 
 
diff --git a/equi-articulated-pose_amd/vgtk/so3conv/functional.py b/equi-articulated-pose_amd/vgtk/so3conv/functional.py
--- a/equi-articulated-pose_amd/vgtk/so3conv/functional.py
+++ b/equi-articulated-pose_amd/vgtk/so3conv/functional.py
@@ -976,13 +976,26 @@
     return bool(_hip.NATIVE_NORM_GLUE and gy.is_cuda and isinstance(count, int) and not norm_fold._syncing(sync))
 
 
+def _listed_rows(gy, narrow=True):
+    hint = _hip.take_rows_hint(gy) if gy.dim() == 4 and gy.is_cuda and gy.is_contiguous() else None
+    if hint is None:
+        return None
+    if BACKWARD_LOG is not None and BACKWARD_LOG:
+        BACKWARD_LOG[-1]['grad rows'] = 'listed'
+    mask = _hip.rows_bitmask(*hint, gy.shape[2])
+    return (mask, gy.shape[3]) if narrow else mask
+
+
 def _backward_narrow(gy, W, x, bn, need_w):
     scale, shift, mean, invstd, count, slope, sync = bn
     b, o = gy.shape[0], gy.shape[1]
+    if _native_norm_bwd(gy, count, sync):
+        listed = _listed_rows(gy)
+        gy = gy.view(b, o, -1)
+        g_bn_w, g_bn_b, k2, k3 = _hip.norm_fold_bwd(*_hip.narrow_conv_bwd_reduce(gy, x, W, scale, shift, mean, invstd, slope, partials=True, listed=listed),
+                                                    scale, count)
+        return (_hip.narrow_conv_bwd_dw(gy, x, W, scale, shift, mean, invstd, k2, k3, slope, listed=listed) if need_w else None), g_bn_w, g_bn_b
     gy = gy.view(b, o, -1)
-    if _native_norm_bwd(gy, count, sync):
-        g_bn_w, g_bn_b, k2, k3 = _hip.norm_fold_bwd(*_hip.narrow_conv_bwd_reduce(gy, x, W, scale, shift, mean, invstd, slope, partials=True), scale, count)
-        return (_hip.narrow_conv_bwd_dw(gy, x, W, scale, shift, mean, invstd, k2, k3, slope) if need_w else None), g_bn_w, g_bn_b
     sg, sgx = _hip.narrow_conv_bwd_reduce(gy, x, W, scale, shift, mean, invstd, slope)
     gW = None
     if need_w:
@@ -1039,6 +1052,7 @@
     gFc = torch.empty(b, c, ldz, dtype=torch.float32, device=z.device)
     _hip.matmul_tail(_weight_operand(W, c, ks), zm, gFc, ncols, (words.view(torch.int32), 4, 1.0))
     gF = _hip.rows_scatter_packed(gFc, c, head.rows, head.n_rows, rp, n, na)
+    _hip.leave_rows_hint(gF, head.rows, head.n_rows, rp)
     fc = _hip.rows_gather_packed(feats, head.rows, head.n_rows, rp, ldz)
     dt = torch.empty(c, o * ks, dtype=torch.float32, device=z.device)
     _hip.matmul_reduce_tail(fc[..., :ra], zm[..., :ra].transpose(1, 2), dt, ncols)
@@ -1058,8 +1072,10 @@
     if bn is not None:
         k1, beta, inv_gamma, count, slope, sync = bn
         native = _native_norm_bwd(gy, count, sync)
+        listed = None
         if native:
-            pg, pgx, gmax, xmax = _hip.bn_act_bwd_reduce_fromy(gy, yact, beta, inv_gamma, slope, partials=True)
+            listed = _listed_rows(gy, narrow=False)
+            pg, pgx, gmax, xmax = _hip.bn_act_bwd_reduce_fromy(gy, yact, beta, inv_gamma, slope, partials=True, listed=listed)
             g_bn_w, g_bn_b, _, _, coef, bound, colmax = _hip.norm_fold_bwd(pg, pgx, k1, count, beta, inv_gamma, gmax, xmax)
         else:
             sg, sgx, gmax, xmax = _hip.bn_act_bwd_reduce_fromy(gy, yact, beta, inv_gamma, slope)
@@ -1068,9 +1084,9 @@
             coef = torch.stack([k1, k2, k3, beta, inv_gamma]).contiguous()
             bound = (k1.abs()[None, :, None] * gmax + k2.abs()[None, :, None] + k3.abs()[None, :, None] * xmax).contiguous()
         if DENSE_TAIL_PACKED and native and _dense_tail_packed_takes(W, feats, head, geo, c, pad_c, ldz, need_f, need_w):
-            z = _hip.so3_dense_bwd_bn(gy, yact, geo, ldz, coef, bound, slope, packed=True)
+            z = _hip.so3_dense_bwd_bn(gy, yact, geo, ldz, coef, bound, slope, packed=True, listed=listed)
             return (*_dense_tail_packed(z, W, feats, head, geo, colmax, p, ldz, need_f, need_w), g_bn_w, g_bn_b)
-        z = _hip.so3_dense_bwd_bn(gy, yact, geo, ldz, coef, bound, slope)
+        z = _hip.so3_dense_bwd_bn(gy, yact, geo, ldz, coef, bound, slope, listed=listed)
         if ldz % 4 == 0 and rp % 4 == 0 and native:
             z_bound = (_hip.so3_dense_zbound(colmax, head.cnt, head.n_rows, rp, p, ldz).view(torch.int32), 4, 1.0)
         elif ldz % 4 == 0 and rp % 4 == 0:
@@ -1085,6 +1101,7 @@
     if need_f:
         gFr = _rows_grad_from_z(z, _weight_operand(W, c, ks, pad_c), c, rp, na, ldz, True, z_bound)
         gF = _hip.rows_scatter(gFr.contiguous(), head.rows, n)
+        _hip.leave_rows_hint(gF, head.rows, None, rp)
     if need_w:
         gW = _weight_grad_rows(z, _hip.rows_gather(feats, head.rows, rp), o, ks, ldz, True)
     return gF, gW, g_bn_w, g_bn_b
@@ -1118,6 +1135,8 @@
             gW = gw if gW is None else gW + gw
         del z
     gF = _hip.rows_scatter(gFr, head.rows, n) if need_f else None
+    if need_f:
+        _hip.leave_rows_hint(gF, head.rows, None, rp)
     return gF, gW
 
 
diff --git a/include/eap_hip.h b/include/eap_hip.h
--- a/include/eap_hip.h
+++ b/include/eap_hip.h
@@ -213,6 +213,8 @@
                                const float *src, float *dst, eap_stream_t stream);
 int eap_rows_scatter_packed_f32(int b, int c, int c_ld, int n, int na, int rp, int rows_ld, int64_t ld, const int32_t *rows,
                                 const int32_t *n_rows, const float *src, float *dst, eap_stream_t stream);
+int eap_rows_bitmask_words(int n);
+int eap_rows_bitmask(int b, int n, int rp, int rows_ld, const int32_t *rows, const int32_t *n_rows, uint32_t *mask, eap_stream_t stream);
 
 int eap_so3_dense_supported(int p, int na, int ks, int rp, int o);
 int eap_so3_dense_member(int b, int p, int n, int nn, int rp, int rows_ld, const int32_t *idx, const int32_t *rows,
@@ -234,6 +236,9 @@
                                             float *y, float *psum, float *psq, eap_stream_t stream);
 int eap_so3_dense_split_bn_f32(int b, int m, int l, int l_src, int na, const uint32_t *rowbound, const int32_t *colmap, const float *grad,
                                const float *act, const float *coef, float slope, float *scale, void *planes, eap_stream_t stream);
+int eap_so3_dense_split_bn_listed_f32(int b, int m, int l, int l_src, int na, const uint32_t *rowbound, const int32_t *colmap, const float *grad,
+                                      const float *act, const float *coef, const uint32_t *listed, float slope, float *scale, void *planes,
+                                      eap_stream_t stream);
 int eap_so3_dense_untranspose_bnact_f32(int b, int o, int p, int na, int p_dst, const int32_t *map, const float *yt, const float *bn_scale,
                                         const float *bn_shift, float slope, float *y, eap_stream_t stream);
 int eap_so3_dense_gplanes_supported(int o, int c, int na, int ks, int rp);
@@ -419,6 +424,9 @@
 int eap_bn_act_fromy_blocks(int64_t n, int na);
 int eap_bn_act_bwd_reduce_fromy_f32(int b, int c, int64_t n, int na, float slope, const float *gy, const float *y, const float *beta,
                                     const float *inv_gamma, float *pg, float *pgx, uint32_t *gmax, uint32_t *xmax, eap_stream_t stream);
+int eap_bn_act_bwd_reduce_fromy_listed_f32(int b, int c, int64_t n, int na, float slope, const float *gy, const float *y, const float *beta,
+                                           const float *inv_gamma, const uint32_t *listed, float *pg, float *pgx, uint32_t *gmax, uint32_t *xmax,
+                                           eap_stream_t stream);
 
 int eap_bn_stats_masked_f32(int b, int c, int64_t n, int na, const float *x, const float *mask, float *psum, float *psq,
                             eap_stream_t stream);
@@ -448,6 +456,12 @@
 int eap_narrow_conv_bwd_dw_f32(int b, int o, int ck, int64_t n, float slope, const float *gy, const float *x, const float *W,
                                const float *scale, const float *shift, const float *mean, const float *invstd, const float *k2,
                                const float *k3, float *partial, float *dW, eap_stream_t stream);
+int eap_narrow_conv_bwd_reduce_listed_f32(int b, int o, int ck, int64_t n, int na, float slope, const float *gy, const float *x, const float *W,
+                                          const float *scale, const float *shift, const float *mean, const float *invstd, const uint32_t *listed,
+                                          float *pg, float *pgx, eap_stream_t stream);
+int eap_narrow_conv_bwd_dw_listed_f32(int b, int o, int ck, int64_t n, int na, float slope, const float *gy, const float *x, const float *W,
+                                      const float *scale, const float *shift, const float *mean, const float *invstd, const float *k2,
+                                      const float *k3, const uint32_t *listed, float *partial, float *dW, eap_stream_t stream);
 
 int eap_norm_fold_train_f32(int o, int parts, int64_t pivot_stride, int64_t count, int64_t eps_bits, int64_t momentum_bits, const float *ps,
                             const float *pq, const float *pivot, const float *gamma, const float *beta, float *running_mean, float *running_var,
```

Result: no change. 173.7 point-clouds/sec (median of 6 runs) (+0.4%).
